# NDLOHGRP/pyReCoDe

Measured on AMD Instinct MI355X. Metric: frames/sec + GB/s in, 4096x4096 uint16 @1% sparsity, 1/2/4/8 GPU, higher is better.
Workload: dtype u16; 1 GPU; 4096x4096 uint16, 1.00% sparsity, L1 + LZ4 frame, source_bit_depth 16, batch 64 frames/GPU/step, 256-frame stack/GPU in HBM; parallelism=dp1 (contiguous frame blocks per rank; single process: no collective), gather_every=0, gathers_issued_in_all=0, launch=single process, collective_ranks=1

## Files before the change

### pyrecode_amd/csrc/rc_api.hip

```cpp
#include "rc_host.h"
#include "rc_deflate_model.h"

thread_local std::string g_last_error;
WorkerPool *g_pool = new WorkerPool;
Util g_utils[RC_MAX_DEV];
thread_local Util *t_util = nullptr;


struct rc_ctx {
    int device = 0;
    hipStream_t own_stream = nullptr, stream = nullptr;
    uint32_t nx = 0, ny = 0, depth = 0, level = 0, op_mode = 0, scheme = 0, clevel = 0, max_batch = 0;
    uint32_t emit = rc::EMIT_RAW;
    rc::Scratch sets[2];
    int cur = 0;
    int last = 0;
    const rc::Scratch &geo() const { return sets[0]; }
    const rc::Scratch &recent() const { return sets[last]; }
    DevMem dmem, model_mem[2];
    PinMem hmem;
    hipStream_t pstream = nullptr;
    hipStream_t pstream_b = nullptr;
    hipStream_t last_ps = nullptr;
    bool two_chains = false;
    hipEvent_t ev_red[2] = {}, ev_post[2] = {}, ev_in[2] = {};
    bool post_pending[2] = {false, false};
    bool pipelined = false;
    bool thr_set = false;
    bool keep_bitmap = true;
    uint32_t src_bytes = 2;
    uint32_t *thr32 = nullptr;
    uint32_t last_n = 0;
    DevBuf d_frames, d_out, d_dark;
    uint64_t *d_rec_off = nullptr;
    uint32_t *d_md = nullptr;
    void *d_ztab = nullptr;
    rc::ValueStage values = rc::VALUES_NONE;
    bool values_on = false;
    bool modelled = false, model_ready = false;
    rc::ZstdModel *d_model = nullptr, *h_model = nullptr;
    rc::ZstdSample *d_sample = nullptr, *h_sample = nullptr;
    rc::DeflateModel *d_dzm = nullptr, *h_dzm = nullptr;
    uint32_t *d_dzhist = nullptr, *h_dzhist = nullptr;
    uint32_t l2_sum = 0;
    rc::u32x2 *d_l2_node[2] = {};
    uint16_t *d_l2_base[2] = {};
    rc::BatchStatus *h_status = nullptr;
    rc::BatchStatus *d_first_err = nullptr;
    uint32_t batch_seq = 0;
    const uint8_t *prev_out = nullptr, *prev_rec = nullptr, *prev_md = nullptr;
    uint64_t prev_out_cap = 0;
    uint32_t prev_n = 0;
    hipEvent_t ev[5] = {};
    float stage_ms[5] = {};
    bool profiling = false;
    uint32_t prof_every = 1, prof_phase = 0;
    bool profile_all = getenv("RC_PROFILE_ALL_STAGES") != nullptr;
    struct PipeSlot {
        uint8_t *d_in = nullptr;
        uint8_t *d_out = nullptr;
        uint64_t *d_rec = nullptr, *h_rec = nullptr;
        uint32_t *d_md = nullptr, *h_md = nullptr;
        rc::BatchStatus *h_stat = nullptr;
        hipEvent_t ev_h2d = nullptr, ev_done = nullptr, ev_fetch = nullptr, ev_val = nullptr;
        uint32_t *d_val = nullptr, *h_val = nullptr;
        bool has_val = false;
        uint32_t n = 0;
        bool zero_copy = false;
        enum State { FREE, SUBMITTED, RESULT_TAKEN, FETCHING } state = FREE;
    } pipe[RC_PIPE_SLOTS];
    hipStream_t copy_stream = nullptr, d2h_stream = nullptr;
    uint32_t val_gap = 0, val_x0 = 0, val_y0 = 0, val_w = 0, val_h = 0;
    std::vector<hipEvent_t> prof_ev;
    size_t prof_used = 0;
    double prof_sum_ms[5] = {};
    uint64_t prof_batches = 0;
};

RC_EXPORT int rc_abi_version(void) { return RC_ABI_VERSION; }

RC_EXPORT const char *rc_strerror(int status)
{
    switch (status) {
    case RC_OK: return "ok";
    case RC_ERR_BAD_ARG: return "bad argument";
    case RC_ERR_OUT_TOO_SMALL: return "output buffer too small";
    case RC_ERR_DEVICE: return "GPU / HIP error";
    case RC_ERR_UNSUPPORTED: return "not implemented on device";
    case RC_ERR_RECORD_TOO_LARGE: return "Buffer size smaller than compressed data size";
    case RC_ERR_CORRUPT: return "corrupt input stream";
    case RC_ERR_WORKSPACE: return "out of device memory for the ctx's workspace";
    default: return "unknown status";
    }
}
RC_EXPORT const char *rc_last_error(void) { return g_last_error.c_str(); }

RC_EXPORT int rc_device_count(int *count)
{
    if (!count) return fail(RC_ERR_BAD_ARG, "count is NULL");
    int n = 0;
    if (hipGetDeviceCount(&n) != hipSuccess) {
        (void)hipGetLastError();
        n = 0;
    }
    *count = n;
    return RC_OK;
}
RC_EXPORT int rc_scheme_on_device(uint32_t scheme)
{
    return (scheme == RC_SCHEME_LZ4 || scheme == RC_SCHEME_ZSTD || scheme == RC_SCHEME_BLOSC_LZ4 || scheme == RC_SCHEME_ZLIB_DEVICE) ? 1 : 0;
}

static int alloc_set(rc_ctx *c, rc::Scratch &sc, DevMem &model_mem)
{
    using namespace rc;
    DevMem &m = c->dmem;
    const uint64_t B = c->max_batch, T = sc.ntiles;
    RC_ALLOC(m, sc.bitmap, B * sc.nb_stride + 64);
    RC_ALLOC(m, sc.tile_cnt, B * T * 4);
    RC_ALLOC(m, sc.tile_off, B * T * 4);
    RC_ALLOC(m, sc.tile_next, B * T * 4);
    RC_ALLOC(m, sc.frame_nnz, B * 4);
    RC_ALLOC(m, sc.frame_cbytes, B * 4);
    RC_ALLOC(m, sc.scan_part, B * ((T + 255) / 256) * 32);
    RC_ALLOC(m, sc.status, sizeof(BatchStatus));
    if (c->level != 3) RC_ALLOC(m, sc.pix_slots, B * T * TILE_PX * 2 + 64);
    if (c->emit != EMIT_RAW) {
        if (c->level == 1) {
            sc.comb = c->emit == EMIT_ZSTD ? COMB_AT_BLK_SLOT : COMB_BEHIND_BLOCK;
            sc.blk_stride = 1536;
        }
        RC_ALLOC(m, sc.blk_slots, B * T * (uint64_t)sc.blk_stride + 256);
        RC_ALLOC(m, sc.blk_size, B * T * 4);
        RC_ALLOC(m, sc.blk_off, B * T * 4);
        if (c->emit == EMIT_DEFLATE) {
            RC_ALLOC(m, sc.blk_aux, B * T * 4);
            RC_ALLOC(m, sc.zl_acc, B * 32);
            HIP_TRY(hipMemset(sc.zl_acc, 0, B * 32));
        }
    }
    if (c->values != VALUES_NONE) {
        const ValueGeom g = value_geom(c->values);
        sc.pixraw_stride = ((sc.N * 2 + 15) & ~15ull) + 32;
        sc.nchunk_max = (uint32_t)((sc.N * 2 + g.chunk - 1) / g.chunk) + 1;
        RC_ALLOC(model_mem, sc.pixraw, B * sc.pixraw_stride + 64);
        RC_ALLOC(model_mem, sc.pix_chunks, B * (uint64_t)sc.nchunk_max * g.slot + 64);
        if (c->values == VALUES_DEFLATE_HUFF) RC_ALLOC(model_mem, sc.chunk_aux, B * (uint64_t)(sc.nchunk_max + 1) * 8);
        RC_ALLOC(model_mem, sc.chunk_size, B * (uint64_t)sc.nchunk_max * 4);
        RC_ALLOC(model_mem, sc.chunk_off, B * (uint64_t)sc.nchunk_max * 4);
        RC_ALLOC(model_mem, sc.frame_pbytes, B * 4);
        HIP_TRY(hipMemset(sc.frame_pbytes, 0, B * 4));
    }
    HIP_TRY(hipMemset(sc.frame_nnz, 0, B * 4));
    HIP_TRY(hipMemset(sc.frame_cbytes, 0, B * 4));
    HIP_TRY(hipMemset(sc.status, 0, sizeof(BatchStatus)));
    return RC_OK;
}

static void free_value_stage(rc_ctx *c)
{
    c->values = rc::VALUES_NONE;
    c->values_on = false;
    for (int k = 0; k < 2; ++k) {
        rc::Scratch &set = c->sets[k];
        c->model_mem[k].release_all();
        set.pixraw = nullptr; set.pix_chunks = nullptr; set.chunk_aux = nullptr; set.chunk_size = nullptr; set.chunk_off = nullptr;
        set.frame_pbytes = nullptr; set.pixraw_stride = 0; set.nchunk_max = 0;
    }
}

static int ctx_alloc(rc_ctx *c)
{
    using namespace rc;
    const uint64_t B = c->max_batch;
    RC_ON_DEVICE(c->device);
    HIP_TRY(hipStreamCreateWithFlags(&c->own_stream, hipStreamNonBlocking));
    HIP_TRY(hipStreamCreateWithFlags(&c->pstream, hipStreamNonBlocking));
    {
        int lo = 0, hi = 0;
        HIP_TRY(hipDeviceGetStreamPriorityRange(&lo, &hi));
        HIP_TRY(hipStreamCreateWithPriority(&c->pstream_b, hipStreamNonBlocking, hi));
    }
    c->last_ps = c->pstream;
    c->stream = c->own_stream;
    DevMem &m = c->dmem;
    int r;
    RC_ALLOC(m, c->sets[0].thr, c->geo().N * 2);
    RC_ALLOC(m, c->d_first_err, sizeof(BatchStatus));
    HIP_TRY(hipMemset(c->d_first_err, 0, sizeof(BatchStatus)));
    c->sets[0].first_err = c->d_first_err;
    c->sets[1] = c->sets[0];
    for (int k = 0; k < 2; ++k)
        if ((r = alloc_set(c, c->sets[k], c->model_mem[k])) != RC_OK) return r;
    c->two_chains = false;
    if (c->level == 2) {
        const uint64_t ids = (uint64_t)c->geo().ntiles * rc::TILE_PX;
        RC_ALLOC(m, c->d_l2_node[0], B * ids * 8);
        HIP_TRY(hipMemset(c->d_l2_node[0], 0, B * ids * 8));
        RC_ALLOC(m, c->d_l2_base[0], B * (uint64_t)c->geo().ntiles * 64 * 2);
        for (int i = 0; i < 2; ++i) {
            Scratch &set = c->sets[i];
            set.l2_node = c->d_l2_node[0]; set.l2_ids_per_frame = ids; set.l2_base = c->d_l2_base[0];
        }
    }
    if (c->emit == EMIT_ZSTD) {
        if ((r = zstd_encoder_tables(m, c->d_ztab)) != RC_OK) return r;
        c->modelled = c->clevel != 0;
        if (c->modelled) {
            RC_ALLOC(m, c->d_model, sizeof(ZstdModel));
            RC_ALLOC(m, c->d_sample, sizeof(ZstdSample));
            RC_ALLOC(c->hmem, c->h_model, sizeof(ZstdModel));
            RC_ALLOC(c->hmem, c->h_sample, sizeof(ZstdSample));
        }
    }
    if (c->values == VALUES_DEFLATE_HUFF) {
        RC_ALLOC(m, c->d_dzm, sizeof(DeflateModel));
        RC_ALLOC(m, c->d_dzhist, 256 * 4);
        RC_ALLOC(c->hmem, c->h_dzm, sizeof(DeflateModel));
        RC_ALLOC(c->hmem, c->h_dzhist, 256 * 4);
    }
    RC_ALLOC(m, c->d_rec_off, (B + 1) * 8);
    RC_ALLOC(m, c->d_md, B * 3 * 4);
    RC_ALLOC(c->hmem, c->h_status, 2 * sizeof(BatchStatus));
    for (auto &e : c->ev) HIP_TRY(hipEventCreate(&e));
    for (auto &e : c->ev_red) HIP_TRY(hipEventCreateWithFlags(&e, hipEventDisableTiming));
    for (auto &e : c->ev_post) HIP_TRY(hipEventCreateWithFlags(&e, hipEventDisableTiming));
    for (auto &e : c->ev_in) HIP_TRY(hipEventCreateWithFlags(&e, hipEventDisableTiming));
    return RC_OK;
}

RC_EXPORT rc_ctx *rc_ctx_create(uint32_t nx, uint32_t ny, uint32_t src_bit_depth, uint32_t reduction_level,
                                uint32_t op_mode, uint32_t scheme, uint32_t clevel, int device_id, uint32_t max_batch,
                                int *status)
{
    int dummy;
    if (!status) status = &dummy;
    *status = RC_OK;
    if (nx == 0 || ny == 0 || max_batch == 0 || max_batch > 65535u || op_mode > 1) {
        *status = fail(RC_ERR_BAD_ARG, "nx, ny, max_batch must be > 0, max_batch <= 65535 and op_mode 0 or 1");
        return nullptr;
    }
    if ((uint64_t)nx * ny >= (1ull << 32)) {
        *status = fail(RC_ERR_BAD_ARG, "nx*ny must be < 2^32");
        return nullptr;
    }
    if ((uint64_t)nx * ny * 2 >= (1ull << 32)) {
        *status = fail(RC_ERR_UNSUPPORTED, "a raw frame of 4 GiB or more (nx*ny*bytes_per_pixel >= 2^32) does not fit the format's u32 size fields");
        return nullptr;
    }
    if (reduction_level < 1 || reduction_level > 3) {
        *status = fail(RC_ERR_UNSUPPORTED, "reduction_level 4 (centroiding) is not implemented on device");
        return nullptr;
    }
    if (reduction_level == 2 && nx > 65535u) {
        *status = fail(RC_ERR_UNSUPPORTED, "reduction_level 2 needs nx <= 65535");
        return nullptr;
    }
    if (src_bit_depth < 1 || src_bit_depth > 32) {
        *status = fail(RC_ERR_UNSUPPORTED, "source_bit_depth must be 1..32 (uint8 / uint16 / uint32 source frames)");
        return nullptr;
    }
    int ndev = 0;
    if (hipGetDeviceCount(&ndev) != hipSuccess || device_id < 0 || device_id >= ndev) {
        (void)hipGetLastError();
        *status = fail(RC_ERR_DEVICE, "no such HIP device (this library has no CPU path)");
        return nullptr;
    }
    rc_ctx *c = new (std::nothrow) rc_ctx();
    if (!c) {
        *status = fail(RC_ERR_DEVICE, "out of host memory");
        return nullptr;
    }
    c->device = device_id;
    c->nx = nx; c->ny = ny; c->depth = src_bit_depth; c->level = reduction_level; c->op_mode = op_mode;
    c->scheme = scheme; c->clevel = clevel; c->max_batch = max_batch;
    c->emit = (op_mode == 1 && rc_scheme_on_device(scheme)) ? scheme : rc::EMIT_RAW;
    c->values = rc::value_stage_of(c->emit, clevel, reduction_level);
    rc::Scratch &sc = c->sets[0];
    sc.N = (uint64_t)nx * ny;
    sc.ntiles = (uint32_t)((sc.N + rc::TILE_PX - 1) / rc::TILE_PX);
    sc.nb = (sc.N + 7) / 8;
    sc.nb_stride = (uint64_t)sc.ntiles * rc::TILE_BM;
    sc.max_batch = max_batch;
    sc.guarded_loads = getenv("RC_REDUCE_GUARDED_LOADS") != nullptr;
    int rcode = ctx_alloc(c);
    if (rcode != RC_OK) {
        *status = rcode;
        std::string keep = g_last_error;
        rc_ctx_destroy(c);
        g_last_error = keep;
        return nullptr;
    }
    return c;
}

RC_EXPORT int rc_ctx_destroy(rc_ctx *c)
{
    if (!c) return RC_OK;
    DeviceGuard dev_guard_;
    (void)dev_guard_.enter(c->device);
    for (hipStream_t st : {c->stream, c->pstream, c->pstream_b, c->own_stream, c->copy_stream, c->d2h_stream})
        if (st) (void)hipStreamSynchronize(st);
    c->dmem.release_all();
    for (DevMem &m : c->model_mem) m.release_all();
    c->hmem.release_all();
    for (auto &p : c->pipe)
        for (hipEvent_t e : {p.ev_h2d, p.ev_done, p.ev_fetch, p.ev_val})
            if (e) (void)hipEventDestroy(e);
    for (hipEvent_t e : {c->ev_red[0], c->ev_red[1], c->ev_post[0], c->ev_post[1], c->ev_in[0], c->ev_in[1]})
        if (e) (void)hipEventDestroy(e);
    for (auto &e : c->ev)
        if (e) (void)hipEventDestroy(e);
    for (auto &e : c->prof_ev) (void)hipEventDestroy(e);
    for (hipStream_t st : {c->copy_stream, c->d2h_stream, c->pstream, c->pstream_b, c->own_stream})
        if (st) (void)hipStreamDestroy(st);
    delete c;
    return RC_OK;
}

RC_EXPORT int rc_ctx_set_stream(rc_ctx *c, void *hip_stream)
{
    if (!c) return fail(RC_ERR_BAD_ARG, "ctx is NULL");
    c->stream = hip_stream ? reinterpret_cast<hipStream_t>(hip_stream) : c->own_stream;
    return RC_OK;
}

RC_EXPORT int rc_set_threshold(rc_ctx *c, const void *thr)
{
    if (!c || !thr) return fail(RC_ERR_BAD_ARG, "ctx / thr is NULL");
    if (c->depth > 16 && c->src_bytes != 4) return fail(RC_ERR_BAD_ARG, "src_bit_depth > 16 means uint32 sources: rc_ctx_set_source_bytes(ctx, 4) first");
    RC_ON_DEVICE(c->device);
    HIP_TRY(hipMemcpyAsync(c->src_bytes == 4 ? (void *)c->thr32 : (void *)c->geo().thr, thr, c->geo().N * (c->src_bytes == 4 ? 4 : 2),
                           is_device_ptr(thr) ? hipMemcpyDeviceToDevice : hipMemcpyHostToDevice,
                           c->stream));
    HIP_TRY(hipStreamSynchronize(c->stream));
    c->thr_set = true;
    return RC_OK;
}

RC_EXPORT int rc_set_dark(rc_ctx *c, const void *dark, int64_t epsilon)
{
    if (!c || !dark) return fail(RC_ERR_BAD_ARG, "ctx / dark is NULL");
    RC_ON_DEVICE(c->device);
    const void *src = dark;
    const uint64_t bytes = c->geo().N * c->src_bytes;
    if (!is_device_ptr(dark)) {
        int r = c->d_dark.ensure(c->dmem, bytes);
        if (r != RC_OK) return r;
        HIP_TRY(hipMemcpyAsync(c->d_dark.p, dark, bytes, hipMemcpyHostToDevice, c->stream));
        src = c->d_dark.p;
    }
    if (c->depth > 16 && c->src_bytes != 4) return fail(RC_ERR_BAD_ARG, "src_bit_depth > 16 means uint32 sources: rc_ctx_set_source_bytes(ctx, 4) first");
    if (c->src_bytes == 4) rc::launch_threshold32(static_cast<const uint32_t *>(src), epsilon, c->geo().N, c->thr32, c->stream);
    else rc::launch_threshold(src, epsilon, c->geo().N, c->geo().thr, c->stream, c->src_bytes);
    HIP_TRY(hipGetLastError());
    HIP_TRY(hipStreamSynchronize(c->stream));
    c->thr_set = true;
    return RC_OK;
}

RC_EXPORT int rc_ctx_set_source_bytes(rc_ctx *c, uint32_t bytes_per_pixel)
{
    if (!c) return fail(RC_ERR_BAD_ARG, "ctx is NULL");
    if (bytes_per_pixel != 1 && bytes_per_pixel != 2 && bytes_per_pixel != 4) return fail(RC_ERR_BAD_ARG, "rc_ctx_set_source_bytes: 1 (uint8), 2 (uint16) or 4 (uint32)");
    if (bytes_per_pixel == 1 && c->depth > 8) return fail(RC_ERR_BAD_ARG, "rc_ctx_set_source_bytes: uint8 sources need src_bit_depth <= 8");
    if (bytes_per_pixel == 2 && c->depth > 16) return fail(RC_ERR_BAD_ARG, "rc_ctx_set_source_bytes: uint16 sources need src_bit_depth <= 16");
    if (c->batch_seq || c->thr_set) return fail(RC_ERR_BAD_ARG, "rc_ctx_set_source_bytes: call before rc_set_dark / rc_set_threshold and the first batch");
    if (c->geo().N * bytes_per_pixel >= (1ull << 32))
        return fail(RC_ERR_UNSUPPORTED, "rc_ctx_set_source_bytes: a raw frame of 4 GiB or more (nx*ny*bytes_per_pixel >= 2^32) does not fit the format's u32 size fields");
    if (bytes_per_pixel == 4) {
        if (c->depth <= 16) return fail(RC_ERR_BAD_ARG, "rc_ctx_set_source_bytes: uint32 sources are what source_bit_depth > 16 means (misc.py:41-49)");
        if (c->level == 2) return fail(RC_ERR_UNSUPPORTED, "rc_ctx_set_source_bytes: reduction level 2 is not implemented for uint32 sources");
        if (c->emit == rc::EMIT_DEFLATE) return fail(RC_ERR_UNSUPPORTED, "rc_ctx_set_source_bytes: the device DEFLATE encoder is not implemented for uint32 sources (use RC_SCHEME_ZLIB: the host's zlib)");
        RC_ON_DEVICE(c->device);
        uint32_t *thr32 = nullptr;
        uint16_t *slots[2] = {nullptr, nullptr};
        bool ok = c->dmem.try_alloc(thr32, c->geo().N * 4) == hipSuccess;
        for (int k = 0; ok && k < 2 && c->level != 3; ++k)
            ok = c->dmem.try_alloc(slots[k], (uint64_t)c->max_batch * c->geo().ntiles * rc::TILE_PX * 4 + 64) == hipSuccess;
        if (!ok) {
            (void)hipGetLastError();
            c->dmem.free_one(thr32);
            for (uint16_t *&p : slots) c->dmem.free_one(p);
            return fail(RC_ERR_DEVICE, "rc_ctx_set_source_bytes: out of device memory for the uint32 threshold / residual slots");
        }
        if (c->depth % 8 == 0) c->depth = 32;
        c->modelled = false;
        free_value_stage(c);
        c->thr32 = thr32;
        for (int k = 0; k < 2; ++k) {
            rc::Scratch *set = &c->sets[k];
            set->pix_slot_bytes = rc::TILE_PX * 4;
            set->comb = rc::COMB_OFF;
            if (c->level != 3) {
                c->dmem.free_one(set->pix_slots);
                set->pix_slots = slots[k];
            }
        }
    }
    c->src_bytes = bytes_per_pixel;
    return RC_OK;
}
RC_EXPORT uint32_t rc_ctx_source_bytes(const rc_ctx *c) { return c ? c->src_bytes : 0; }

RC_EXPORT uint64_t rc_out_capacity(const rc_ctx *c, uint32_t n) { return c ? (uint64_t)n * c->geo().N * c->src_bytes : 0; }

RC_EXPORT uint32_t rc_md_fields(const rc_ctx *c)
{
    if (!c) return 0;
    const bool comp = c->emit != rc::EMIT_RAW;
    if (c->level != 3) return comp ? 3 : 1;
    return comp ? 1 : 0;
}

static int fit_value_model(rc_ctx *c, const void *frames_dev, uint32_t n)
{
    using namespace rc;
    const bool dz = c->values == VALUES_DEFLATE_HUFF;
    hipStream_t s = c->stream;
    const Scratch &sc = c->sets[c->cur];
    const uint32_t ns = n < 2 ? n : 2;
    void *d_sample = dz ? (void *)c->d_dzhist : c->d_sample, *h_sample = dz ? (void *)c->h_dzhist : c->h_sample;
    void *d_model = dz ? (void *)c->d_dzm : c->d_model, *h_model = dz ? (void *)c->h_dzm : c->h_model;
    const size_t sample_bytes = dz ? 256 * 4 : sizeof(ZstdSample), model_bytes = dz ? sizeof(DeflateModel) : sizeof(ZstdModel);
    for (int k = 0; k < 2; ++k)
        if (c->post_pending[k]) HIP_TRY(hipStreamWaitEvent(s, c->ev_post[k], 0));
    HIP_TRY(hipMemsetAsync(d_sample, 0, sample_bytes, s));
    if (dz) {
        launch_reduce(sc, frames_dev, ns, 1u, CODEC_DEFLATE, true, c->depth, s, nullptr, c->src_bytes);
        launch_scans(sc, ns, true, true, s);
        RecordParams rp;
        rp.level = 1u; rp.emit = c->emit; rp.depth = c->depth; rp.first_frame_id = 0; rp.packed_slots = 1u;
        rp.frame_bytes = c->geo().N * c->src_bytes;
        rp.pix_mode = PIX_MODE_FLAT;
        launch_assemble(sc, rp, ns, nullptr, nullptr, c->batch_seq, s);
        launch_pd_hist(sc, ns, c->depth, c->d_dzhist, s);
    } else {
        launch_reduce(sc, frames_dev, ns, c->level == 3 ? 3u : 1u, CODEC_ZSTD_FAST, true, c->depth, s, nullptr, c->src_bytes);
        launch_zstd_sample(sc, ns, c->level == 1, c->depth, c->d_sample, s);
    }
    HIP_TRY(hipGetLastError());
    HIP_TRY(hipMemcpyAsync(h_sample, d_sample, sample_bytes, hipMemcpyDeviceToHost, s));
    HIP_TRY(hipStreamSynchronize(s));
    if (dz) {
        dm_build_model(c->h_dzhist, c->h_dzm);
        c->values_on = c->h_dzm->usable != 0;
    } else {
        zstd_model_from_sample(c->h_sample, c->h_model, c->clevel == 1 ? 50u : (c->clevel == 2 ? 20u : 0u));
        if (c->values == VALUES_NONE || !zm_code_pays(c->h_sample->pix, c->h_model->pix_code)) c->h_model->valid &= ~ZM_PIX_CODE;
        c->values_on = (c->h_model->valid & ZM_PIX_CODE) != 0;
    }
    HIP_TRY(hipMemcpyAsync(d_model, h_model, model_bytes, hipMemcpyHostToDevice, s));
    HIP_TRY(hipStreamSynchronize(s));
    for (Scratch &set : c->sets) {
        if (dz) { set.dz_model = c->d_dzm; continue; }
        const ZstdModel &M = *c->h_model;
        set.zm_model = c->d_model;
        set.zm_lit_code = c->d_model->lit_code;
        set.zm_valid = M.valid;
        set.zm_budget = zm_block_budget(M, BLK_SLOT);
        set.zm_seq_bits = (M.valid & ZM_SEQ_TABLES) ? M.seq.ll_log + M.seq.ml_log : 12u;
    }
    c->model_ready = true;
    return RC_OK;
}

static uint32_t fused_codec(uint32_t emit, uint32_t clevel, bool modelled, uint32_t src_bytes)
{
    using namespace rc;
    switch (emit) {
    case EMIT_ZSTD: return modelled && src_bytes != 4 ? CODEC_ZSTD_MODELLED : CODEC_ZSTD_FAST;
    case EMIT_LZ4: return clevel != 0 ? CODEC_LZ4_EVENTS : CODEC_LZ4_RUNS;
    case EMIT_BLOSC: return CODEC_BLOSC;
    case EMIT_DEFLATE: return CODEC_DEFLATE;
    default: return CODEC_NONE;
    }
}

static int enqueue_batch(rc_ctx *c, const void *frames_dev, uint32_t n, uint32_t first_frame_id, uint8_t *out_dev,
                         uint64_t out_cap, uint64_t *rec_off_dev, uint32_t *md_dev, bool timed)
{
    using namespace rc;
    hipStream_t s = c->stream;
    if ((c->modelled || c->values == VALUES_DEFLATE_HUFF) && !c->model_ready) {
        int r = fit_value_model(c, frames_dev, n);
        if (r != RC_OK) return r;
    }
    RecordParams rp;
    rp.level = c->level == 3 ? 3u : 1u;
    rp.emit = c->emit; rp.depth = c->depth; rp.first_frame_id = first_frame_id;
    rp.packed_slots = 1u;
    rp.frame_bytes = c->geo().N * c->src_bytes;
    hipEvent_t *ev = nullptr;
    if (timed) ev = c->ev;
    else if (c->profiling && (c->prof_phase++ % c->prof_every) == 0) {
        if (c->prof_used + 5 > c->prof_ev.size()) {
            for (int i = 0; i < 5; ++i) {
                hipEvent_t e;
                HIP_TRY(hipEventCreate(&e));
                c->prof_ev.push_back(e);
            }
        }
        ev = c->prof_ev.data() + c->prof_used;
        c->prof_used += 5;
    }
    const int k = c->cur;
    c->cur ^= 1;
    c->last = k;
    const rc::Scratch &sc = c->sets[k];
    const bool two = c->pipelined && c->two_chains;
    hipStream_t ps = two && k == 1 ? c->pstream_b : c->pstream;
    c->last_ps = ps;
    if (c->post_pending[k]) HIP_TRY(hipStreamWaitEvent(s, c->ev_post[k], 0));
    if (ev) HIP_TRY(hipEventRecord(ev[0], s));
    const bool fitted_seq = c->modelled && (c->h_model->valid & ZM_SEQ_TABLES);
    hipStream_t tail = nullptr;
    if (sc.N % TILE_PX) {
        HIP_TRY(hipEventRecord(c->ev_in[k], s));
        HIP_TRY(hipStreamWaitEvent(ps, c->ev_in[k], 0));
        tail = ps;
    }
    const uint32_t codec = fused_codec(c->emit, c->clevel, c->modelled, c->src_bytes);
    const bool keep_maps = c->keep_bitmap || c->emit == EMIT_RAW;
    if (c->src_bytes == 4)
        launch_reduce32(sc, static_cast<const uint32_t *>(frames_dev), c->thr32, n, c->level, c->depth, s, codec, keep_maps);
    else
        launch_reduce(sc, frames_dev, n, c->level, codec, keep_maps, c->depth, s, tail, c->src_bytes);
    const bool all_ev = ev && (timed || c->profile_all);
    hipEvent_t red = ev ? ev[1] : c->ev_red[k];
    HIP_TRY(hipEventRecord(red, s));
    HIP_TRY(hipStreamWaitEvent(ps, red, 0));
    if (c->level == 2) launch_l2(sc, n, c->nx, c->l2_sum, c->depth, ps);
    const bool lits_only = c->modelled && (c->h_model->valid & ZM_LITS_ONLY);
    if (c->emit == EMIT_ZSTD && !lits_only) launch_zstd_fse(sc, n, fitted_seq ? (const void *)&c->d_model->seq : c->d_ztab, fitted_seq, ps);
    if (all_ev) HIP_TRY(hipEventRecord(ev[2], ps));
    launch_scans(sc, n, c->level != 3, c->emit != EMIT_RAW, ps);
    if (all_ev) HIP_TRY(hipEventRecord(ev[3], ps));
    if (c->values_on) {
        rp.pix_mode = PIX_MODE_FLAT;
        launch_assemble(sc, rp, n, out_dev, rec_off_dev, c->batch_seq, ps);
        launch_values_encode(c->values, sc, n, c->depth, ps);
        launch_values_scan(c->values, sc, n, c->depth, ps);
        rp.pix_mode = PIX_MODE_SKIP;
    }
    if (two && c->post_pending[k ^ 1]) {
        auto overlap = [](const uint8_t *a, uint64_t an, const uint8_t *b, uint64_t bn) { return a && b && a < b + bn && b < a + an; };
        const uint8_t *rec8 = reinterpret_cast<const uint8_t *>(rec_off_dev), *md8 = reinterpret_cast<const uint8_t *>(md_dev);
        if (overlap(out_dev, out_cap, c->prev_out, c->prev_out_cap) || overlap(rec8, (uint64_t)(n + 1) * 8, c->prev_rec, (uint64_t)(c->prev_n + 1) * 8) ||
            overlap(md8, (uint64_t)n * 12, c->prev_md, (uint64_t)c->prev_n * 12))
            HIP_TRY(hipStreamWaitEvent(ps, c->ev_post[k ^ 1], 0));
    }
    c->prev_out = out_dev; c->prev_out_cap = out_cap; c->prev_n = n;
    c->prev_rec = reinterpret_cast<const uint8_t *>(rec_off_dev); c->prev_md = reinterpret_cast<const uint8_t *>(md_dev);
    launch_layout(sc, rp, n, out_cap, rec_off_dev, md_dev, ps);
    launch_assemble(sc, rp, n, out_dev, rec_off_dev, c->batch_seq, ps);
    ++c->batch_seq;
    if (c->values_on) launch_values_gather(c->values, sc, n, c->depth, 16, out_dev, rec_off_dev, ps);
    if (ev) HIP_TRY(hipEventRecord(ev[4], ps));
    if (two && c->post_pending[k ^ 1]) HIP_TRY(hipStreamWaitEvent(ps, c->ev_post[k ^ 1], 0));
    HIP_TRY(hipEventRecord(c->ev_post[k], ps));
    c->post_pending[k] = true;
    if (!c->pipelined) HIP_TRY(hipStreamWaitEvent(s, c->ev_post[k], 0));
    HIP_TRY(hipGetLastError());
    c->last_n = n;
    return RC_OK;
}

static int check_batch_args(rc_ctx *c, const void *frames, uint32_t n, const void *out, const void *rec, const void *md)
{
    if (!c || !frames || !out || !rec || !md) return fail(RC_ERR_BAD_ARG, "NULL argument");
    if (n == 0 || n > c->max_batch) return fail(RC_ERR_BAD_ARG, "n must be in 1..max_batch");
    if (!c->thr_set) return fail(RC_ERR_BAD_ARG, "threshold not set (rc_set_threshold / rc_set_dark)");
    return RC_OK;
}

RC_EXPORT int rc_reduce_compress_batch_async(rc_ctx *c, const void *frames_dev, uint32_t n, uint32_t first_frame_id,
                                             uint8_t *out_dev, uint64_t out_cap, uint64_t *rec_offsets_dev, uint32_t *md_dev)
{
    int r = check_batch_args(c, frames_dev, n, out_dev, rec_offsets_dev, md_dev);
    if (r != RC_OK) return r;
    RC_ON_DEVICE(c->device);
    return enqueue_batch(c, frames_dev, n, first_frame_id, out_dev, out_cap, rec_offsets_dev, md_dev, false);
}

static void l2_second_chain(rc_ctx *c)
{
    if (c->level != 2 || c->two_chains) return;
    const uint64_t B = c->max_batch, ids = (uint64_t)c->geo().ntiles * rc::TILE_PX;
    if (!c->d_l2_node[1]) {
        bool ok = c->dmem.try_alloc(c->d_l2_node[1], B * ids * 8) == hipSuccess && hipMemset(c->d_l2_node[1], 0, B * ids * 8) == hipSuccess &&
                  c->dmem.try_alloc(c->d_l2_base[1], B * (uint64_t)c->geo().ntiles * 64 * 2) == hipSuccess && hipDeviceSynchronize() == hipSuccess;
        if (!ok) {
            (void)hipGetLastError();
            c->dmem.free_one(c->d_l2_node[1]);
            c->dmem.free_one(c->d_l2_base[1]);
            return;
        }
    }
    c->sets[1].l2_node = c->d_l2_node[1];
    c->sets[1].l2_base = c->d_l2_base[1];
    c->two_chains = true;
}

RC_EXPORT int rc_ctx_set_pipelined(rc_ctx *c, int on)
{
    if (!c) return fail(RC_ERR_BAD_ARG, "ctx is NULL");
    RC_ON_DEVICE(c->device);
    HIP_TRY(hipStreamSynchronize(c->pstream));
    HIP_TRY(hipStreamSynchronize(c->pstream_b));
    if (on) l2_second_chain(c);
    c->pipelined = on != 0;
    return RC_OK;
}
RC_EXPORT int rc_ctx_wait_results(rc_ctx *c, void *hip_stream)
{
    if (!c) return fail(RC_ERR_BAD_ARG, "ctx is NULL");
    RC_ON_DEVICE(c->device);
    if (c->post_pending[c->last])
        HIP_TRY(hipStreamWaitEvent(hip_stream ? reinterpret_cast<hipStream_t>(hip_stream) : c->stream, c->ev_post[c->last], 0));
    return RC_OK;
}

RC_EXPORT int rc_ctx_sync(rc_ctx *c)
{
    if (!c) return fail(RC_ERR_BAD_ARG, "ctx is NULL");
    RC_ON_DEVICE(c->device);
    HIP_TRY(hipStreamSynchronize(c->pstream_b));
    HIP_TRY(hipMemcpyAsync(&c->h_status[0], c->recent().status, sizeof(rc::BatchStatus), hipMemcpyDeviceToHost, c->pstream));
    HIP_TRY(hipMemcpyAsync(&c->h_status[1], c->d_first_err, sizeof(rc::BatchStatus), hipMemcpyDeviceToHost, c->pstream));
    HIP_TRY(hipMemsetAsync(c->d_first_err, 0, sizeof(rc::BatchStatus), c->pstream));
    HIP_TRY(hipStreamSynchronize(c->pstream));
    HIP_TRY(hipStreamSynchronize(c->stream));
    const uint32_t n_batches = c->batch_seq;
    c->batch_seq = 0;
    for (size_t b = 0; b + 5 <= c->prof_used; b += 5) {
        float ms;
        if (!c->profile_all) {
            if (hipEventElapsedTime(&ms, c->prof_ev[b], c->prof_ev[b + 1]) == hipSuccess) c->prof_sum_ms[0] += ms;
        } else
        for (int i = 0; i < 4; ++i)
            if (hipEventElapsedTime(&ms, c->prof_ev[b + i], c->prof_ev[b + i + 1]) == hipSuccess) c->prof_sum_ms[i] += ms;
        if (hipEventElapsedTime(&ms, c->prof_ev[b], c->prof_ev[b + 4]) == hipSuccess) c->prof_sum_ms[4] += ms;
        ++c->prof_batches;
    }
    c->prof_used = 0;
    if (c->h_status[1].total != 0) c->h_status[1] = rc::first_err_decode(c->h_status[1].total);
    if (c->h_status[1].code != 0) {
        char msg[160];
        if (n_batches > 1)
            snprintf(msg, sizeof msg, "%s (frame %u of batch %llu of the %u enqueued since the last sync)", rc_strerror(c->h_status[1].code),
                     c->h_status[1].frame, (unsigned long long)c->h_status[1].total, n_batches);
        else
            snprintf(msg, sizeof msg, "%s (frame %u of the batch)", rc_strerror(c->h_status[1].code), c->h_status[1].frame);
        return fail(c->h_status[1].code, msg);
    }
    return RC_OK;
}

RC_EXPORT int rc_reduce_compress_batch(rc_ctx *c, const void *frames, uint32_t n, uint32_t first_frame_id, uint8_t *out,
                                       uint64_t out_cap, uint64_t *rec_offsets, uint32_t *md)
{
    int r = check_batch_args(c, frames, n, out, rec_offsets, md);
    if (r != RC_OK) return r;
    RC_ON_DEVICE(c->device);
    const uint64_t frame_bytes = c->geo().N * c->src_bytes;
    const void *fdev = frames;
    if (!is_device_ptr(frames)) {
        r = c->d_frames.ensure(c->dmem, (uint64_t)n * frame_bytes);
        if (r != RC_OK) return r;
        HIP_TRY(hipMemcpyAsync(c->d_frames.p, frames, (uint64_t)n * frame_bytes, hipMemcpyHostToDevice, c->stream));
        fdev = c->d_frames.p;
    }
    uint8_t *odev = out;
    uint64_t cap = out_cap;
    const bool out_host = !is_device_ptr(out);
    if (out_host) {
        const uint64_t worst = (uint64_t)n * frame_bytes;
        cap = out_cap < worst ? out_cap : worst;
        r = c->d_out.ensure(c->dmem, cap);
        if (r != RC_OK) return r;
        odev = c->d_out.p;
    }
    r = enqueue_batch(c, fdev, n, first_frame_id, odev, cap, c->d_rec_off, c->d_md, true);
    if (r != RC_OK) return r;
    r = rc_ctx_sync(c);
    for (int i = 0; i < 4; ++i) (void)hipEventElapsedTime(&c->stage_ms[i], c->ev[i], c->ev[i + 1]);
    (void)hipEventElapsedTime(&c->stage_ms[4], c->ev[0], c->ev[4]);
    if (r != RC_OK) return r;
    int r2 = copy_out(rec_offsets, c->d_rec_off, (uint64_t)(n + 1) * 8, c->stream);
    if (r2 == RC_OK) r2 = copy_out(md, c->d_md, (uint64_t)n * 12, c->stream);
    if (r2 == RC_OK && out_host) r2 = copy_out(out, c->d_out.p, c->h_status->total, c->stream);
    if (r2 != RC_OK) return r2;
    HIP_TRY(hipStreamSynchronize(c->stream));
    return RC_OK;
}

RC_EXPORT void *rc_host_alloc(uint64_t bytes)
{
    void *p = nullptr;
    if (hipHostMalloc(&p, bytes ? bytes : 16, hipHostMallocDefault) != hipSuccess) {
        (void)hipGetLastError();
        fail(RC_ERR_DEVICE, "hipHostMalloc failed");
        return nullptr;
    }
    return p;
}
RC_EXPORT int rc_host_free(void *p)
{
    if (p) HIP_TRY(hipHostFree(p));
    return RC_OK;
}
RC_EXPORT int rc_host_register(void *p, uint64_t bytes)
{
    if (!p || !bytes) return fail(RC_ERR_BAD_ARG, "NULL / zero argument");
    HIP_TRY(hipHostRegister(p, bytes, hipHostRegisterDefault));
    return RC_OK;
}
RC_EXPORT int rc_host_unregister(void *p)
{
    if (p) HIP_TRY(hipHostUnregister(p));
    return RC_OK;
}

static int pipe_slot_init(rc_ctx *c, rc_ctx::PipeSlot &p)
{
    const uint64_t B = c->max_batch;
    if (!c->copy_stream) HIP_TRY(hipStreamCreateWithFlags(&c->copy_stream, hipStreamNonBlocking));
    if (!c->d2h_stream) HIP_TRY(hipStreamCreateWithFlags(&c->d2h_stream, hipStreamNonBlocking));
    RC_ALLOC(c->dmem, p.d_in, B * c->geo().N * c->src_bytes + 64);
    RC_ALLOC(c->dmem, p.d_out, rc_out_capacity(c, (uint32_t)B) + 64);
    RC_ALLOC(c->dmem, p.d_rec, (B + 1) * 8);
    RC_ALLOC(c->dmem, p.d_md, B * 12);
    RC_ALLOC(c->hmem, p.h_rec, (B + 1) * 8);
    RC_ALLOC(c->hmem, p.h_md, B * 12);
    RC_ALLOC(c->hmem, p.h_stat, sizeof(rc::BatchStatus));
    HIP_TRY(hipEventCreateWithFlags(&p.ev_h2d, hipEventDisableTiming));
    HIP_TRY(hipEventCreateWithFlags(&p.ev_done, hipEventDisableTiming));
    HIP_TRY(hipEventCreateWithFlags(&p.ev_fetch, hipEventDisableTiming));
    HIP_TRY(hipEventCreateWithFlags(&p.ev_val, hipEventDisableTiming));
    RC_ALLOC(c->dmem, p.d_val, B * 4 + 64);
    RC_ALLOC(c->hmem, p.h_val, B * 4 + 64);
    return RC_OK;
}

RC_EXPORT int rc_ctx_set_validation(rc_ctx *c, uint32_t gap, uint32_t x0, uint32_t y0, uint32_t w, uint32_t h)
{
    if (!c) return fail(RC_ERR_BAD_ARG, "ctx is NULL");
    if (gap && (w == 0 || h == 0 || w > 128 || h > 128 || (uint64_t)x0 + w > c->nx || (uint64_t)y0 + h > c->ny))
        return fail(RC_ERR_BAD_ARG, "rc_ctx_set_validation: the region must lie inside the frame and hold at most 128 x 128 pixels");
    c->val_gap = gap; c->val_x0 = x0; c->val_y0 = y0; c->val_w = w; c->val_h = h;
    return RC_OK;
}

RC_EXPORT int rc_pipe_validation(rc_ctx *c, uint32_t slot, uint32_t *counts)
{
    if (!c || slot >= RC_PIPE_SLOTS || !counts) return fail(RC_ERR_BAD_ARG, "NULL argument / slot out of range");
    rc_ctx::PipeSlot &p = c->pipe[slot];
    if (p.state != p.SUBMITTED && p.state != p.RESULT_TAKEN) return fail(RC_ERR_BAD_ARG, "nothing submitted on this slot");
    if (!p.has_val) { for (uint32_t i = 0; i < p.n; ++i) counts[i] = 0xFFFFFFFFu; return RC_OK; }
    HIP_TRY(hipEventSynchronize(p.ev_val));
    memcpy(counts, p.h_val, (uint64_t)p.n * 4);
    return RC_OK;
}

RC_EXPORT int rc_pipe_submit(rc_ctx *c, uint32_t slot, const void *frames_host, uint32_t n, uint32_t first_frame_id)
{
    if (!c || !frames_host || slot >= RC_PIPE_SLOTS) return fail(RC_ERR_BAD_ARG, "NULL argument / slot out of range");
    if (n == 0 || n > c->max_batch) return fail(RC_ERR_BAD_ARG, "n must be in 1..max_batch");
    if (!c->thr_set) return fail(RC_ERR_BAD_ARG, "threshold not set (rc_set_threshold / rc_set_dark)");
    RC_ON_DEVICE(c->device);
    rc_ctx::PipeSlot &p = c->pipe[slot];
    if (p.state != p.FREE) return fail(RC_ERR_BAD_ARG, "slot is still in use (result / fetch_wait not called)");
    if (!p.d_in) {
        int r = pipe_slot_init(c, p);
        if (r != RC_OK) return r;
    }
    if (!c->pipelined) {
        HIP_TRY(hipStreamSynchronize(c->pstream));
        HIP_TRY(hipStreamSynchronize(c->pstream_b));
        l2_second_chain(c);
        c->pipelined = true;
    }
    const void *fdev = nullptr;
    hipPointerAttribute_t a;
    if (hipPointerGetAttributes(&a, frames_host) == hipSuccess) {
        if (a.type == hipMemoryTypeHost && a.devicePointer) fdev = a.devicePointer;
    } else (void)hipGetLastError();
    p.zero_copy = fdev != nullptr;
    if (!fdev) {
        HIP_TRY(hipMemcpyAsync(p.d_in, frames_host, (uint64_t)n * c->geo().N * c->src_bytes, hipMemcpyHostToDevice, c->copy_stream));
        HIP_TRY(hipEventRecord(p.ev_h2d, c->copy_stream));
        HIP_TRY(hipStreamWaitEvent(c->stream, p.ev_h2d, 0));
        fdev = p.d_in;
    }
    int r = enqueue_batch(c, fdev, n, first_frame_id, p.d_out, rc_out_capacity(c, c->max_batch), p.d_rec, p.d_md, false);
    if (r != RC_OK) return r;
    p.has_val = c->val_gap != 0;
    if (p.has_val) {
        rc::launch_roi_components(fdev, c->src_bytes == 4 ? (const void *)c->thr32 : (const void *)c->geo().thr, c->geo().N, c->nx, n, first_frame_id, c->val_gap, c->val_x0, c->val_y0, c->val_w, c->val_h, p.d_val, c->stream, c->src_bytes);
        HIP_TRY(hipGetLastError());
        HIP_TRY(hipMemcpyAsync(p.h_val, p.d_val, (uint64_t)n * 4, hipMemcpyDeviceToHost, c->stream));
        HIP_TRY(hipEventRecord(p.ev_val, c->stream));
    }
    if (p.zero_copy) HIP_TRY(hipEventRecord(p.ev_h2d, c->stream));
    hipStream_t ps = c->last_ps;
    HIP_TRY(hipMemcpyAsync(p.h_rec, p.d_rec, (uint64_t)(n + 1) * 8, hipMemcpyDeviceToHost, ps));
    HIP_TRY(hipMemcpyAsync(p.h_md, p.d_md, (uint64_t)n * 12, hipMemcpyDeviceToHost, ps));
    HIP_TRY(hipMemcpyAsync(p.h_stat, c->recent().status, sizeof(rc::BatchStatus), hipMemcpyDeviceToHost, ps));
    HIP_TRY(hipEventRecord(p.ev_done, ps));
    p.n = n;
    p.state = p.SUBMITTED;
    return RC_OK;
}

RC_EXPORT int rc_pipe_input_done(rc_ctx *c, uint32_t slot)
{
    if (!c || slot >= RC_PIPE_SLOTS) return fail(RC_ERR_BAD_ARG, "NULL argument / slot out of range");
    if (c->pipe[slot].state == rc_ctx::PipeSlot::FREE) return RC_OK;
    HIP_TRY(hipEventSynchronize(c->pipe[slot].ev_h2d));
    return RC_OK;
}

RC_EXPORT int rc_pipe_result(rc_ctx *c, uint32_t slot, uint64_t *rec_offsets, uint32_t *md, uint64_t *total)
{
    if (!c || slot >= RC_PIPE_SLOTS || !rec_offsets || !md || !total) return fail(RC_ERR_BAD_ARG, "NULL argument / slot out of range");
    rc_ctx::PipeSlot &p = c->pipe[slot];
    if (p.state != p.SUBMITTED) return fail(RC_ERR_BAD_ARG, "nothing submitted on this slot");
    HIP_TRY(hipEventSynchronize(p.ev_done));
    p.state = p.RESULT_TAKEN;
    if (p.h_stat->code != 0) {
        char msg[128];
        snprintf(msg, sizeof msg, "%s (frame %u of the batch)", rc_strerror(p.h_stat->code), p.h_stat->frame);
        p.state = p.FREE;
        return fail(p.h_stat->code, msg);
    }
    memcpy(rec_offsets, p.h_rec, (uint64_t)(p.n + 1) * 8);
    memcpy(md, p.h_md, (uint64_t)p.n * 12);
    *total = p.h_stat->total;
    return RC_OK;
}

RC_EXPORT int rc_pipe_fetch(rc_ctx *c, uint32_t slot, uint8_t *dst_host, uint64_t bytes)
{
    if (!c || slot >= RC_PIPE_SLOTS || (!dst_host && bytes)) return fail(RC_ERR_BAD_ARG, "NULL argument / slot out of range");
    rc_ctx::PipeSlot &p = c->pipe[slot];
    if (p.state != p.RESULT_TAKEN) return fail(RC_ERR_BAD_ARG, "rc_pipe_result has not been called for this slot");
    if (bytes > p.h_stat->total) return fail(RC_ERR_BAD_ARG, "more bytes than the batch's records hold");
    RC_ON_DEVICE(c->device);
    if (bytes) HIP_TRY(hipMemcpyAsync(dst_host, p.d_out, bytes, hipMemcpyDeviceToHost, c->d2h_stream));
    HIP_TRY(hipEventRecord(p.ev_fetch, c->d2h_stream));
    p.state = p.FETCHING;
    return RC_OK;
}

RC_EXPORT int rc_pipe_fetch_wait(rc_ctx *c, uint32_t slot)
{
    if (!c || slot >= RC_PIPE_SLOTS) return fail(RC_ERR_BAD_ARG, "NULL argument / slot out of range");
    rc_ctx::PipeSlot &p = c->pipe[slot];
    if (p.state == p.RESULT_TAKEN) { p.state = p.FREE; return RC_OK; }
    if (p.state != p.FETCHING) return fail(RC_ERR_BAD_ARG, "rc_pipe_fetch has not been called for this slot");
    HIP_TRY(hipEventSynchronize(p.ev_fetch));
    p.state = p.FREE;
    return RC_OK;
}

RC_EXPORT int rc_ctx_refit_model(rc_ctx *c)
{
    if (!c) return fail(RC_ERR_BAD_ARG, "ctx is NULL");
    c->model_ready = false;
    return RC_OK;
}

RC_EXPORT int rc_get_binary_map(rc_ctx *c, uint32_t i, uint8_t *bitmap_out)
{
    if (!c || !bitmap_out) return fail(RC_ERR_BAD_ARG, "NULL argument");
    if (i >= c->last_n) return fail(RC_ERR_BAD_ARG, "frame index outside the most recent batch");
    if (!c->keep_bitmap && c->emit != rc::EMIT_RAW && c->level != 2) return fail(RC_ERR_BAD_ARG, "binary maps are not kept (rc_ctx_keep_binary_maps(ctx, 0))");
    RC_ON_DEVICE(c->device);
    int r = copy_out(bitmap_out, c->recent().bitmap + (uint64_t)i * c->geo().nb_stride, c->geo().nb, c->stream);
    if (r != RC_OK) return r;
    HIP_TRY(hipStreamSynchronize(c->stream));
    return RC_OK;
}

RC_EXPORT int rc_ctx_set_profiling(rc_ctx *c, int on)
{
    if (!c) return fail(RC_ERR_BAD_ARG, "ctx is NULL");
    c->profiling = on != 0;
    c->prof_every = on > 1 ? (uint32_t)on : 1u;
    c->prof_phase = 0;
    for (double &v : c->prof_sum_ms) v = 0;
    c->prof_batches = 0;
    return RC_OK;
}
RC_EXPORT int rc_ctx_get_profile(rc_ctx *c, double sum_ms[5], uint64_t *batches)
{
    if (!c || !sum_ms || !batches) return fail(RC_ERR_BAD_ARG, "NULL argument");
    memcpy(sum_ms, c->prof_sum_ms, sizeof c->prof_sum_ms);
    *batches = c->prof_batches;
    return RC_OK;
}

RC_EXPORT int rc_ctx_set_l2_statistics(rc_ctx *c, uint32_t l2_statistics)
{
    if (!c || l2_statistics > 2) return fail(RC_ERR_BAD_ARG, "l2_statistics must be 0, 1 (max) or 2 (sum)");
    c->l2_sum = l2_statistics == 2 ? 1u : 0u;
    return RC_OK;
}

RC_EXPORT int rc_ctx_keep_binary_maps(rc_ctx *c, int on)
{
    if (!c) return fail(RC_ERR_BAD_ARG, "ctx is NULL");
    c->keep_bitmap = on != 0;
    return RC_OK;
}

RC_EXPORT int rc_get_stage_ms(rc_ctx *c, float ms[5])
{
    if (!c || !ms) return fail(RC_ERR_BAD_ARG, "NULL argument");
    memcpy(ms, c->stage_ms, sizeof c->stage_ms);
    return RC_OK;
}

RC_EXPORT int64_t rc_unpack_frame_sparse(uint32_t nx, uint32_t ny, uint32_t bit_depth, const uint8_t *bitmap,
                                         const uint8_t *pixvals, uint64_t pixvals_bytes, uint64_t *out,
                                         uint64_t out_cap_triplets, uint32_t reduction_level)
{
    if (!bitmap || nx == 0 || ny == 0 || (!out && out_cap_triplets)) return fail(RC_ERR_BAD_ARG, "NULL / zero argument");
    if (reduction_level == 1 && (bit_depth == 0 || bit_depth > 64)) return fail(RC_ERR_BAD_ARG, "bit_depth must be 1..64");
    if (reduction_level == 1 && !pixvals && pixvals_bytes) return fail(RC_ERR_BAD_ARG, "pixvals is NULL");
    UtilScope util_scope;
    int r = util_scope.enter();
    if (r != RC_OK) return r;
    Util &u = g_util;
    const uint64_t N = (uint64_t)nx * ny, nb = (N + 7) / 8, nb8 = (nb + 7) / 8;
    const uint32_t nblk = (uint32_t)((nb8 + rc::WG - 1) / rc::WG);
    const uint8_t *d_bm = nullptr, *d_px = nullptr;
    r = stage_in(bitmap, nb, u.a, d_bm, nb8 * 8 - nb + 8);
    if (r != RC_OK) return r;
    if (reduction_level == 1 && pixvals_bytes) {
        r = stage_in(pixvals, pixvals_bytes, u.b, d_px);
        if (r != RC_OK) return r;
    }
    r = u.w.ensure(u.dmem, (uint64_t)nblk * 8 + 16);
    if (r != RC_OK) return r;
    uint32_t *blk_cnt = u.w.as<uint32_t>(), *blk_off = blk_cnt + nblk;
    uint64_t *nnz_dev = reinterpret_cast<uint64_t *>(blk_cnt + 2 * (uint64_t)nblk);
    rc::launch_expand_count(d_bm, nb8, N, blk_cnt, blk_off, nnz_dev, u.stream);
    HIP_TRY(hipMemcpyAsync(u.h_scalar, nnz_dev, 8, hipMemcpyDeviceToHost, u.stream));
    HIP_TRY(hipStreamSynchronize(u.stream));
    const uint64_t nnz = *u.h_scalar;
    if (!out) return (int64_t)nnz;
    if (nnz > out_cap_triplets) return fail(RC_ERR_OUT_TOO_SMALL, "out holds fewer triplets than the bitmap has set bits");
    if (reduction_level == 1 && (nnz * bit_depth + 7) / 8 > pixvals_bytes)
        return fail(RC_ERR_CORRUPT, "pixvals shorter than popcount(bitmap) * bit_depth bits");
    if (nnz == 0) return 0;
    StagedOut so;
    if ((r = so.begin(out, nnz * 24)) != RC_OK) return r;
    rc::launch_expand_emit(d_bm, nb8, N, nx, blk_off, d_px, pixvals_bytes, bit_depth, reduction_level, nnz, so.as<uint64_t>(), u.stream);
    HIP_TRY(hipGetLastError());
    if ((r = so.finish(out, nnz * 24)) != RC_OK) return r;
    return (int64_t)nnz;
}

RC_EXPORT int rc_bit_pack(const uint16_t *pixvals, uint64_t n, uint32_t bit_depth, uint8_t *out, uint64_t out_n)
{
    if (!out || (!pixvals && n)) return fail(RC_ERR_BAD_ARG, "NULL argument");
    if (bit_depth == 0 || bit_depth > 32) return fail(RC_ERR_BAD_ARG, "bit_depth must be 1..32");
    if (out_n != (n * bit_depth + 7) / 8) return fail(RC_ERR_BAD_ARG, "out_n must be ceil(n*bit_depth/8)");
    if (out_n == 0) return RC_OK;
    UtilScope util_scope;
    int r = util_scope.enter();
    if (r != RC_OK) return r;
    Util &u = g_util;
    const uint16_t *d_in = nullptr;
    r = stage_in(pixvals, n * 2, u.a, d_in);
    if (r != RC_OK) return r;
    StagedOut so;
    if ((r = so.begin(out, out_n)) != RC_OK) return r;
    rc::launch_bit_pack(d_in, n, bit_depth, so.as<uint8_t>(), out_n, u.stream);
    HIP_TRY(hipGetLastError());
    return so.finish(out, out_n);
}

RC_EXPORT int rc_bit_unpack(const uint8_t *packed, uint64_t packed_bytes, uint64_t n, uint32_t bit_depth, uint64_t *out)
{
    if (!out || (!packed && packed_bytes)) return fail(RC_ERR_BAD_ARG, "NULL argument");
    if (bit_depth == 0 || bit_depth > 64) return fail(RC_ERR_BAD_ARG, "bit_depth must be 1..64");
    if ((n * bit_depth + 7) / 8 > packed_bytes) return fail(RC_ERR_CORRUPT, "packed shorter than n * bit_depth bits");
    if (n == 0) return RC_OK;
    UtilScope util_scope;
    int r = util_scope.enter();
    if (r != RC_OK) return r;
    Util &u = g_util;
    const uint8_t *d_in = nullptr;
    r = stage_in(packed, packed_bytes, u.a, d_in);
    if (r != RC_OK) return r;
    StagedOut so;
    if ((r = so.begin(out, n * 8)) != RC_OK) return r;
    rc::launch_bit_unpack(d_in, packed_bytes, n, bit_depth, so.as<uint64_t>(), u.stream);
    HIP_TRY(hipGetLastError());
    return so.finish(out, n * 8);
}

RC_EXPORT int rc_synth_dark(int device_id, uint32_t seed, uint64_t n_pixels, uint16_t *dark_dev)
{
    if (!dark_dev) return fail(RC_ERR_BAD_ARG, "NULL argument");
    RC_ON_DEVICE(device_id);
    rc::launch_synth_dark(seed, n_pixels, dark_dev, nullptr);
    HIP_TRY(hipGetLastError());
    HIP_TRY(hipDeviceSynchronize());
    return RC_OK;
}
RC_EXPORT int rc_synth_frames_clustered(int device_id, uint32_t seed, uint32_t first_frame, uint32_t n_frames, uint32_t nx, uint32_t ny,
                                        uint32_t seed_ppm, const uint16_t *dark_dev, uint16_t *frames_dev)
{
    if (!dark_dev || !frames_dev || n_frames == 0 || nx == 0 || ny == 0) return fail(RC_ERR_BAD_ARG, "NULL / zero argument");
    if ((uint64_t)nx * ny > 0xFFFFFFFFull) return fail(RC_ERR_BAD_ARG, "rc_synth_frames_clustered: nx * ny must fit 32 bits");
    RC_ON_DEVICE(device_id);
    rc::launch_synth_frames_clustered(seed, first_frame, n_frames, nx, ny, seed_ppm, dark_dev, frames_dev, nullptr);
    HIP_TRY(hipGetLastError());
    HIP_TRY(hipDeviceSynchronize());
    return RC_OK;
}
RC_EXPORT int rc_synth_frames(int device_id, uint32_t seed, uint32_t first_frame, uint32_t n_frames, uint64_t n_pixels,
                              uint32_t sparsity_ppm, const uint16_t *dark_dev, uint16_t *frames_dev)
{
    if (!dark_dev || !frames_dev || n_frames == 0) return fail(RC_ERR_BAD_ARG, "NULL / zero argument");
    RC_ON_DEVICE(device_id);
    rc::launch_synth_frames(seed, first_frame, n_frames, n_pixels, sparsity_ppm, dark_dev, frames_dev, nullptr);
    HIP_TRY(hipGetLastError());
    HIP_TRY(hipDeviceSynchronize());
    return RC_OK;
}
```

### pyrecode_amd/csrc/rc_codec_api.hip

```cpp
#include "rc_host.h"

template <class Encode, class Total, class Gather>
static int tiled_compress(const uint8_t *src, uint64_t n, uint8_t *dst, uint64_t dst_cap, uint64_t *out_n, const uint8_t *empty, uint64_t empty_n,
                          Encode encode, Total total_of, Gather gather)
{
    using namespace rc;
    Util &u = g_util;
    if (n == 0) {
        if (dst_cap < empty_n) return fail(RC_ERR_OUT_TOO_SMALL, "rc_compress: dst too small");
        HIP_TRY(hipMemcpy(dst, empty, empty_n, is_device_ptr(dst) ? hipMemcpyHostToDevice : hipMemcpyHostToHost));
        *out_n = empty_n;
        return RC_OK;
    }
    Scratch sc;
    sc.ntiles = (uint32_t)((n + TILE_BM - 1) / TILE_BM);
    sc.nb = n;
    sc.nb_stride = (uint64_t)sc.ntiles * TILE_BM;
    const uint8_t *d_src = nullptr;
    int r = stage_in(src, n, u.a, d_src, sc.nb_stride - n + 16);
    if (r != RC_OK) return r;
    sc.bitmap = const_cast<uint8_t *>(d_src);
    const uint64_t T = sc.ntiles;
    r = u.w.ensure(u.dmem, T * BLK_SLOT + T * 8 + 64);
    if (r != RC_OK) return r;
    sc.blk_slots = u.w.p;
    sc.blk_size = reinterpret_cast<uint32_t *>(u.w.p + T * BLK_SLOT);
    sc.blk_off = sc.blk_size + T;
    sc.frame_cbytes = sc.blk_off + T;
    if ((r = encode(sc)) != RC_OK) return r;
    launch_scans(sc, 1, false, true, u.stream);
    HIP_TRY(hipMemcpyAsync(u.h_scalar, sc.frame_cbytes, 4, hipMemcpyDeviceToHost, u.stream));
    HIP_TRY(hipStreamSynchronize(u.stream));
    const uint64_t total = total_of(T, *reinterpret_cast<uint32_t *>(u.h_scalar));
    if (total > dst_cap) return fail(RC_ERR_OUT_TOO_SMALL, "rc_compress: dst too small (see rc_compress_bound)");
    StagedOut so;
    if ((r = so.begin(dst, total)) != RC_OK) return r;
    gather(sc, so.as<uint8_t>());
    HIP_TRY(hipGetLastError());
    if ((r = so.finish(dst, total)) != RC_OK) return r;
    *out_n = total;
    return RC_OK;
}

RC_EXPORT int rc_compress(uint32_t scheme, uint32_t level, const uint8_t *src, uint64_t n, uint8_t *dst, uint64_t dst_cap,
                          uint64_t *out_n)
{
    using namespace rc;
    if (!dst || !out_n || (!src && n)) return fail(RC_ERR_BAD_ARG, "NULL argument");
    if (scheme != RC_SCHEME_LZ4 && scheme != RC_SCHEME_ZSTD && scheme != RC_SCHEME_BLOSC_LZ4)
        return fail(RC_ERR_UNSUPPORTED, "rc_compress: compression scheme not implemented on device");
    UtilScope util_scope;
    int r = util_scope.enter();
    if (r != RC_OK) return r;
    Util &u = g_util;
    if (scheme == RC_SCHEME_BLOSC_LZ4) {
        if (n >= (1ull << 31) - 16) return fail(RC_ERR_BAD_ARG, "rc_compress: a blosc1 chunk holds < 2 GiB");
        const uint8_t f[16] = {2, 1, 0x36, 8, 0, 0, 0, 0, 0, 0, 0, 0, 16, 0, 0, 0};
        return tiled_compress(src, n, dst, dst_cap, out_n, f, sizeof f,
                              [&](const Scratch &sc) { launch_blosc_encode_blocks(sc, 1, u.stream); return RC_OK; },
                              [](uint64_t T, uint32_t blocks) { return 16ull + 4ull * T + blocks; },
                              [&](const Scratch &sc, uint8_t *d_out) { launch_blosc_gather(sc, d_out, u.stream); });
    }
    if (n >= (1ull << 32)) return fail(RC_ERR_BAD_ARG, "rc_compress: input must be < 4 GiB");
    if (scheme == RC_SCHEME_LZ4) {
        const uint32_t h = lz4f_descriptor(0x40);
        const uint8_t f[11] = {0x04, 0x22, 0x4D, 0x18, (uint8_t)h, (uint8_t)(h >> 8), (uint8_t)(h >> 16), 0, 0, 0, 0};
        return tiled_compress(src, n, dst, dst_cap, out_n, f, sizeof f,
                              [&](const Scratch &sc) { launch_lz4_encode_buffer(sc, u.stream, level != 0); return RC_OK; },
                              [](uint64_t, uint32_t blocks) { return 7ull + blocks + 4; },
                              [&](const Scratch &sc, uint8_t *d_out) { launch_lz4f_gather(sc, h, d_out, u.stream); });
    }
    const uint8_t f[9] = {0x28, 0xB5, 0x2F, 0xFD, 0x00, 0x00, 0x01, 0x00, 0x00};
    return tiled_compress(src, n, dst, dst_cap, out_n, f, sizeof f,
                          [&](const Scratch &sc) {
                              int rt = zstd_encoder_tables(u.dmem, u.ztab);
                              if (rt == RC_OK) launch_zstd_encode_blocks(sc, 1, u.ztab, u.stream);
                              return rt;
                          },
                          [](uint64_t, uint32_t blocks) { return 6ull + blocks; },
                          [&](const Scratch &sc, uint8_t *d_out) { launch_zstd_gather(sc, d_out, u.stream); });
}

static int lz4_decompress(const uint8_t *src, uint64_t n, uint8_t *dst, uint64_t dst_cap, uint64_t *out_n)
{
    using namespace rc;
    Util &u = g_util;
    HostView h;
    int r = h.open(src, n);
    if (r != RC_OK) return r;
    if (n < 11 || h.rd32(0) != 0x184D2204u) return fail(RC_ERR_CORRUPT, "not an LZ4 frame");
    const uint32_t flg = h[4], bd = h[5];
    if ((flg >> 6) != 1 || (flg & 2) || (bd & 0x8F) || ((bd >> 4) & 7) < 4) return fail(RC_ERR_CORRUPT, "bad LZ4 frame descriptor");
    const int linked = !((flg >> 5) & 1), bsum = (flg >> 4) & 1, csize = (flg >> 3) & 1, csum = (flg >> 2) & 1, dict = flg & 1;
    const uint64_t bmax = 1ull << (8 + 2 * ((bd >> 4) & 7));
    uint64_t ip = 6 + (csize ? 8 : 0) + (dict ? 4 : 0) + 1;
    std::vector<Lz4Block> blks;
    for (;;) {
        if (ip + 4 > n) return fail(RC_ERR_CORRUPT, "truncated LZ4 frame");
        uint32_t bs = h.rd32(ip);
        ip += 4;
        if (bs == 0) break;
        const uint32_t raw = bs >> 31;
        bs &= 0x7FFFFFFFu;
        if (bs > bmax || ip + bs > n) return fail(RC_ERR_CORRUPT, "LZ4 block exceeds the frame");
        blks.push_back(Lz4Block{ip, bs, raw});
        ip += bs + (bsum ? 4 : 0);
    }
    if (csum) ip += 4;
    if (ip != n) return fail(RC_ERR_CORRUPT, "trailing bytes after the LZ4 frame");
    const uint32_t nblk = (uint32_t)blks.size();
    if (nblk == 0) { *out_n = 0; return RC_OK; }
    const uint8_t *d_src = nullptr;
    r = stage_in(src, n, u.a, d_src);
    if (r != RC_OK) return r;
    const uint64_t tab = (uint64_t)nblk * sizeof(Lz4Block), szs = ((uint64_t)nblk * 4 + 7) & ~7ull, offs = (uint64_t)nblk * 8;
    r = u.w.ensure(u.dmem, tab + szs + offs + 16);
    if (r != RC_OK) return r;
    Lz4Block *d_blks = u.w.as<Lz4Block>();
    uint32_t *d_sizes = reinterpret_cast<uint32_t *>(u.w.p + tab);
    uint64_t *d_offs = reinterpret_cast<uint64_t *>(u.w.p + tab + szs);
    int *d_err = reinterpret_cast<int *>(u.w.p + tab + szs + offs);
    HIP_TRY(hipMemcpyAsync(d_blks, blks.data(), tab, hipMemcpyHostToDevice, u.stream));
    HIP_TRY(hipMemsetAsync(d_err, 0, 4, u.stream));
    launch_lz4_decode(d_src, d_blks, nblk, d_sizes, nullptr, nullptr, ~0ull, linked, d_err, u.stream);
    std::vector<uint32_t> sizes(nblk);
    int err = 0;
    HIP_TRY(hipMemcpyAsync(sizes.data(), d_sizes, (uint64_t)(linked ? 1 : nblk) * 4, hipMemcpyDeviceToHost, u.stream));
    HIP_TRY(hipMemcpyAsync(&err, d_err, 4, hipMemcpyDeviceToHost, u.stream));
    HIP_TRY(hipStreamSynchronize(u.stream));
    if (err) return fail(RC_ERR_CORRUPT, "malformed LZ4 block");
    std::vector<uint64_t> off(nblk, 0);
    uint64_t total = 0;
    if (linked) total = sizes[0];
    else
        for (uint32_t b = 0; b < nblk; ++b) {
            if (sizes[b] > bmax) return fail(RC_ERR_CORRUPT, "LZ4 block decodes beyond its declared maximum");
            off[b] = total;
            total += sizes[b];
        }
    *out_n = total;
    if (total > dst_cap) return fail(RC_ERR_OUT_TOO_SMALL, "rc_decompress: dst too small");
    if (total == 0) return RC_OK;
    StagedOut so;
    if ((r = so.begin(dst, total)) != RC_OK) return r;
    HIP_TRY(hipMemcpyAsync(d_offs, off.data(), offs, hipMemcpyHostToDevice, u.stream));
    uint32_t max_stored = 0;
    for (const Lz4Block &q : blks) if (q.raw) max_stored = std::max(max_stored, q.size);
    launch_lz4_decode(d_src, d_blks, nblk, nullptr, d_offs, so.as<uint8_t>(), total, linked, d_err, u.stream, max_stored);
    HIP_TRY(hipGetLastError());
    HIP_TRY(hipMemcpyAsync(&err, d_err, 4, hipMemcpyDeviceToHost, u.stream));
    if ((r = so.finish(dst, total)) != RC_OK) return r;
    if (err) return fail(RC_ERR_CORRUPT, "malformed LZ4 block");
    return RC_OK;
}

static int blosc_decompress(const uint8_t *src, uint64_t n, uint8_t *dst, uint64_t dst_cap, uint64_t *out_n)
{
    using namespace rc;
    Util &u = g_util;
    HostView h;
    int r = h.open(src, n);
    if (r != RC_OK) return r;
    if (n < 16 || h[0] != 2) return fail(RC_ERR_CORRUPT, "not a blosc1 chunk");
    const uint32_t flags = h[2], typesize = h[3] ? h[3] : 1;
    const uint64_t nbytes = h.rd32(4), blocksize = h.rd32(8), cbytes = h.rd32(12);
    if (cbytes != n || nbytes >= (1ull << 31)) return fail(RC_ERR_CORRUPT, "blosc1 header disagrees with the chunk length");
    *out_n = nbytes;
    if (nbytes > dst_cap) return fail(RC_ERR_OUT_TOO_SMALL, "rc_decompress: dst too small");
    if (nbytes == 0) return RC_OK;
    if (flags & 0x02) {
        if (n != 16 + nbytes) return fail(RC_ERR_CORRUPT, "bad memcpyed blosc1 chunk");
        HIP_TRY(hipMemcpy(dst, src + 16, nbytes, hipMemcpyDefault));
        return RC_OK;
    }
    if ((flags >> 5) != 1) return fail(RC_ERR_UNSUPPORTED, "blosc1 chunk: only the LZ4 codec is decoded on device");
    if (blocksize == 0 || blocksize > nbytes) return fail(RC_ERR_CORRUPT, "bad blosc1 blocksize");
    const uint64_t nblocks = (nbytes + blocksize - 1) / blocksize;
    if (16 + 4 * nblocks > n) return fail(RC_ERR_CORRUPT, "truncated blosc1 chunk");
    std::vector<Lz4Block> blks;
    std::vector<uint64_t> offs;
    std::vector<uint32_t> want;
    for (uint64_t b = 0; b < nblocks; ++b) {
        const uint64_t bsize = std::min<uint64_t>(blocksize, nbytes - b * blocksize);
        const bool leftover = bsize != blocksize;
        const bool split = !(flags & 0x10) && typesize <= 16 && blocksize / typesize >= 128 && !leftover;
        const uint32_t nsplits = split ? typesize : 1;
        const uint64_t neblock = bsize / nsplits;
        uint64_t pos = h.rd32(16 + 4 * b);
        for (uint32_t j = 0; j < nsplits; ++j) {
            if (pos + 4 > n) return fail(RC_ERR_CORRUPT, "blosc1 block table points outside the chunk");
            const uint32_t cs = h.rd32(pos);
            pos += 4;
            if (pos + cs > n || cs > neblock + neblock / 255 + 16) return fail(RC_ERR_CORRUPT, "blosc1 block exceeds the chunk");
            blks.push_back(Lz4Block{pos, cs, cs == neblock ? 1u : 0u});
            offs.push_back(b * blocksize + j * neblock);
            want.push_back((uint32_t)neblock);
            pos += cs;
        }
    }
    const uint32_t nb = (uint32_t)blks.size();
    const uint8_t *d_src = nullptr;
    r = stage_in(src, n, u.a, d_src);
    if (r != RC_OK) return r;
    const uint64_t tab = (uint64_t)nb * sizeof(Lz4Block), szs = ((uint64_t)nb * 4 + 7) & ~7ull, ofs = (uint64_t)nb * 8;
    r = u.w.ensure(u.dmem, tab + szs + ofs + 16);
    if (r != RC_OK) return r;
    r = u.b.ensure(u.dmem, nbytes + 16);
    if (r != RC_OK) return r;
    Lz4Block *d_blks = u.w.as<Lz4Block>();
    uint32_t *d_sizes = reinterpret_cast<uint32_t *>(u.w.p + tab);
    uint64_t *d_offs = reinterpret_cast<uint64_t *>(u.w.p + tab + szs);
    int *d_err = reinterpret_cast<int *>(u.w.p + tab + szs + ofs);
    HIP_TRY(hipMemcpyAsync(d_blks, blks.data(), tab, hipMemcpyHostToDevice, u.stream));
    HIP_TRY(hipMemcpyAsync(d_offs, offs.data(), ofs, hipMemcpyHostToDevice, u.stream));
    HIP_TRY(hipMemsetAsync(d_err, 0, 4, u.stream));
    launch_lz4_decode(d_src, d_blks, nb, d_sizes, nullptr, nullptr, ~0ull, 0, d_err, u.stream);
    std::vector<uint32_t> sizes(nb);
    int err = 0;
    HIP_TRY(hipMemcpyAsync(sizes.data(), d_sizes, (uint64_t)nb * 4, hipMemcpyDeviceToHost, u.stream));
    HIP_TRY(hipMemcpyAsync(&err, d_err, 4, hipMemcpyDeviceToHost, u.stream));
    HIP_TRY(hipStreamSynchronize(u.stream));
    if (err) return fail(RC_ERR_CORRUPT, "malformed LZ4 block inside the blosc1 chunk");
    for (uint32_t i = 0; i < nb; ++i)
        if (sizes[i] != want[i]) return fail(RC_ERR_CORRUPT, "blosc1 block decodes to the wrong size");
    uint32_t max_stored = 0;
    for (const Lz4Block &q : blks) if (q.raw) max_stored = std::max(max_stored, q.size);
    launch_lz4_decode(d_src, d_blks, nb, nullptr, d_offs, u.b.p, nbytes, 0, d_err, u.stream, max_stored);
    StagedOut so;
    if ((r = so.begin(dst, nbytes)) != RC_OK) return r;
    launch_blosc_unshuffle(u.b.p, so.as<uint8_t>(), nbytes, (uint32_t)blocksize, typesize, (flags & 0x04) ? 4u : ((flags & 0x01) ? 1u : 0u), u.stream);
    HIP_TRY(hipGetLastError());
    HIP_TRY(hipMemcpyAsync(&err, d_err, 4, hipMemcpyDeviceToHost, u.stream));
    if ((r = so.finish(dst, nbytes)) != RC_OK) return r;
    if (err) return fail(RC_ERR_CORRUPT, "malformed LZ4 block inside the blosc1 chunk");
    return RC_OK;
}

static int zstd_decompress(const uint8_t *src, uint64_t n, uint8_t *dst, uint64_t dst_cap, uint64_t *out_n)
{
    using namespace rc;
    Util &u = g_util;
    HostView h;
    int r = h.open(src, n);
    if (r != RC_OK) return r;
    std::vector<ZdBlock> all, comp, raw;
    ZdTables T;
    uint64_t bound = 0;
    const int zr = zd_index_frame(h.h, 0, n, 0, TILE_BM, ~0ull, all, T, &bound);
    if (zr == ZD_FOREIGN) return fail(RC_ERR_UNSUPPORTED, "rc_decompress: zstd stream outside the device decoder's subset (use the stock decoder)");
    if (zr != ZD_OK) return fail(RC_ERR_CORRUPT, "malformed zstd frame");
    uint32_t raw_max = 0;
    for (const ZdBlock &b : all) {
        if (b.type == 2) { if (b.regen > 1024) return fail(RC_ERR_UNSUPPORTED, "rc_decompress: zstd block larger than the device decoder's rows"); comp.push_back(b); }
        else { raw.push_back(b); raw_max = std::max(raw_max, b.regen); }
    }
    if (bound > dst_cap + 1024) { *out_n = bound; return fail(RC_ERR_OUT_TOO_SMALL, "rc_decompress: dst too small (out_n = an upper bound of the decoded size)"); }
    uint32_t row = TILE_BM;
    for (const ZdBlock &b : comp) if (b.regen > (uint32_t)TILE_BM) row = 1024;
    const uint8_t *d_src = nullptr;
    r = stage_in(src, n, u.a, d_src);
    if (r != RC_OK) return r;
    const uint64_t sz_blk = (comp.size() + raw.size()) * sizeof(ZdBlock) + 64;
    if ((r = u.zd_blocks.ensure(u.dmem, sz_blk)) != RC_OK || (r = u.zd_tables.ensure(u.dmem, sizeof(ZdTables) + 64)) != RC_OK ||
        (r = u.zd_ctl.ensure(u.dmem, 256)) != RC_OK || (r = u.zd_out.ensure(u.dmem, bound + 64)) != RC_OK ||
        (r = zstd_predefined_tables(u)) != RC_OK)
        return r;
    hipStream_t s = u.stream;
    ZdBlock *d_comp = u.zd_blocks.as<ZdBlock>(), *d_raw = d_comp + comp.size();
    ZdFrameList *d_lists = u.zd_ctl.as<ZdFrameList>();
    uint64_t *d_base = reinterpret_cast<uint64_t *>(u.zd_ctl.p + 32);
    int *d_err = reinterpret_cast<int *>(u.zd_ctl.p + 48);
    uint32_t *d_prod = reinterpret_cast<uint32_t *>(u.zd_ctl.p + 56);
    const ZdFrameList lists[2] = {{d_comp, (uint32_t)comp.size(), 0}, {d_raw, (uint32_t)raw.size(), 0}};
    const uint64_t base0 = 0;
    const uint32_t none = 0xFFFFFFFFu;
    if (!comp.empty()) HIP_TRY(hipMemcpyAsync(d_comp, comp.data(), comp.size() * sizeof(ZdBlock), hipMemcpyHostToDevice, s));
    if (!raw.empty()) HIP_TRY(hipMemcpyAsync(d_raw, raw.data(), raw.size() * sizeof(ZdBlock), hipMemcpyHostToDevice, s));
    HIP_TRY(hipMemcpyAsync(u.zd_tables.p, &T, sizeof T, hipMemcpyHostToDevice, s));
    HIP_TRY(hipMemcpyAsync(d_lists, lists, sizeof lists, hipMemcpyHostToDevice, s));
    HIP_TRY(hipMemcpyAsync(d_base, &base0, 8, hipMemcpyHostToDevice, s));
    HIP_TRY(hipMemsetAsync(d_err, 0, 4, s));
    HIP_TRY(hipMemsetAsync(u.zd_out.p, 0, bound + 64, s));
    HIP_TRY(hipMemcpyAsync(d_prod, &none, 4, hipMemcpyHostToDevice, s));
    if (!comp.empty()) launch_block_decode(rc::EMIT_ZSTD, (int)row, d_src, d_lists, 1, (uint32_t)comp.size(), u.zd_tables.p, u.zd_predef, u.zd_out.p, d_base, d_err, s, d_prod);
    launch_block_copy(d_src, d_lists + 1, 1, (uint32_t)raw.size(), raw_max, u.zd_out.p, d_base, s);
    HIP_TRY(hipGetLastError());
    int err = 0;
    uint32_t prod = none;
    HIP_TRY(hipMemcpyAsync(&err, d_err, 4, hipMemcpyDeviceToHost, s));
    HIP_TRY(hipMemcpyAsync(&prod, d_prod, 4, hipMemcpyDeviceToHost, s));
    HIP_TRY(hipStreamSynchronize(s));
    if (err) return fail(RC_ERR_CORRUPT, "malformed zstd block");
    uint64_t total = bound;
    if (prod != none) {
        for (const ZdBlock &b : comp) if (b.flex) total = bound - (b.regen - prod);
    }
    *out_n = total;
    if (total > dst_cap) return fail(RC_ERR_OUT_TOO_SMALL, "rc_decompress: dst too small");
    if (total) HIP_TRY(hipMemcpy(dst, u.zd_out.p, total, is_device_ptr(dst) ? hipMemcpyDeviceToDevice : hipMemcpyDeviceToHost));
    return RC_OK;
}

RC_EXPORT int rc_decompress(uint32_t scheme, const uint8_t *src, uint64_t n, uint8_t *dst, uint64_t dst_cap, uint64_t *out_n)
{
    if (!src || !out_n || (!dst && dst_cap)) return fail(RC_ERR_BAD_ARG, "NULL argument");
    if (scheme != RC_SCHEME_LZ4 && scheme != RC_SCHEME_BLOSC_LZ4 && scheme != RC_SCHEME_ZSTD)
        return fail(RC_ERR_UNSUPPORTED, "rc_decompress: compression scheme not implemented on device");
    UtilScope util_scope;
    int r = util_scope.enter();
    if (r != RC_OK) return r;
    if (scheme == RC_SCHEME_ZSTD) return zstd_decompress(src, n, dst, dst_cap, out_n);
    return scheme == RC_SCHEME_LZ4 ? lz4_decompress(src, n, dst, dst_cap, out_n) : blosc_decompress(src, n, dst, dst_cap, out_n);
}
RC_EXPORT uint64_t rc_compress_bound(uint32_t scheme, uint64_t n)
{
    const uint64_t blocks = (n + rc::TILE_BM - 1) / rc::TILE_BM;
    if (scheme == RC_SCHEME_LZ4) return 7 + n + 4 * blocks + 4;
    if (scheme == RC_SCHEME_ZSTD) return 9 + n + 3 * blocks;
    if (scheme == RC_SCHEME_BLOSC_LZ4) return 16 + n + 8 * blocks;
    return 0;
}
```

### pyrecode_amd/csrc/rc_gather.hip

```cpp
#include <cstdlib>

#include "rc_launch.h"
#include "rc_record.h"
#include "rc_deflate_block.h"

namespace rc {

struct GatherArgs {
    const uint8_t *blk_slots, *bitmap;
    const uint16_t *pix_slots;
    const uint32_t *blk_size, *blk_off, *tile_cnt, *tile_off, *tile_next, *frame_nnz, *frame_cbytes, *frame_pbytes;
    const uint32_t *blk_aux;
    uint32_t *zl_acc;
    uint8_t *pixraw;
    BatchStatus *status, *first_err;
    uint64_t nb, nb_stride, pixraw_stride;
    uint32_t ntiles, blk_stride, pix_slot_bytes, comb;
};

typedef u32x4 u32x4_u __attribute__((aligned(1)));
typedef u32x2 u32x2_u __attribute__((aligned(1)));
typedef uint32_t u32_u __attribute__((aligned(1)));
typedef uint16_t u16_u __attribute__((aligned(1)));

__device__ __forceinline__ uint32_t lane_get(uint32_t v, uint32_t src_lane)
{
    return (uint32_t)__builtin_amdgcn_ds_bpermute((int)(4u * src_lane), (int)v);
}

template <bool BITS>
__device__ __forceinline__ u32x4 shift_piece(const u32x4 &x, uint32_t e, uint32_t sh)
{
    u32x4 y = x;
    if (BITS) {
        y[0] = __builtin_amdgcn_alignbit(x[1], x[0], sh); y[1] = __builtin_amdgcn_alignbit(x[2], x[1], sh);
        y[2] = __builtin_amdgcn_alignbit(x[3], x[2], sh); y[3] = __builtin_amdgcn_alignbit(e, x[3], sh);
    }
    return y;
}
__device__ __forceinline__ void put_piece(uint8_t *p, const u32x4 &y, uint32_t valid)
{
    if (valid >= 16) { *reinterpret_cast<u32x4_u *>(p) = y; return; }
    uint32_t a0 = y[0], a1 = y[1];
    if (valid & 8u) { *reinterpret_cast<u32x2_u *>(p) = u32x2{a0, a1}; p += 8; a0 = y[2]; a1 = y[3]; }
    if (valid & 4u) { *reinterpret_cast<u32_u *>(p) = a0; p += 4; a0 = a1; }
    if (valid & 2u) { *reinterpret_cast<u16_u *>(p) = (uint16_t)a0; p += 2; a0 >>= 16; }
    if (valid & 1u) *p = (uint8_t)a0;
}

struct AdlerAcc { uint32_t A, W; };
__device__ __forceinline__ void adler_piece(AdlerAcc &acc, const u32x4 &y, uint32_t valid, uint32_t sp)
{
    uint32_t a = 0, q = 0;
#pragma unroll
    for (int k = 0; k < 4; ++k) {
        const uint32_t nb = valid > 4u * k ? min(valid - 4u * k, 4u) : 0u;
        const uint32_t v = y[k] & (nb >= 4u ? 0xFFFFFFFFu : ((1u << (8u * nb)) - 1u));
        a = __builtin_amdgcn_sad_u8(v, 0u, a);
        q = __builtin_amdgcn_udot4(v, 0x03020100u + 0x04040404u * (uint32_t)k, q, false);
    }
    acc.A += a;
    acc.W = (acc.W + (sp % ADLER_P) * a + q) % ADLER_P;
}
__device__ __forceinline__ void adler_byte(AdlerAcc &acc, uint32_t byte, uint32_t sp)
{
    acc.A += byte;
    acc.W = (acc.W + (sp % ADLER_P) * byte) % ADLER_P;
}

struct ResidGeom { uint32_t b_lo, n, ps0, avail; };
__device__ __forceinline__ ResidGeom resid_geom(uint32_t coff, uint32_t cnt, uint32_t d)
{
    const uint64_t dbit = (uint64_t)coff * d;
    const uint32_t nbits = cnt * d;
    const uint64_t b_lo = (dbit + 7) >> 3, b_hi = (dbit + nbits + 7) >> 3;
    ResidGeom g{(uint32_t)b_lo, (uint32_t)(b_hi - b_lo), (uint32_t)(8 * b_lo - dbit), (uint32_t)((dbit + nbits) & 7u)};
    if (g.avail && g.n) --g.n;
    else g.avail = 0;
    return g;
}

constexpr int GATHER_U = 4, GATHER_UB = 3;
constexpr int GATHER_WPE = 8;
template <bool BITS, int U, bool ADLER>
__global__ __launch_bounds__(64) __attribute__((amdgpu_waves_per_eu(GATHER_WPE))) void k_gather(GatherArgs sc, RecordParams rp, uint8_t *__restrict__ out, const uint64_t *__restrict__ rec_off,
                                               uint32_t lz4f_hdr_bitmap, uint32_t lz4f_hdr_pix, uint32_t batch_seq, uint32_t gpf, uint32_t nitems, uint32_t tpi)
{
    if (sc.status->code != 0) {
        if (blockIdx.x == 0 && threadIdx.x == 0 && sc.first_err)
            atomicMax(reinterpret_cast<unsigned long long *>(&sc.first_err->total), first_err_key(batch_seq, sc.status->code, sc.status->frame));
        return;
    }
    const uint32_t lane = (uint32_t)lane_id();
    const bool flat = rp.pix_mode == PIX_MODE_FLAT, skip_pix = rp.pix_mode == PIX_MODE_SKIP;
    const bool pixp = rp.level == 1 && rp.packed_slots && !skip_pix;
    const bool plain_pos = rp.emit == EMIT_RAW || flat;
    const uint32_t d = rp.depth;
    const FrameFmt ff = frame_fmt(rp.emit);
    const uint32_t bhdr = bitmap_hdr(ff, rp.emit, sc.ntiles);
    const uint8_t *pix_base = reinterpret_cast<const uint8_t *>(sc.pix_slots);
    for (uint32_t item = blockIdx.x; item < nitems; item += gridDim.x) {
        const uint32_t f = item / gpf, g = item - f * gpf, t0 = tpi * g, t = t0 + lane;
        const bool have = lane < tpi && t < sc.ntiles;
        const uint64_t frow = (uint64_t)f * sc.ntiles;
        uint8_t *rec = flat ? sc.pixraw + (uint64_t)f * sc.pixraw_stride : out + rec_off[f];
        const uint32_t nnz = rp.level == 1 ? sc.frame_nnz[f] : 0;
        const uint32_t npk = rp.level == 1 ? packed_bytes(nnz, d) : 0;
        uint64_t bitmap_pos = 0, pix_pos = 0;
        uint32_t cb = 0;
        if (!flat) {
            if (rp.emit == EMIT_RAW) { bitmap_pos = rp.level == 1 ? 8 : 4; pix_pos = bitmap_pos + sc.nb; }
            else { cb = bhdr + sc.frame_cbytes[f] + ff.end; bitmap_pos = rp.level == 1 ? 16 : 8; pix_pos = bitmap_pos + cb; }
        }
        if (g == 0 && lane == 0 && !flat) record_fixed_fields(sc, rp, f, rec, bitmap_pos, pix_pos, cb, npk, ff, skip_pix, lz4f_hdr_bitmap, lz4f_hdr_pix);
        uint8_t *pdst = rec + pix_pos;

        uint32_t word = 0, bsz = 0, bdst = 0, cnt = 0, rn = 0, rdst = 0, rs = 0xFFFFFFFFu, ps0 = 0, flags = 0, blo = 0;
        AdlerAcc ad{0u, 0u};
        if (have && rp.emit != EMIT_RAW && (!flat || (sc.comb == COMB_BEHIND_BLOCK && pixp))) word = sc.blk_size[frow + t];
        if (have && !flat) {
            if (rp.emit == EMIT_RAW) {
                const uint64_t b0 = (uint64_t)t * TILE_BM;
                bsz = (uint32_t)min((uint64_t)TILE_BM, sc.nb - b0);
                bdst = (uint32_t)(bitmap_pos + b0);
            } else {
                bsz = word;
                const uint32_t boff = bhdr + sc.blk_off[frow + t];
                bdst = (uint32_t)bitmap_pos + boff;
                if (rp.emit == EMIT_BLOSC) store_u32_le(rec + bitmap_pos + 16 + 4 * (uint64_t)t, boff);
            }
        }
        if (have && pixp) {
            cnt = sc.tile_cnt[frow + t];
            if (cnt) {
                const ResidGeom q = resid_geom(sc.tile_off[frow + t], cnt, d);
                ps0 = q.ps0;
                if (ADLER) blo = q.b_lo;
                if (sc.comb) {
                    const uint32_t ro16 = sc.comb == COMB_AT_BLK_SLOT ? (uint32_t)BLK_SLOT / 16 : (word + 15) >> 4, r16 = (cnt * d + 127) >> 7;
                    if (16 * (ro16 + r16) <= sc.blk_stride) rs = 16 * ro16;
                }
                if (q.n && !plain_pos && ((uint64_t)q.b_lo >> ff.chunk_shift) != (((uint64_t)q.b_lo + q.n - 1) >> ff.chunk_shift)) flags = 1u << 31;
                else rn = q.n;
                rdst = (uint32_t)(pix_pos + (plain_pos ? (uint64_t)q.b_lo : stored_pos(ff, q.b_lo)));
            }
        }
        uint32_t ext_cnt = 0, ext_first = 0;
        if (BITS && pixp && t0 + tpi < sc.ntiles) {
            ext_cnt = sc.tile_cnt[frow + t0 + tpi];
            if (ext_cnt)
                ext_first = *reinterpret_cast<const uint32_t *>(residual_src(sc, frow + t0 + tpi, sc.comb == COMB_BEHIND_BLOCK ? sc.blk_size[frow + t0 + tpi] : 0u, ext_cnt, d));
        }
        const uint8_t *slot = rp.emit == EMIT_RAW ? sc.bitmap + (uint64_t)f * sc.nb_stride + (uint64_t)t0 * TILE_BM : sc.blk_slots + (frow + t0) * sc.blk_stride;
        const uint32_t slot_stride = rp.emit == EMIT_RAW ? (uint32_t)TILE_BM : sc.blk_stride;
        const uint8_t *rslot = pix_base + (frow + t0) * sc.pix_slot_bytes;

        const uint32_t nb16 = (bsz + 15) >> 4, tot = nb16 + ((rn + 15) >> 4);
        const uint32_t incl = wave_incl_scan(tot), cum = incl - tot, T = wave_last(incl);
        const uint32_t packed = bsz | (ps0 << 10) | (rn << 13) | flags;
        for (uint32_t i0 = 0; 64u * i0 < T; i0 += U) {
            u32x4 x[U];
            uint32_t e[U], dsto[U], meta[U];
            uint32_t spos[ADLER ? U : 1];
#pragma unroll
            for (int u = 0; u < U; ++u) {
                const uint32_t P = 64u * (i0 + u) + lane;
                uint32_t k = 0;
#pragma unroll
                for (uint32_t step = 32; step; step >>= 1) {
                    const uint32_t c = lane_get(cum, k + step);
                    if (c <= P) k += step;
                }
                const uint32_t ck = lane_get(cum, k), pk = lane_get(packed, k), bd = lane_get(bdst, k), rd = lane_get(rdst, k), rsk = lane_get(rs, k);
                const uint32_t blk = ADLER ? lane_get(blo, k) : 0u;
                const uint32_t bsz_k = pk & 1023u, ps0_k = (pk >> 10) & 7u, rn_k = (pk >> 13) & 0x7FFFu;
                const uint32_t idx = P - ck, nbk = (bsz_k + 15) >> 4;
                const bool isb = idx < nbk;
                const uint32_t j = isb ? idx : idx - nbk;
                const uint32_t left = (isb ? bsz_k : rn_k) - 16u * j;
                const bool act = P < T;
                const uint8_t *src = isb ? slot + (uint64_t)k * slot_stride + 16u * j
                                         : (rsk == 0xFFFFFFFFu ? rslot + (uint64_t)k * sc.pix_slot_bytes : slot + (uint64_t)k * slot_stride + rsk) + 16u * j;
                dsto[u] = (isb ? bd : rd) + 16u * j;
                meta[u] = act ? (min(left, 16u) | ((isb ? 0u : ps0_k) << 8)) : 0u;
                if (ADLER) spos[u] = isb ? 0xFFFFFFFFu : blk + 16u * j;
                x[u] = u32x4{0u, 0u, 0u, 0u};
                e[u] = 0;
                if (act) {
                    x[u] = *reinterpret_cast<const u32x4 *>(src);
                    if (BITS && !isb && ps0_k) e[u] = *reinterpret_cast<const uint32_t *>(src + 16);
                }
            }
#pragma unroll
            for (int u = 0; u < U; ++u)
                if (meta[u] & 0xFFu) {
                    const u32x4 y = shift_piece<BITS>(x[u], e[u], meta[u] >> 8);
                    put_piece(rec + dsto[u], y, meta[u] & 0xFFu);
                    if (ADLER && spos[u] != 0xFFFFFFFFu) adler_piece(ad, y, meta[u] & 0xFFu, spos[u]);
                }
        }
        if (pixp) {
        ResidGeom q{0u, 0u, 0u, 0u};
        if (cnt) q = resid_geom(sc.tile_off[frow + t], cnt, d);
        for (uint64_t m = __builtin_amdgcn_ballot_w64((packed >> 31) != 0); m; m &= m - 1) {
            const uint32_t k = (uint32_t)__builtin_ctzll(m);
            const uint32_t n = lane_get(q.n, k), p0 = lane_get(q.ps0, k), b0 = lane_get(q.b_lo, k), rsk = lane_get(rs, k);
            const uint32_t *s32 = reinterpret_cast<const uint32_t *>(rsk == 0xFFFFFFFFu ? rslot + (uint64_t)k * sc.pix_slot_bytes : slot + (uint64_t)k * slot_stride + rsk);
            for (uint32_t i = lane; i < n; i += 64) {
                const uint32_t qb = 8 * i + p0;
                const uint32_t v = __builtin_amdgcn_alignbit(s32[(qb >> 5) + 1], s32[qb >> 5], qb & 31u) & 0xFFu;
                pdst[stored_pos(ff, (uint64_t)b0 + i)] = (uint8_t)v;
                if (ADLER) adler_byte(ad, v, b0 + i);
            }
        }
        if (BITS) {

        const uint32_t fin_avail = q.avail, fin_q = 8 * q.n + q.ps0, fin_b = q.b_lo + q.n;
        const uint8_t *psrc = rs == 0xFFFFFFFFu ? rslot + (uint64_t)lane * sc.pix_slot_bytes : slot + (uint64_t)lane * slot_stride + rs;
        const uint32_t first = cnt ? *reinterpret_cast<const uint32_t *>(psrc) : 0u;
        uint32_t byte = 0, got = 8;
        if (fin_avail) {
            byte = (*reinterpret_cast<const u32_u *>(psrc + (fin_q >> 3)) >> (fin_q & 7u)) & ((1u << fin_avail) - 1u);
            got = fin_avail;
        }
        const uint64_t nonempty = __builtin_amdgcn_ballot_w64(cnt != 0);
        uint32_t cur = lane;
        while (__builtin_amdgcn_ballot_w64(got < 8 && cur < 64) != 0) {
            const uint64_t higher = cur >= 63 ? 0ull : nonempty & (~0ull << (cur + 1));
            const uint32_t nxt = higher ? (uint32_t)__builtin_ctzll(higher) : 64u;
            const uint32_t cc = lane_get(cnt, nxt & 63u), fd = lane_get(first, nxt & 63u);
            if (got < 8 && cur < 64) {
                const bool in = nxt < 64;
                const uint32_t c2 = in ? cc : ext_cnt, f2 = in ? fd : ext_first;
                if (in || c2) {
                    const uint32_t take = min(8u - got, c2 * d);
                    byte |= (f2 & ((1u << take) - 1u)) << got;
                    got += take;
                    cur = nxt;
                } else cur = 65;
            }
        }
        if (got < 8) {
            uint32_t tt = cur == 65 ? (t0 + tpi - 1 < sc.ntiles ? sc.tile_next[frow + t0 + tpi - 1] : sc.ntiles) : (t0 + tpi < sc.ntiles ? sc.tile_next[frow + t0 + tpi] : sc.ntiles);
            while (tt < sc.ntiles) {
                const uint32_t cc = sc.tile_cnt[frow + tt];
                const uint32_t fd = *reinterpret_cast<const uint32_t *>(residual_src(sc, frow + tt, sc.comb == COMB_BEHIND_BLOCK ? sc.blk_size[frow + tt] : 0u, cc, d));
                const uint32_t take = min(8u - got, cc * d);
                byte |= (fd & ((1u << take) - 1u)) << got;
                got += take;
                if (got >= 8) break;
                tt = sc.tile_next[frow + tt];
            }
        }
        if (fin_avail) {
            pdst[plain_pos ? (uint64_t)fin_b : stored_pos(ff, fin_b)] = (uint8_t)byte;
            if (ADLER) adler_byte(ad, byte & 0xFFu, fin_b);
        }
        }
        }
        if (ADLER && !flat) {
            const uint32_t aux = have ? sc.blk_aux[frow + t] : 0u;
            const uint32_t tA0 = wave_last(wave_incl_scan(aux & 0xFFFFu)), tW0 = wave_last(wave_incl_scan(aux >> 16));
            const uint32_t tA1 = wave_last(wave_incl_scan(ad.A % ADLER_P)), tW1 = wave_last(wave_incl_scan(ad.W));
            if (lane == 0) {
                uint32_t *acc = sc.zl_acc + 8 * (uint64_t)f;
                if (tA0 | tW0) {
                    __hip_atomic_fetch_add(&acc[0], tA0 % ADLER_P, __ATOMIC_RELAXED, __HIP_MEMORY_SCOPE_AGENT);
                    __hip_atomic_fetch_add(&acc[1], tW0 % ADLER_P, __ATOMIC_RELAXED, __HIP_MEMORY_SCOPE_AGENT);
                }
                if (tA1 | tW1) {
                    __hip_atomic_fetch_add(&acc[2], tA1 % ADLER_P, __ATOMIC_RELAXED, __HIP_MEMORY_SCOPE_AGENT);
                    __hip_atomic_fetch_add(&acc[3], tW1 % ADLER_P, __ATOMIC_RELAXED, __HIP_MEMORY_SCOPE_AGENT);
                }
            }
        }
    }
}

__global__ __launch_bounds__(64) void k_zlib_finish(GatherArgs sc, RecordParams rp, uint8_t *__restrict__ out, const uint64_t *__restrict__ rec_off, uint32_t B)
{
    const uint32_t f = blockIdx.x * 64 + threadIdx.x;
    if (f >= B || sc.status->code != 0) return;
    const FrameFmt ff = frame_fmt(rp.emit);
    const uint32_t *acc = sc.zl_acc + 8 * (uint64_t)f;
    uint8_t *rec = out + rec_off[f];
    const uint32_t cb = bitmap_hdr(ff, rp.emit, sc.ntiles) + sc.frame_cbytes[f] + ff.end, bitmap_pos = rp.level == 1 ? 16u : 8u;
    store_u32_be(rec + bitmap_pos + cb - 4, adler_from_sums(sc.nb, acc[0], acc[1]));
    if (rp.level == 1 && rp.pix_mode != PIX_MODE_SKIP) {
        const uint32_t npk = packed_bytes(sc.frame_nnz[f], rp.depth);
        store_u32_be(rec + bitmap_pos + cb + stored_size(ff, npk) - 4, adler_from_sums(npk, acc[2], acc[3]));
    }
}


void launch_gather(const Scratch &sc, const RecordParams &rp, uint32_t B, uint8_t *out, const uint64_t *rec_off, uint32_t hdr_bitmap, uint32_t hdr_pix,
                   uint32_t batch_seq, hipStream_t s)
{
    uint32_t tpi = 64;
    while (tpi > 8 && (uint64_t)B * ((sc.ntiles + tpi - 1) / tpi) < 1024) tpi >>= 1;
    const uint32_t gpf = (sc.ntiles + tpi - 1) / tpi, nitems = gpf * B, wgs = nitems;
    const GatherArgs ga{sc.blk_slots, sc.bitmap, sc.pix_slots, sc.blk_size, sc.blk_off, sc.tile_cnt, sc.tile_off, sc.tile_next, sc.frame_nnz, sc.frame_cbytes,
                        sc.frame_pbytes, sc.blk_aux, sc.zl_acc, sc.pixraw, sc.status, sc.first_err, sc.nb, sc.nb_stride, sc.pixraw_stride, sc.ntiles, sc.blk_stride, sc.pix_slot_bytes, sc.comb};
    const bool bits = rp.level == 1 && rp.depth % 8 != 0;
    if (rp.emit == EMIT_DEFLATE) {
        if (bits) hipLaunchKernelGGL((k_gather<true, GATHER_UB - 1, true>), dim3(wgs), dim3(64), 0, s, ga, rp, out, rec_off, hdr_bitmap, hdr_pix, batch_seq, gpf, nitems, tpi);
        else hipLaunchKernelGGL((k_gather<false, GATHER_U, true>), dim3(wgs), dim3(64), 0, s, ga, rp, out, rec_off, hdr_bitmap, hdr_pix, batch_seq, gpf, nitems, tpi);
        if (rp.pix_mode != PIX_MODE_FLAT) hipLaunchKernelGGL(k_zlib_finish, dim3((B + 63) / 64), dim3(64), 0, s, ga, rp, out, rec_off, B);
    } else if (bits)
        hipLaunchKernelGGL((k_gather<true, GATHER_UB, false>), dim3(wgs), dim3(64), 0, s, ga, rp, out, rec_off, hdr_bitmap, hdr_pix, batch_seq, gpf, nitems, tpi);
    else
        hipLaunchKernelGGL((k_gather<false, GATHER_U, false>), dim3(wgs), dim3(64), 0, s, ga, rp, out, rec_off, hdr_bitmap, hdr_pix, batch_seq, gpf, nitems, tpi);
}

}
```

### pyrecode_amd/csrc/rc_launch.h

```cpp
#pragma once
#include <hip/hip_runtime.h>
#include <stdint.h>

#include "../../include/recode_hip.h"
#include "rc_device.h"

namespace rc {

struct ZstdModel;
struct DeflateModel;
struct InfStream;

constexpr uint32_t COMB_OFF = 0u;
constexpr uint32_t COMB_BEHIND_BLOCK = 1u;
constexpr uint32_t COMB_AT_BLK_SLOT = 2u;

struct Scratch {
    uint64_t N = 0;
    uint32_t ntiles = 0;
    uint64_t nb = 0;
    uint64_t nb_stride = 0;
    uint32_t max_batch = 0;
    bool guarded_loads = false;
    uint16_t *thr = nullptr;
    uint8_t *bitmap = nullptr;
    uint16_t *pix_slots = nullptr;
    uint32_t pix_slot_bytes = SLOT_PX * 2;
    uint32_t *tile_cnt = nullptr;
    uint32_t *tile_off = nullptr;
    uint32_t *tile_next = nullptr;
    uint8_t *blk_slots = nullptr;
    uint32_t blk_stride = BLK_SLOT;
    uint32_t comb = COMB_OFF;
    uint32_t *blk_size = nullptr;
    uint32_t *blk_aux = nullptr;
    uint32_t *zl_acc = nullptr;
    uint32_t *blk_off = nullptr;
    uint32_t *frame_nnz = nullptr;
    uint32_t *frame_cbytes = nullptr;
    uint32_t *scan_part = nullptr;
    BatchStatus *status = nullptr;
    BatchStatus *first_err = nullptr;
    uint8_t *pixraw = nullptr;
    uint64_t pixraw_stride = 0;
    uint8_t *pix_chunks = nullptr;
    uint32_t *chunk_size = nullptr;
    uint32_t *chunk_off = nullptr;
    uint32_t *frame_pbytes = nullptr;
    uint32_t nchunk_max = 0;
    const ZstdModel *zm_model = nullptr;
    const void *zm_lit_code = nullptr;
    uint32_t zm_valid = 0, zm_budget = 0, zm_seq_bits = 12;
    u32x2 *l2_node = nullptr;
    uint64_t l2_ids_per_frame = 0;
    uint16_t *l2_base = nullptr;
    uint32_t *chunk_aux = nullptr;
    const DeflateModel *dz_model = nullptr;
};

constexpr uint32_t EMIT_RAW = 0u;
constexpr uint32_t EMIT_ZSTD = 1u;
constexpr uint32_t EMIT_LZ4 = 2u;
constexpr uint32_t EMIT_BLOSC = 8u;
constexpr uint32_t EMIT_DEFLATE = 0x100u;
static_assert(EMIT_ZSTD == RC_SCHEME_ZSTD && EMIT_LZ4 == RC_SCHEME_LZ4 && EMIT_BLOSC == RC_SCHEME_BLOSC_LZ4 && EMIT_DEFLATE == RC_SCHEME_ZLIB_DEVICE,
              "rc_ctx_create assigns emit = compression_scheme");

constexpr int CODEC_NONE = 0;
constexpr int CODEC_ZSTD_FAST = 1;
constexpr int CODEC_LZ4_RUNS = 2;
constexpr int CODEC_ZSTD_MODELLED = 3;
constexpr int CODEC_LZ4_EVENTS = 4;
constexpr int CODEC_DEFLATE = 5;
constexpr int CODEC_BLOSC = 8;

constexpr uint32_t PIX_MODE_STORED = 0u;
constexpr uint32_t PIX_MODE_FLAT = 1u;
constexpr uint32_t PIX_MODE_SKIP = 2u;

struct RecordParams {
    uint32_t level;
    uint32_t emit;
    uint32_t depth;
    uint32_t packed_slots;
    uint32_t first_frame_id;
    uint64_t frame_bytes;
    uint32_t pix_mode = PIX_MODE_STORED;
};

void launch_threshold(const void *dark, int64_t eps, uint64_t N, uint16_t *thr, hipStream_t s, uint32_t src_bytes = 2);
void launch_reduce(const Scratch &sc, const void *frames, uint32_t B, uint32_t level, uint32_t codec, bool keep_bitmap,
                   uint32_t depth, hipStream_t s, hipStream_t s_tail = nullptr, uint32_t src_bytes = 2);
void launch_threshold32(const uint32_t *dark, int64_t eps, uint64_t N, uint32_t *thr, hipStream_t s);
void launch_reduce32(const Scratch &sc, const uint32_t *frames, const uint32_t *thr32, uint32_t B, uint32_t level, uint32_t depth, hipStream_t s,
                     uint32_t codec = CODEC_NONE, bool keep_bitmap = true);
void launch_l2(const Scratch &sc, uint32_t B, uint32_t nx, uint32_t use_sum, uint32_t depth, hipStream_t s);
void launch_scans(const Scratch &sc, uint32_t B, bool with_counts, bool with_blocks, hipStream_t s);
void launch_layout(const Scratch &sc, const RecordParams &rp, uint32_t B, uint64_t out_cap, uint64_t *rec_off,
                   uint32_t *md, hipStream_t s);
void launch_assemble(const Scratch &sc, const RecordParams &rp, uint32_t B, uint8_t *out, const uint64_t *rec_off,
                     uint32_t batch_seq, hipStream_t s);
void launch_gather(const Scratch &sc, const RecordParams &rp, uint32_t B, uint8_t *out, const uint64_t *rec_off, uint32_t hdr_bitmap, uint32_t hdr_pix,
                   uint32_t batch_seq, hipStream_t s);
enum ValueStage : uint32_t {
    VALUES_NONE = 0,
    VALUES_ZSTD_HUFF,
    VALUES_DEFLATE_HUFF,
};
inline ValueStage value_stage_of(uint32_t emit, uint32_t clevel, uint32_t level)
{
    if (level == 1 && emit == EMIT_ZSTD && clevel != 0) return VALUES_ZSTD_HUFF;
    return level == 1 && emit == EMIT_DEFLATE && clevel >= 2 ? VALUES_DEFLATE_HUFF : VALUES_NONE;
}
constexpr uint32_t PIX_CHUNK = 1008, PIX_SLOT = 1024, PD_CHUNK = 1u << 15, PD_SLOT = PD_CHUNK + 32;
struct ValueGeom { uint32_t chunk, slot; };
inline ValueGeom value_geom(ValueStage kind) { return kind == VALUES_DEFLATE_HUFF ? ValueGeom{PD_CHUNK, PD_SLOT} : ValueGeom{PIX_CHUNK, PIX_SLOT}; }
void launch_values_encode(ValueStage kind, const Scratch &sc, uint32_t B, uint32_t depth, hipStream_t s);
void launch_values_scan(ValueStage kind, const Scratch &sc, uint32_t B, uint32_t depth, hipStream_t s);
void launch_values_gather(ValueStage kind, const Scratch &sc, uint32_t B, uint32_t depth, uint32_t level1_hdr, uint8_t *out, const uint64_t *rec_off,
                          hipStream_t s);
void launch_pd_hist(const Scratch &sc, uint32_t B, uint32_t depth, uint32_t *hist_dev, hipStream_t s);
struct Lz4Block { uint64_t src_off; uint32_t size; uint32_t raw; };
void launch_lz4_encode_buffer(const Scratch &sc, hipStream_t s, bool events = false);
void launch_lz4_encode_rows(const Scratch &sc, uint32_t B, hipStream_t s, bool events);
void launch_lz4f_gather(const Scratch &sc, uint32_t hdr3, uint8_t *out, hipStream_t s);
void launch_lz4_decode(const uint8_t *src, const Lz4Block *blks, uint32_t nblk, uint32_t *sizes, const uint64_t *dst_off,
                       uint8_t *dst, uint64_t cap, int linked, int *err, hipStream_t s, uint32_t max_stored = 0);
uint32_t lz4f_descriptor(uint8_t bd);
void launch_blosc_encode_blocks(const Scratch &sc, uint32_t B, hipStream_t s);
void launch_blosc_gather(const Scratch &sc, uint8_t *out, hipStream_t s);
void launch_blosc_unshuffle(const uint8_t *in, uint8_t *out, uint64_t nbytes, uint32_t blocksize, uint32_t typesize,
                            uint32_t shuffle, hipStream_t s);
void launch_zstd_encode_blocks(const Scratch &sc, uint32_t B, const void *tables_dev, hipStream_t s);
void launch_zstd_tokenize_rows(const Scratch &sc, uint32_t B, hipStream_t s);
void launch_zstd_fse(const Scratch &sc, uint32_t B, const void *tables_dev, bool fitted, hipStream_t s);
void launch_zstd_sample(const Scratch &sc, uint32_t B, bool with_pix, uint32_t depth, void *sample_dev, hipStream_t s);
size_t zstd_model_bytes();
size_t zstd_sample_bytes();
void zstd_model_from_sample(const void *sample_host, void *model_host, uint32_t speed_permille = 0);
void launch_zstd_gather(const Scratch &sc, uint8_t *out, hipStream_t s);
size_t zstd_tables_bytes();
void zstd_tables_host(void *dst);

template <class S>
__host__ __device__ inline const uint8_t *residual_src(const S &sc, uint64_t ft, uint32_t bn, uint32_t cnt, uint32_t d)
{
    if (sc.comb) {
        const uint32_t ro16 = sc.comb == COMB_AT_BLK_SLOT ? (uint32_t)BLK_SLOT / 16 : (bn + 15) >> 4, r16 = (cnt * d + 127) >> 7;
        if (16 * (ro16 + r16) <= sc.blk_stride) return sc.blk_slots + ft * sc.blk_stride + 16 * ro16;
    }
    return reinterpret_cast<const uint8_t *>(sc.pix_slots) + ft * sc.pix_slot_bytes;
}

void launch_inflate(const uint8_t *data, const InfStream *streams, uint32_t n_map, uint32_t n_val, uint32_t map_cap_max, uint32_t map_units_max,
                    uint32_t val_cap_max, uint32_t val_units_max, uint32_t *cand_pos, uint32_t *ncand, uint32_t *link, uint32_t *unit_cand,
                    uint8_t *out, int *err, hipStream_t s);

void launch_roi_components(const void *frames, const void *thr, uint64_t N, uint32_t nx, uint32_t n, uint32_t first_frame_id, uint32_t gap,
                           uint32_t x0, uint32_t y0, uint32_t w, uint32_t h, uint32_t *counts, hipStream_t s, uint32_t src_bytes = 2);

constexpr uint32_t CALIB_LDS_MAX_FRAMES = 512;
void launch_calib_stats(const uint16_t *stack, uint32_t n, uint64_t N, uint32_t n_stats, float *median, float *sdev, int32_t *range2, hipStream_t s);
void launch_calib_hist(const uint16_t *frames, uint32_t n_stats, uint64_t N, const float *median, const double *edges, uint32_t n_bins,
                       uint64_t *counts, hipStream_t s);
void launch_calib_top(const uint16_t *stack, uint32_t n, uint64_t N, const float *median, uint32_t k, float *acc, uint64_t *n_undefined, hipStream_t s);
}
```

### pyrecode_amd/csrc/rc_reduce.hip

```cpp
#include <cstddef>
#include <cstdlib>
#include <type_traits>

#include "rc_launch.h"
#include "rc_values.h"
#include "rc_pack.h"
#ifdef RC_PHASE_TIMING
__device__ unsigned long long g_phase[16];
#define RC_LZ4_PHASE 1
#endif
#include "rc_lz4_block.h"
#include "rc_zstd_wave.h"
#include "rc_deflate_block.h"

namespace rc {

#ifdef RC_PHASE_TIMING
#define RC_PHASE_BEGIN unsigned long long ph_t_ = __builtin_amdgcn_s_memtime(); unsigned long long ph_a_[8] = {};
#define RC_PHASE(i) do { const unsigned long long ph_n_ = __builtin_amdgcn_s_memtime(); ph_a_[i] = ph_n_ - ph_t_; ph_t_ = ph_n_; \
        if ((i) == 6 && lane_id() == 0 && (blockIdx.x & 63u) == 0) { for (int q_ = 0; q_ < 7; ++q_) atomicAdd(&g_phase[q_], ph_a_[q_]); atomicAdd(&g_phase[7], 1ull); } } while (0)
#else
#define RC_PHASE_BEGIN
#define RC_PHASE(i) do { } while (0)
#endif
constexpr int REDUCE_BZ = 4;

__device__ __forceinline__ uint32_t pk_sub_sat_u16(uint32_t a, uint32_t b)
{
    uint32_t r;
    asm("v_pk_sub_u16 %0, %1, %2 clamp" : "=v"(r) : "v"(a), "v"(b));
    return r;
}
__device__ __forceinline__ uint32_t pk_add_u16(uint32_t a, uint32_t b)
{
    uint32_t r;
    asm("v_pk_add_u16 %0, %1, %2" : "=v"(r) : "v"(a), "v"(b));
    return r;
}
__device__ __forceinline__ uint32_t pk_min_u16(uint32_t a, uint32_t b)
{
    uint32_t r;
    asm("v_pk_min_u16 %0, %1, %2" : "=v"(r) : "v"(a), "v"(b));
    return r;
}

__global__ void k_threshold(const uint16_t *__restrict__ dark, uint32_t eps16, uint64_t N, uint16_t *__restrict__ thr)
{
    uint64_t i = (uint64_t)blockIdx.x * blockDim.x + threadIdx.x;
    const uint64_t stride = (uint64_t)gridDim.x * blockDim.x;
    for (; i < N; i += stride) thr[i] = (uint16_t)(dark[i] + eps16);
}

__global__ void k_threshold8(const uint8_t *__restrict__ dark, uint32_t eps8, uint64_t N, uint16_t *__restrict__ thr)
{
    uint64_t i = (uint64_t)blockIdx.x * blockDim.x + threadIdx.x;
    const uint64_t stride = (uint64_t)gridDim.x * blockDim.x;
    for (; i < N; i += stride) thr[i] = (uint16_t)(uint8_t)(dark[i] + eps8);
}

void launch_threshold(const void *dark, int64_t eps, uint64_t N, uint16_t *thr, hipStream_t s, uint32_t src_bytes)
{
    uint32_t blocks = (uint32_t)((N + 255) / 256);
    if (blocks > 4096) blocks = 4096;
    if (src_bytes == 1)
        hipLaunchKernelGGL(k_threshold8, dim3(blocks), dim3(256), 0, s, static_cast<const uint8_t *>(dark), (uint32_t)((uint64_t)eps & 0xFF), N, thr);
    else
        hipLaunchKernelGGL(k_threshold, dim3(blocks), dim3(256), 0, s, static_cast<const uint16_t *>(dark), (uint32_t)((uint64_t)eps & 0xFFFF), N, thr);
}

template <int SB> struct Src;
template <> struct Src<2> { typedef uint16_t T; typedef u32x4 X; };
template <> struct Src<1> { typedef uint8_t T; typedef u32x2 X; };
__device__ __forceinline__ u32x4 widen8(const u32x2 &v)
{
    return u32x4{__builtin_amdgcn_perm(0u, v[0], 0x0C010C00u), __builtin_amdgcn_perm(0u, v[0], 0x0C030C02u),
                 __builtin_amdgcn_perm(0u, v[1], 0x0C010C00u), __builtin_amdgcn_perm(0u, v[1], 0x0C030C02u)};
}
__device__ __forceinline__ u32x4 widen8(const u32x4 &v) { return v; }

template <bool ALIGNED, bool STREAM, int SB = 2>
__device__ __forceinline__ typename Src<SB>::X load8(const typename Src<SB>::T *__restrict__ base, uint64_t px0, uint64_t N, uint32_t fill)
{
    typedef typename Src<SB>::X X;
    constexpr int PER = 4 / SB;
    if (ALIGNED || px0 + 8 <= N) {
        if (px0 < N) {
            typedef X XU __attribute__((aligned(SB)));
            const XU *p = reinterpret_cast<const XU *>(base + px0);
            return STREAM ? __builtin_nontemporal_load(p) : *p;
        }
    }
    X v;
#pragma unroll
    for (int j = 0; j < 8 / PER; ++j) {
        uint32_t w = 0;
#pragma unroll
        for (int e = 0; e < PER; ++e) {
            const uint64_t k = px0 + (uint64_t)(PER * j + e);
            const uint32_t val = (!ALIGNED && k < N) ? (uint32_t)base[k] : fill;
            w |= val << (8 * SB * e);
        }
        v[j] = w;
    }
    return v;
}

struct Pending {
    bool valid;
    uint64_t ft;
    uint32_t f;
    uint32_t cnt;
    uint32_t csize;
    uint32_t staged;
    u32x2 own;
    uint64_t cown;
    uint32_t aux;
    bool last;
    uint32_t depth;
    uint16_t *buf;
};

__device__ __forceinline__ void vm_issue_loads(u32x4 (&x)[R], const uint16_t *lane_ptr)
{
    const uint8_t *p0 = reinterpret_cast<const uint8_t *>(lane_ptr), *p1 = p0 + 4096;
    asm volatile("global_load_dwordx4 %0, %4, off nt\n\t"
                 "global_load_dwordx4 %1, %4, off offset:1024 nt\n\t"
                 "global_load_dwordx4 %2, %4, off offset:2048 nt\n\t"
                 "global_load_dwordx4 %3, %4, off offset:3072 nt"
                 : "=&v"(x[0]), "=&v"(x[1]), "=&v"(x[2]), "=&v"(x[3]) : "v"(p0) : "memory");
    asm volatile("global_load_dwordx4 %0, %4, off nt\n\t"
                 "global_load_dwordx4 %1, %4, off offset:1024 nt\n\t"
                 "global_load_dwordx4 %2, %4, off offset:2048 nt\n\t"
                 "global_load_dwordx4 %3, %4, off offset:3072 nt"
                 : "=&v"(x[4]), "=&v"(x[5]), "=&v"(x[6]), "=&v"(x[7]) : "v"(p1) : "memory");
}
__device__ __forceinline__ void vm_issue_loads(u32x2 (&x)[R], const uint8_t *lane_ptr)
{
    asm volatile("global_load_dwordx2 %0, %8, off nt\n\t"
                 "global_load_dwordx2 %1, %8, off offset:512 nt\n\t"
                 "global_load_dwordx2 %2, %8, off offset:1024 nt\n\t"
                 "global_load_dwordx2 %3, %8, off offset:1536 nt\n\t"
                 "global_load_dwordx2 %4, %8, off offset:2048 nt\n\t"
                 "global_load_dwordx2 %5, %8, off offset:2560 nt\n\t"
                 "global_load_dwordx2 %6, %8, off offset:3072 nt\n\t"
                 "global_load_dwordx2 %7, %8, off offset:3584 nt"
                 : "=&v"(x[0]), "=&v"(x[1]), "=&v"(x[2]), "=&v"(x[3]), "=&v"(x[4]), "=&v"(x[5]), "=&v"(x[6]), "=&v"(x[7]) : "v"(lane_ptr) : "memory");
}
__device__ __forceinline__ void vm_issue_load1(u32x4 &xr, const uint16_t *lane_ptr, int r)
{
    const uint8_t *p = reinterpret_cast<const uint8_t *>(lane_ptr) + (r >= 4 ? 4096 : 0);
    switch (r & 3) {
    case 0: asm volatile("global_load_dwordx4 %0, %1, off nt" : "=&v"(xr) : "v"(p) : "memory"); break;
    case 1: asm volatile("global_load_dwordx4 %0, %1, off offset:1024 nt" : "=&v"(xr) : "v"(p) : "memory"); break;
    case 2: asm volatile("global_load_dwordx4 %0, %1, off offset:2048 nt" : "=&v"(xr) : "v"(p) : "memory"); break;
    default: asm volatile("global_load_dwordx4 %0, %1, off offset:3072 nt" : "=&v"(xr) : "v"(p) : "memory"); break;
    }
}
__device__ __forceinline__ void vm_issue_load1(u32x2 &xr, const uint8_t *p, int r)
{
    switch (r) {
    case 0: asm volatile("global_load_dwordx2 %0, %1, off nt" : "=&v"(xr) : "v"(p) : "memory"); break;
    case 1: asm volatile("global_load_dwordx2 %0, %1, off offset:512 nt" : "=&v"(xr) : "v"(p) : "memory"); break;
    case 2: asm volatile("global_load_dwordx2 %0, %1, off offset:1024 nt" : "=&v"(xr) : "v"(p) : "memory"); break;
    case 3: asm volatile("global_load_dwordx2 %0, %1, off offset:1536 nt" : "=&v"(xr) : "v"(p) : "memory"); break;
    case 4: asm volatile("global_load_dwordx2 %0, %1, off offset:2048 nt" : "=&v"(xr) : "v"(p) : "memory"); break;
    case 5: asm volatile("global_load_dwordx2 %0, %1, off offset:2560 nt" : "=&v"(xr) : "v"(p) : "memory"); break;
    case 6: asm volatile("global_load_dwordx2 %0, %1, off offset:3072 nt" : "=&v"(xr) : "v"(p) : "memory"); break;
    default: asm volatile("global_load_dwordx2 %0, %1, off offset:3584 nt" : "=&v"(xr) : "v"(p) : "memory"); break;
    }
}
template <class X>
__device__ __forceinline__ void vm_wait_loads(uint32_t later, X (&x)[R])
{
    switch (later) {
    case 1: asm volatile("s_waitcnt vmcnt(1)" ::: "memory"); break;
    case 2: asm volatile("s_waitcnt vmcnt(2)" ::: "memory"); break;
    case 3: asm volatile("s_waitcnt vmcnt(3)" ::: "memory"); break;
    case 4: asm volatile("s_waitcnt vmcnt(4)" ::: "memory"); break;
    case 5: asm volatile("s_waitcnt vmcnt(5)" ::: "memory"); break;
    case 6: asm volatile("s_waitcnt vmcnt(6)" ::: "memory"); break;
    case 7: asm volatile("s_waitcnt vmcnt(7)" ::: "memory"); break;
    case 8: asm volatile("s_waitcnt vmcnt(8)" ::: "memory"); break;
    default: asm volatile("s_waitcnt vmcnt(0)" ::: "memory"); break;
    }
    asm volatile("" : "+v"(x[0]), "+v"(x[1]), "+v"(x[2]), "+v"(x[3]), "+v"(x[4]), "+v"(x[5]), "+v"(x[6]), "+v"(x[7]) :: "memory");
}

constexpr int STAGE_CAP = 256;
struct __attribute__((aligned(16))) WaveStage {
    uint16_t val[TILE_PX];
    uint16_t out[STAGE_CAP];
};
static_assert(offsetof(WaveStage, out) == sizeof(uint16_t) * TILE_PX && STAGE_CAP >= 64, "compact_dense_in_place: `out` lies right behind `val`, an entry per lane");

__device__ __forceinline__ uint32_t store_lines2(const uint8_t *s0, uint8_t *d0, uint32_t q0, const uint8_t *s1, uint8_t *d1, uint32_t q1)
{
    const uint32_t total = q0 + q1, lane = (uint32_t)lane_id();
    for (uint32_t base = 0; base < total; base += 64) {
        const uint32_t i = base + lane;
        if (i < total) {
            const bool second = i >= q0;
            const uint32_t j = second ? i - q0 : i;
            const u32x4 v = *reinterpret_cast<const u32x4 *>((second ? s1 : s0) + 16 * j);
            *reinterpret_cast<u32x4 *>((second ? d1 : d0) + 16 * j) = v;
        }
    }
    return (total + 63u) >> 6;
}

template <bool LEVEL1, int CODEC, bool KEEP_BITMAP>
__device__ __forceinline__ uint32_t flush_pending(const Pending &p, uint32_t tile, uint32_t n_blk, uint8_t *__restrict__ bitmap,
                                                  uint64_t nb_stride, uint16_t *__restrict__ pix_slots, uint32_t *__restrict__ tile_cnt,
                                                  uint8_t *__restrict__ blk_slots, uint32_t *__restrict__ blk_size, Lz4Lds *lz,
                                                  const WaveStage *st, uint32_t blk_stride, uint32_t comb, uint32_t *__restrict__ blk_aux)
{
    if (!p.valid) return 0;
    const int lane = lane_id();
    uint32_t nst = 0;
    const uint8_t *s0 = nullptr, *s1 = nullptr;
    uint8_t *d0 = nullptr, *d1 = nullptr;
    uint32_t q0 = 0, q1 = 0, bsz = 0;
    if (LEVEL1) {
        s0 = reinterpret_cast<const uint8_t *>(p.buf);
        d0 = reinterpret_cast<uint8_t *>(pix_slots + p.ft * SLOT_PX);
        q0 = ((((p.cnt * p.depth + 31) >> 5) + 31u) & ~31u) >> 2;
    }
    if (CODEC == CODEC_LZ4_RUNS || CODEC == CODEC_LZ4_EVENTS || CODEC == CODEC_BLOSC) {
        const uint64_t bytes = CODEC != CODEC_BLOSC ? ((uint64_t)p.own[0] | ((uint64_t)p.own[1] << 32)) : p.cown;
        bsz = lz4_stage_slot(bytes, n_blk, p.csize, *lz, CODEC == CODEC_BLOSC);
    }
    if (CODEC == CODEC_ZSTD_FAST || CODEC == CODEC_ZSTD_MODELLED) {
        (void)zstd_stage_slot(n_blk, p.last, p.staged, *lz);
        bsz = p.staged ? p.staged : 4u;
    }
    if (CODEC == CODEC_DEFLATE) bsz = p.csize;
    if (CODEC) {
        s1 = lz->out;
        d1 = blk_slots + p.ft * blk_stride;
        q1 = min((((bsz + 3) >> 2) + 31u) & ~31u, (uint32_t)BLK_SLOT / 4) >> 2;
    }
    if (LEVEL1 && CODEC && comb) {
        const uint32_t ro16 = comb == COMB_AT_BLK_SLOT ? (uint32_t)BLK_SLOT / 16 : (bsz + 15) >> 4, r16 = (p.cnt * p.depth + 127) >> 7;
        if (16 * (ro16 + r16) <= blk_stride) {
            d0 = d1 + 16 * ro16;
            if (comb == COMB_AT_BLK_SLOT) q0 = (r16 + 7u) & ~7u;
            else { q1 = ro16; q0 = ((ro16 + r16 + 7u) & ~7u) - ro16; }
        }
    }
    if (q0 + q1) nst += store_lines2(s0, d0, q0, s1, d1, q1);
    if (KEEP_BITMAP) {
        *reinterpret_cast<u32x2 *>(bitmap + (uint64_t)p.f * nb_stride + (uint64_t)tile * TILE_BM + lane * 8) = p.own;
        nst += 1;
    }
    if (LEVEL1 || CODEC) {
        const uint32_t word = CODEC == CODEC_ZSTD_FAST || CODEC == CODEC_ZSTD_MODELLED ? p.csize : bsz;
        if (LEVEL1 && CODEC == CODEC_DEFLATE) {
            if (lane < 3) *(lane == 0 ? &tile_cnt[p.ft] : (lane == 1 ? &blk_size[p.ft] : &blk_aux[p.ft])) = lane == 0 ? p.cnt : (lane == 1 ? word : p.aux);
        } else if (LEVEL1 && CODEC) {
            if (lane < 2) *(lane == 0 ? &tile_cnt[p.ft] : &blk_size[p.ft]) = lane == 0 ? p.cnt : word;
        } else if (LEVEL1) {
            if (lane == 0) tile_cnt[p.ft] = p.cnt;
        } else if (CODEC == CODEC_DEFLATE) {
            if (lane < 2) *(lane == 0 ? &blk_size[p.ft] : &blk_aux[p.ft]) = lane == 0 ? word : p.aux;
        } else {
            if (lane == 0) blk_size[p.ft] = word;
        }
        nst += 1;
    }
    return (uint32_t)__builtin_amdgcn_readfirstlane((int)nst);
}

__device__ __forceinline__ void compact_dense_in_place(WaveStage *st, const uint8_t *bm)
{
    const int lane = lane_id();
    uint32_t inc[3], tot[3];
#pragma unroll
    for (int g = 0; g < 3; ++g) {
        uint32_t pk = 0;
#pragma unroll
        for (int k = 0; k < 3; ++k)
            if (3 * g + k < R) pk |= (uint32_t)__builtin_popcount((uint32_t)bm[(3 * g + k) * 64 + lane]) << (10 * k);
        inc[g] = wave_incl_scan(pk);
        tot[g] = wave_last(inc[g]);
    }
    uint32_t base = 0;
#pragma unroll
    for (int r = 0; r < R; ++r) {
        const uint32_t m = bm[r * 64 + lane];
        const uint32_t dst = base + ((inc[r / 3] >> (10 * (r % 3))) & 0x3FFu) - (uint32_t)__builtin_popcount(m);
        const u32x4 v = (reinterpret_cast<const u32x4 *>(st->val) + lane)[r * 64];
        __builtin_amdgcn_wave_barrier();
        uint16_t *const vo = st->val;
#pragma unroll
        for (int j = 0; j < 8; ++j) {
            const uint32_t a = (m >> j) & 1u ? dst + (uint32_t)__builtin_popcount(m & ((1u << j) - 1u)) : (uint32_t)TILE_PX + (uint32_t)lane;
            vo[a] = (uint16_t)(v[j >> 1] >> (16 * (j & 1)));
        }
        __builtin_amdgcn_wave_barrier();
        base += (tot[r / 3] >> (10 * (r % 3))) & 0x3FFu;
    }
}

constexpr uint32_t FUSED12_CAP = (uint32_t)(STAGE_CAP * 16 / 12);
__device__ __forceinline__ void compact_pack12(WaveStage *st, const u32x2 &own, uint32_t exc, uint32_t cnt)
{
    const int lane = lane_id();
    uint32_t *out32 = reinterpret_cast<uint32_t *>(st->out);
    *reinterpret_cast<u32x2 *>(out32 + 2 * lane) = u32x2{0u, 0u};
    __builtin_amdgcn_wave_barrier();
    const uint16_t *mine = st->val + 64 * lane;
    uint64_t q = (uint64_t)own[0] | ((uint64_t)own[1] << 32);
    uint32_t left = cnt, P = 12u * exc;
    do {
        uint32_t x[4];
#pragma unroll
        for (int k = 0; k < 4; ++k) {
            const uint32_t i = q ? (uint32_t)__builtin_ctzll(q) : 0u;
            q &= q - 1;
            x[k] = mine[i];
        }
#pragma unroll
        for (int k = 0; k < 4; ++k) x[k] = (uint32_t)k < left ? (x[k] & 0xFFFu) : 0u;
        const uint32_t lo = x[0] | (x[1] << 12) | (x[2] << 24), hi = (x[2] >> 8) | (x[3] << 4);
        const uint32_t w = P >> 5, sh = P & 31u;
        const uint64_t a = (uint64_t)lo << sh, b = (uint64_t)hi << sh;
        const uint32_t d0 = (uint32_t)a, d1 = (uint32_t)(a >> 32) | (uint32_t)b, d2 = (uint32_t)(b >> 32);
        if (left) {
            __hip_atomic_fetch_or(&out32[w], d0, __ATOMIC_RELAXED, __HIP_MEMORY_SCOPE_WAVEFRONT);
            if (d1) __hip_atomic_fetch_or(&out32[w + 1], d1, __ATOMIC_RELAXED, __HIP_MEMORY_SCOPE_WAVEFRONT);
            if (d2) __hip_atomic_fetch_or(&out32[w + 2], d2, __ATOMIC_RELAXED, __HIP_MEMORY_SCOPE_WAVEFRONT);
        }
        left = left > 4u ? left - 4u : 0u;
        P += 48u;
    } while (__builtin_amdgcn_ballot_w64(left != 0) != 0);
    __builtin_amdgcn_wave_barrier();
}

template <bool ALIGNED, bool ASMLOAD, bool LEVEL1, int CODEC, bool KEEP_BITMAP, bool RAWVAL, int SB>
__device__ __forceinline__ void reduce_one_frame(typename Src<SB>::X (&x)[R], const typename Src<SB>::T *__restrict__ cur, const typename Src<SB>::T *__restrict__ next, bool have_next,
                                                 const u32x4 (&t)[R], uint64_t lane_px0, uint64_t N, bool full,
                                                 uint32_t f, uint32_t tile, uint64_t ft, uint32_t n_blk, uint8_t *__restrict__ bitmap,
                                                 uint64_t nb_stride, uint16_t *__restrict__ pix_slots,
                                                 uint32_t *__restrict__ tile_cnt, uint8_t *__restrict__ blk_slots,
                                                 uint32_t *__restrict__ blk_size, Lz4Lds *s_lz, uint8_t *s_bm, WaveStage *st,
                                                 Pending &pend, uint32_t &stores_behind, const ZmParams &zp, uint32_t blk_stride, uint32_t comb,
                                                 uint32_t *__restrict__ blk_aux)
{
    const int lane = lane_id();
    RC_PHASE_BEGIN
    if (ASMLOAD) vm_wait_loads(stores_behind, x);
    else if (ALIGNED && full) {
        typedef typename Src<SB>::X XU __attribute__((aligned(SB)));
        const XU *p = reinterpret_cast<const XU *>(cur + lane_px0);
#pragma unroll
        for (int r = 0; r < R; ++r) x[r] = __builtin_nontemporal_load(p + r * (GROUP_PX / 8));
    } else {
#pragma unroll
        for (int r = 0; r < R; ++r) x[r] = load8<ALIGNED, true, SB>(cur, lane_px0 + (uint64_t)r * GROUP_PX, N, 0);
    }
    RC_PHASE(0);
    uint32_t m8[R];
#pragma unroll
    for (int r = 0; r < R; ++r) {
        const u32x4 tt = t[r];
        u32x4 xv = widen8(x[r]);
#pragma unroll
        for (int k = 0; k < 4; ++k) xv[k] = pk_sub_sat_u16(xv[k], tt[k]);
        const uint32_t one = 0x00010001u;
        uint32_t M = 0;
#pragma unroll
        for (int k = 3; k >= 0; --k)
            M = __builtin_amdgcn_udot2(__builtin_bit_cast(u16x2, pk_min_u16(xv[k], one)),
                                       __builtin_bit_cast(u16x2, (uint32_t)((1u << (2 * k)) | (2u << (2 * k + 16)))), M, false);
        m8[r] = M;
        if (LEVEL1) {
            u32x4 v = xv;
            if (RAWVAL) {
#pragma unroll
                for (int k = 0; k < 4; ++k) v[k] = pk_add_u16(v[k], tt[k]);
            }
            (reinterpret_cast<u32x4 *>(st->val) + lane)[r * 64] = v;
        }
        if (ASMLOAD && have_next) vm_issue_load1(x[r], next + lane_px0, r);
    }
    RC_PHASE(1);
    RC_PHASE(2);
    pend.valid = true;
    pend.ft = ft;
    pend.f = f;
    pend.cnt = 0;
    pend.csize = 0;
    pend.buf = st->out;
    if (LEVEL1 || KEEP_BITMAP || CODEC) {
        uint8_t *bm = CODEC ? s_lz->raw : s_bm;
#pragma unroll
        for (int r = 0; r < R; ++r) bm[r * 64 + lane] = (uint8_t)m8[r];
        __builtin_amdgcn_wave_barrier();
        pend.own = *reinterpret_cast<const u32x2 *>(&bm[lane * 8]);
    }
    RC_PHASE(3);
    if (LEVEL1) {
        const uint32_t cnt = (uint32_t)__builtin_popcount(pend.own[0]) + (uint32_t)__builtin_popcount(pend.own[1]);
        const uint32_t inc = wave_incl_scan(cnt);
        const uint32_t wave_total = wave_last(inc);
        bool packed = false;
        if (pend.depth == 12 && wave_total <= FUSED12_CAP) {
            if (wave_total) compact_pack12(st, pend.own, inc - cnt, cnt);
            packed = true;
        } else if (wave_total <= (uint32_t)STAGE_CAP) {
#pragma unroll
            for (int h = 0; h < 2; ++h) {
                const uint16_t *mine = st->val + 64 * lane + 32 * h;
                uint32_t qh = pend.own[h];
                uint32_t o = inc - cnt + (h ? (uint32_t)__builtin_popcount(pend.own[0]) : 0u);
                while (qh) {
                    const uint32_t i0 = (uint32_t)__builtin_ctz(qh);
                    qh &= qh - 1;
                    const bool two = qh != 0;
                    const uint32_t i1 = two ? (uint32_t)__builtin_ctz(qh) : i0;
                    qh &= qh - 1;
                    const uint16_t v0 = mine[i0], v1 = mine[i1];
                    st->out[o] = v0;
                    if (two) st->out[o + 1] = v1;
                    o += 2;
                }
            }
        } else {
            pend.buf = st->val;
            __builtin_amdgcn_wave_barrier();
            compact_dense_in_place(st, CODEC ? s_lz->raw : s_bm);
        }
        __builtin_amdgcn_wave_barrier();
        pend.cnt = wave_total;
        if (!packed && pend.depth < 16 && wave_total) pack_stage(pend.buf, wave_total, pend.depth);
    }
    RC_PHASE(4);
    if (CODEC == CODEC_LZ4_RUNS) {
        const uint64_t bytes = (uint64_t)pend.own[0] | ((uint64_t)pend.own[1] << 32);
        pend.csize = lz4_encode_block<false>(bytes, n_blk, *s_lz);
    }
    if (CODEC == CODEC_LZ4_EVENTS) {
        const uint64_t bytes = (uint64_t)pend.own[0] | ((uint64_t)pend.own[1] << 32);
        pend.csize = lz4_encode_block<true>(bytes, n_blk, *s_lz);
    }
    if (CODEC == CODEC_ZSTD_FAST) {
        const uint64_t bytes = (uint64_t)pend.own[0] | ((uint64_t)pend.own[1] << 32);
        pend.csize = zstd_tokenize_block(bytes, n_blk, pend.last, *s_lz, pend.staged);
    }
    if (CODEC == CODEC_ZSTD_MODELLED) {
        const uint64_t bytes = (uint64_t)pend.own[0] | ((uint64_t)pend.own[1] << 32);
        pend.csize = zstd_tokenize_block_m(bytes, n_blk, pend.last, *s_lz, pend.staged, zp);
    }
    if (CODEC == CODEC_DEFLATE) {
        const uint64_t bytes = (uint64_t)pend.own[0] | ((uint64_t)pend.own[1] << 32);
        pend.aux = deflate_adler_word(bytes, tile);
        pend.csize = deflate_encode_block<true>(bytes, n_blk, pend.last, *s_lz);
    }
    if (CODEC == CODEC_BLOSC) {
        const uint64_t bytes = (uint64_t)pend.own[0] | ((uint64_t)pend.own[1] << 32);
        pend.cown = bitshuffle_block(bytes, n_blk, *s_lz);
        pend.csize = lz4_encode_block(pend.cown, n_blk, *s_lz);
    }
    RC_PHASE(5);
    stores_behind = flush_pending<LEVEL1, CODEC, KEEP_BITMAP>(pend, tile, n_blk, bitmap, nb_stride, pix_slots, tile_cnt, blk_slots, blk_size, s_lz, st, blk_stride, comb, blk_aux);
    pend.valid = false;
    RC_PHASE(6);
}

template <int RWAVES, int BZ, bool ALIGNED, bool ASMLOAD, bool LEVEL1, int CODEC, bool KEEP_BITMAP, bool RAWVAL, int SB>
__global__ __launch_bounds__(64 * RWAVES) __attribute__((amdgpu_waves_per_eu((ALIGNED && ASMLOAD) ? ((RWAVES == 4 && LEVEL1) ? 3 : 4) : 1))) void k_reduce_tiles(const typename Src<SB>::T *__restrict__ frames,
                                                       const uint16_t *__restrict__ thr, uint64_t N, uint32_t ntiles,
                                                       uint32_t tile0, uint32_t tile_end,
                                                       uint32_t B, uint32_t ngroups, uint64_t nb,
                                                       uint8_t *__restrict__ bitmap, uint64_t nb_stride,
                                                       uint16_t *__restrict__ pix_slots, uint32_t *__restrict__ tile_cnt,
                                                       uint8_t *__restrict__ blk_slots, uint32_t *__restrict__ blk_size, uint32_t depth,
                                                       BatchStatus *__restrict__ status, ZmParams zm, uint32_t blk_stride, uint32_t comb,
                                                       uint32_t *__restrict__ blk_aux)
{
    if (blockIdx.x == 0 && threadIdx.x == 0) { status->code = 0; status->frame = 0; status->total = 0; }
    __shared__ uint16_t s_code[CODEC == CODEC_ZSTD_MODELLED ? 256 : 2];
    if (CODEC == CODEC_ZSTD_MODELLED) {
        for (uint32_t i = threadIdx.x; i < 128; i += 64 * RWAVES) reinterpret_cast<uint32_t *>(s_code)[i] = reinterpret_cast<const uint32_t *>(zm.lit_code)[i];
        __syncthreads();
        zm.lit_code = s_code;
    }
    __shared__ Lz4Lds s_lz[CODEC ? RWAVES : 1];
    __shared__ __attribute__((aligned(16))) uint8_t s_bm[CODEC ? 1 : RWAVES][CODEC ? 16 : TILE_BM];
    __shared__ WaveStage s_stage[LEVEL1 ? RWAVES : 1];

    const uint32_t xcd = blockIdx.x & 7u, j = blockIdx.x >> 3;
    const uint32_t grp = j % ngroups;
    const uint32_t tblock = (j / ngroups) * 8u + xcd;
    const int lane = lane_id();
    const int w = __builtin_amdgcn_readfirstlane((int)(threadIdx.x >> 6));
    const uint32_t tile = tile0 + tblock * RWAVES + w;
    if (tile >= tile_end) return;
    const uint64_t lane_px0 = (uint64_t)tile * TILE_PX + (uint64_t)lane * 8;
    const uint32_t f0 = grp * BZ;
    if (f0 >= B) return;
    const bool full = (uint64_t)(tile + 1) * TILE_PX <= N;

    typename Src<SB>::X xa[R];
    if (ASMLOAD) vm_issue_loads(xa, frames + (uint64_t)f0 * N + lane_px0);
    u32x4 t[R];
#pragma unroll
    for (int r = 0; r < R; ++r) t[r] = load8<ALIGNED, false, 2>(thr, lane_px0 + (uint64_t)r * GROUP_PX, N, 0xFFFF);
    const uint32_t n_blk = (uint32_t)min((uint64_t)TILE_BM, nb - (uint64_t)tile * TILE_BM);
    Lz4Lds *lz = &s_lz[CODEC ? w : 0];
    uint8_t *bm = s_bm[CODEC ? 0 : w];
    WaveStage *st = &s_stage[LEVEL1 ? w : 0];
    Pending pend;
    pend.valid = false;
    pend.ft = 0; pend.f = 0; pend.cnt = 0; pend.csize = 0; pend.own = u32x2{0u, 0u};
    pend.staged = 0; pend.last = tile + 1 == ntiles; pend.cown = 0; pend.aux = 0;
    pend.depth = (LEVEL1 && !RAWVAL) ? depth : 16u;
    pend.buf = nullptr;

    uint32_t stores_behind = 0;
#pragma unroll 1
    for (int z = 0; z < BZ; ++z) {
        const uint32_t f = f0 + z;
        if (f >= B) break;
        const bool nxt = z + 1 < BZ && f + 1 < B;
        reduce_one_frame<ALIGNED, ASMLOAD, LEVEL1, CODEC, KEEP_BITMAP, RAWVAL, SB>(xa, frames + (uint64_t)f * N, frames + (uint64_t)(f + 1) * N, nxt, t,
                                                                             lane_px0, N, full, f, tile, (uint64_t)f * ntiles + tile, n_blk,
                                                                             bitmap, nb_stride, pix_slots, tile_cnt, blk_slots,
                                                                             blk_size, lz, bm, st, pend, stores_behind, zm, blk_stride, comb, blk_aux);
        if (!nxt) break;
    }
    flush_pending<LEVEL1, CODEC, KEEP_BITMAP>(pend, tile, n_blk, bitmap, nb_stride, pix_slots, tile_cnt, blk_slots, blk_size, lz, st, blk_stride, comb, blk_aux);
}

template <int BZ, bool AL, bool L1, int CODEC, bool KEEP, bool RAW, int SB>
static void launch_reduce_t(const Scratch &sc, const typename Src<SB>::T *frames, uint32_t B, uint32_t depth, hipStream_t s, hipStream_t s_tail)
{
    const uint32_t ngroups = (B + BZ - 1) / BZ;
    const uint32_t nfull = AL ? (uint32_t)(sc.N / TILE_PX) : 0u;
    const ZmParams zm{reinterpret_cast<const uint16_t *>(sc.zm_lit_code), sc.zm_valid, sc.zm_budget, sc.zm_seq_bits};
    const uint32_t comb = (L1 && !RAW && CODEC) ? sc.comb : COMB_OFF;
    const bool three = L1 && !RAW && CODEC != CODEC_DEFLATE &&
                       (CODEC == CODEC_LZ4_RUNS || CODEC == CODEC_LZ4_EVENTS || sc.ntiles > 8192 || (CODEC == CODEC_ZSTD_MODELLED && (sc.zm_valid & ZM_LITS_ONLY)));
    auto go = [&](auto rw) {
        constexpr int RW = decltype(rw)::value;
        auto grid_for = [&](uint32_t nt) { return (((nt + RW - 1) / RW + 7) / 8) * 8 * ngroups; };
        if (nfull)
            hipLaunchKernelGGL((k_reduce_tiles<RW, BZ, AL, AL, L1, CODEC, KEEP, RAW, SB>), dim3(grid_for(nfull)), dim3(64 * RW), 0, s, frames, sc.thr, sc.N,
                               sc.ntiles, 0u, nfull, B, ngroups, sc.nb, sc.bitmap, sc.nb_stride, sc.pix_slots, sc.tile_cnt, sc.blk_slots,
                               sc.blk_size, depth, sc.status, zm, sc.blk_stride, comb, sc.blk_aux);
        if (nfull < sc.ntiles) {
            if (AL && sc.N % 8 != 0)
                hipLaunchKernelGGL((k_reduce_tiles<RW, BZ, false, false, L1, CODEC, KEEP, RAW, SB>), dim3(grid_for(sc.ntiles - nfull)), dim3(64 * RW), 0, nfull ? s_tail : s, frames,
                                   sc.thr, sc.N, sc.ntiles, nfull, sc.ntiles, B, ngroups, sc.nb, sc.bitmap, sc.nb_stride, sc.pix_slots, sc.tile_cnt,
                                   sc.blk_slots, sc.blk_size, depth, sc.status, zm, sc.blk_stride, comb, sc.blk_aux);
            else
                hipLaunchKernelGGL((k_reduce_tiles<RW, BZ, AL, false, L1, CODEC, KEEP, RAW, SB>), dim3(grid_for(sc.ntiles - nfull)), dim3(64 * RW), 0, nfull ? s_tail : s, frames,
                                   sc.thr, sc.N, sc.ntiles, nfull, sc.ntiles, B, ngroups, sc.nb, sc.bitmap, sc.nb_stride, sc.pix_slots, sc.tile_cnt,
                                   sc.blk_slots, sc.blk_size, depth, sc.status, zm, sc.blk_stride, comb, sc.blk_aux);
        }
    };
    if constexpr (SB == 2) {
        if (three) { go(int_c<3>{}); return; }
    }
    go(int_c<4>{});
}
template <int BZ, bool AL, bool L1, bool RAW, int SB>
static void launch_reduce_c(const Scratch &sc, const typename Src<SB>::T *frames, uint32_t B, uint32_t codec, bool keep, uint32_t depth, hipStream_t s, hipStream_t s_tail)
{
    if (RAW) keep = true;
#define RC_CODEC(C)                                                                                      \
    if (codec == C) {                                                                                    \
        if (keep) launch_reduce_t<BZ, AL, L1, C, true, RAW, SB>(sc, frames, B, depth, s, s_tail);        \
        else if (!RAW) launch_reduce_t<BZ, AL, L1, C, false, false, SB>(sc, frames, B, depth, s, s_tail); \
        return;                                                                                          \
    }
    RC_CODEC(CODEC_LZ4_RUNS) RC_CODEC(CODEC_LZ4_EVENTS) RC_CODEC(CODEC_ZSTD_FAST) RC_CODEC(CODEC_ZSTD_MODELLED) RC_CODEC(CODEC_BLOSC) RC_CODEC(CODEC_DEFLATE)
#undef RC_CODEC
    launch_reduce_t<BZ, AL, L1, CODEC_NONE, true, RAW, SB>(sc, frames, B, depth, s, s_tail);
}
template <int BZ, bool AL, int SB>
static void launch_reduce_a(const Scratch &sc, const typename Src<SB>::T *frames, uint32_t B, uint32_t level, uint32_t codec, bool keep,
                            uint32_t depth, hipStream_t s, hipStream_t s_tail)
{
    if (level == 2) launch_reduce_c<BZ, AL, true, true, SB>(sc, frames, B, codec, keep, depth, s, s_tail);
    else if (level == 1) launch_reduce_c<BZ, AL, true, false, SB>(sc, frames, B, codec, keep, depth, s, s_tail);
    else launch_reduce_c<BZ, AL, false, false, SB>(sc, frames, B, codec, keep, depth, s, s_tail);
}
#ifdef RC_PHASE_TIMING
extern "C" __attribute__((visibility("default"))) int rc_debug_phases(unsigned long long *out16)
{
    unsigned long long z[16] = {};
    if (hipDeviceSynchronize() != hipSuccess) return -1;
    if (hipMemcpyFromSymbol(out16, HIP_SYMBOL(g_phase), sizeof z) != hipSuccess) return -1;
    if (hipMemcpyToSymbol(HIP_SYMBOL(g_phase), z, sizeof z) != hipSuccess) return -1;
    return 0;
}
#endif
void launch_reduce(const Scratch &sc, const void *frames, uint32_t B, uint32_t level, uint32_t codec, bool keep_bitmap,
                   uint32_t depth, hipStream_t s, hipStream_t s_tail, uint32_t src_bytes)
{
    if (depth == 0 || depth > 16) depth = 16;
    if (!s_tail) s_tail = s;
    const bool aligned = !sc.guarded_loads;
    if (src_bytes == 1) {
        const uint8_t *f8 = static_cast<const uint8_t *>(frames);
        if (aligned) launch_reduce_a<REDUCE_BZ, true, 1>(sc, f8, B, level, codec, keep_bitmap, depth, s, s_tail);
        else launch_reduce_a<REDUCE_BZ, false, 1>(sc, f8, B, level, codec, keep_bitmap, depth, s, s_tail);
        return;
    }
    const uint16_t *f16 = static_cast<const uint16_t *>(frames);
    if (aligned) launch_reduce_a<REDUCE_BZ, true, 2>(sc, f16, B, level, codec, keep_bitmap, depth, s, s_tail);
    else launch_reduce_a<REDUCE_BZ, false, 2>(sc, f16, B, level, codec, keep_bitmap, depth, s, s_tail);
}

constexpr int SCAN_T = 256, SCAN_W = SCAN_T / 64;

__device__ __forceinline__ uint32_t scan_block_excl(uint32_t v, uint32_t *sm, uint32_t *total)
{
    const int w = threadIdx.x >> 6;
    const uint32_t inc = wave_incl_scan(v);
    if (lane_id() == 63) sm[w] = inc;
    __syncthreads();
    uint32_t base = 0, tot = 0;
#pragma unroll
    for (int i = 0; i < SCAN_W; ++i) {
        const uint32_t x = sm[i];
        if (i < w) base += x;
        tot += x;
    }
    __syncthreads();
    *total = tot;
    return base + inc - v;
}

template <int SCAN_I>
__device__ __forceinline__ void scan_row(uint32_t *__restrict__ row, uint32_t *__restrict__ orow, uint32_t n,
                                         uint32_t *__restrict__ total, uint32_t *sm, const uint32_t *adj = nullptr)
{
    uint32_t carry = 0;
    for (uint32_t t0 = 0; t0 < n; t0 += SCAN_T * SCAN_I) {
        const uint32_t t = t0 + threadIdx.x * SCAN_I;
        uint32_t v[SCAN_I], s = 0;
#pragma unroll
        for (int k = 0; k < SCAN_I; ++k) {
            v[k] = t + k < n ? row[t + k] : 0;
            if (adj) {
                v[k] &= 0xFFFFu;
                if (t + k == adj[0]) v[k] += adj[1];
                if (t + k == adj[2]) v[k] += adj[3];
                if (t + k < n) row[t + k] = v[k];
            }
            s += v[k];
        }
        uint32_t tot;
        uint32_t ex = carry + scan_block_excl(s, sm, &tot);
#pragma unroll
        for (int k = 0; k < SCAN_I; ++k) {
            if (t + k < n) orow[t + k] = ex;
            ex += v[k];
        }
        carry += tot;
    }
    if (threadIdx.x == 0) *total = carry;
}

__device__ __forceinline__ void zstd_rewrite_defs(const uint32_t *__restrict__ row, uint8_t *__restrict__ slots, uint32_t stride,
                                                  const uint8_t *__restrict__ tree, uint32_t tl, const uint8_t *__restrict__ sdesc, uint32_t sl,
                                                  uint32_t t_tree, uint32_t t_seq, uint32_t which, uint8_t *s_img, uint32_t *s_pos)
{
    for (int pass = 0; pass < 2; ++pass) {
        const uint32_t t = pass == 0 ? t_tree : t_seq;
        if (t == 0xFFFFFFFFu || (pass == 1 && t == t_tree) || !((which >> pass) & 1u)) continue;
        const uint32_t a_tl = pass == 0 ? tl : 0u, a_sl = (pass == 1 || t_seq == t_tree) ? sl : 0u;
        uint8_t *slot = slots + (uint64_t)t * stride;
        const uint32_t size = row[t] & 0xFFFFu;
        __syncthreads();
        for (uint32_t i = threadIdx.x; i < (size + 3) / 4; i += blockDim.x)
            reinterpret_cast<uint32_t *>(s_img)[i] = reinterpret_cast<const uint32_t *>(slot)[i];
        __syncthreads();
        if (threadIdx.x == 0) { uint32_t q; (void)zm_block_needs(s_img, &q); *s_pos = q; }
        __syncthreads();
        const uint32_t pos = *s_pos;
        for (uint32_t i = threadIdx.x; i < size + a_tl + a_sl; i += blockDim.x)
            slot[i] = zm_defs_byte(s_img, pos, tree, a_tl, sdesc, a_sl, i);
    }
    __syncthreads();
}

__device__ __forceinline__ void zstd_place_defs(const uint32_t *__restrict__ row, uint32_t n, uint8_t *__restrict__ slots, uint32_t stride,
                                                const uint8_t *__restrict__ tree, uint32_t tree_len, const uint8_t *__restrict__ sdesc,
                                                uint32_t sdesc_len, uint32_t *adj)
{
    __shared__ uint32_t s_first[2];
    __shared__ uint32_t s_pos;
    __shared__ __attribute__((aligned(16))) uint8_t s_img[PIX_SLOT + 16];
    if (threadIdx.x < 2) s_first[threadIdx.x] = 0xFFFFFFFFu;
    __syncthreads();
    const uint32_t w0 = row[0];
    const bool both0 = (w0 & ZW_TREE) && ((w0 & ZW_SEQ) || !sdesc_len);
    if (both0) {
        if (threadIdx.x == 0) { s_first[0] = 0; if (sdesc_len) s_first[1] = 0; }
    } else {
        uint32_t mt = 0xFFFFFFFFu, mq = 0xFFFFFFFFu;
        for (uint32_t t = threadIdx.x; t < n; t += SCAN_T) {
            const uint32_t w = row[t];
            if ((w & ZW_TREE) && t < mt) mt = t;
            if ((w & ZW_SEQ) && t < mq) mq = t;
        }
        if (mt != 0xFFFFFFFFu) atomicMin(&s_first[0], mt);
        if (mq != 0xFFFFFFFFu) atomicMin(&s_first[1], mq);
    }
    __syncthreads();
    const uint32_t t_tree = s_first[0], t_seq = s_first[1];
    const uint32_t tl = t_tree != 0xFFFFFFFFu ? tree_len : 0u, sl = t_seq != 0xFFFFFFFFu ? sdesc_len : 0u;
    if (threadIdx.x == 0) { adj[0] = t_tree; adj[1] = tl; adj[2] = t_seq; adj[3] = sl; }
    zstd_rewrite_defs(row, slots, stride, tree, tl, sdesc, sl, t_tree, t_seq, 3u, s_img, &s_pos);
}

__global__ __launch_bounds__(SCAN_T) void k_pix_scan(Scratch sc, uint32_t depth)
{
    __shared__ uint32_t sm[SCAN_W];
    __shared__ uint32_t s_adj[4];
    const uint32_t f = blockIdx.x;
    const ZstdModel *M = sc.zm_model;
    const uint32_t npk = packed_bytes(sc.frame_nnz[f], depth);
    const uint32_t nch = value_chunks(npk, PIX_CHUNK);
    uint32_t *row = sc.chunk_size + (uint64_t)f * sc.nchunk_max;
    zstd_place_defs(row, nch, sc.pix_chunks + (uint64_t)f * sc.nchunk_max * PIX_SLOT, PIX_SLOT, M->pix_desc, M->pix_desc_len, nullptr, 0, s_adj);
    scan_row<16>(row, sc.chunk_off + (uint64_t)f * sc.nchunk_max, nch, sc.frame_pbytes + f, sm, s_adj);
}
void launch_pix_scan(const Scratch &sc, uint32_t B, uint32_t depth, hipStream_t s)
{
    hipLaunchKernelGGL(k_pix_scan, dim3(B), dim3(SCAN_T), 0, s, sc, depth);
}

template <int SCAN_I>
__global__ __launch_bounds__(SCAN_T) void k_scan_frames(Scratch sc, int with_counts, int with_blocks)
{
    __shared__ uint32_t sm[SCAN_W];
    __shared__ uint32_t s_carry;
    __shared__ uint32_t s_adj[4];
    const uint32_t f = blockIdx.x, n = sc.ntiles;
    const uint64_t fr = (uint64_t)f * n;
    if (with_blocks) {
        if (sc.zm_model) {
            const ZstdModel *M = sc.zm_model;
            zstd_place_defs(sc.blk_size + fr, n, sc.blk_slots + fr * sc.blk_stride, sc.blk_stride, M->lit_desc, M->lit_desc_len, M->seq_desc,
                            M->seq_desc_len, s_adj);
        }
        scan_row<SCAN_I>(sc.blk_size + fr, sc.blk_off + fr, n, sc.frame_cbytes + f, sm, sc.zm_model ? s_adj : nullptr);
    }
    if (!with_counts) return;
    uint32_t *row = sc.tile_cnt + fr;
    scan_row<SCAN_I>(row, sc.tile_off + fr, n, sc.frame_nnz + f, sm);
    uint32_t *nrow = sc.tile_next + fr;
    if (threadIdx.x == 0) s_carry = n;
    __syncthreads();
    const uint32_t per_round = SCAN_T * SCAN_I;
    const uint32_t nrounds = (n + per_round - 1) / per_round;
    for (uint32_t c = nrounds; c-- > 0;) {
        const uint32_t t = c * per_round + threadIdx.x * SCAN_I;
        uint32_t v[SCAN_I];
        uint32_t first = 0xFFFFFFFFu;
#pragma unroll
        for (int k = SCAN_I - 1; k >= 0; --k) {
            v[k] = t + k < n ? row[t + k] : 0;
            if (v[k]) first = t + k;
        }
        uint32_t m = first;
#pragma unroll
        for (int d = 1; d < 64; d <<= 1) {
            const uint32_t y = __shfl_down(m, d);
            if (lane_id() + d < 64) m = min(m, y);
        }
        const int w = threadIdx.x >> 6;
        if (lane_id() == 0) sm[w] = m;
        __syncthreads();
        uint32_t right = s_carry;
#pragma unroll
        for (int i = SCAN_W - 1; i >= 0; --i)
            if (i > w) right = min(right, sm[i]);
        uint32_t excl = __shfl_down(m, 1);
        if (lane_id() == 63) excl = 0xFFFFFFFFu;
        uint32_t nxt = min(excl, right);
#pragma unroll
        for (int k = SCAN_I - 1; k >= 0; --k) {
            if (t + k < n) nrow[t + k] = nxt;
            if (v[k]) nxt = t + k;
        }
        __syncthreads();
        if (threadIdx.x == 0) {
            uint32_t all = s_carry;
#pragma unroll
            for (int i = 0; i < SCAN_W; ++i) all = min(all, sm[i]);
            s_carry = all;
        }
        __syncthreads();
    }
}

constexpr int SEG_I = 16, SEG = SCAN_T * SEG_I;
struct ScanPart { uint32_t blk_sum, cnt_sum, first_nonempty, first_tree, first_seq, pad[3]; };

__global__ __launch_bounds__(SCAN_T) void k_scan_seg(Scratch sc, int with_counts, int with_blocks)
{
    __shared__ uint32_t sm[SCAN_W];
    __shared__ uint32_t s_min[3];
    const uint32_t seg = blockIdx.x, f = blockIdx.y, n = sc.ntiles, nseg = gridDim.x;
    const uint64_t fr = (uint64_t)f * n;
    const uint32_t t = seg * SEG + threadIdx.x * SEG_I;
    ScanPart *part = reinterpret_cast<ScanPart *>(sc.scan_part) + (uint64_t)f * nseg + seg;
    if (threadIdx.x < 3) s_min[threadIdx.x] = 0xFFFFFFFFu;
    __syncthreads();
    uint32_t blk_sum = 0, cnt_sum = 0;
    if (with_blocks) {
        uint32_t *row = sc.blk_size + fr, *orow = sc.blk_off + fr;
        const bool zm = sc.zm_model != nullptr;
        uint32_t v[SEG_I], sum = 0, mt = 0xFFFFFFFFu, mq = 0xFFFFFFFFu;
#pragma unroll
        for (int k = 0; k < SEG_I; ++k) {
            const uint32_t w = t + k < n ? row[t + k] : 0;
            if (zm) {
                if ((w & ZW_TREE) && mt == 0xFFFFFFFFu) mt = t + k;
                if ((w & ZW_SEQ) && mq == 0xFFFFFFFFu) mq = t + k;
                v[k] = w & 0xFFFFu;
                if (t + k < n) row[t + k] = v[k];
            } else v[k] = w;
            sum += v[k];
        }
        if (mt != 0xFFFFFFFFu) atomicMin(&s_min[1], mt);
        if (mq != 0xFFFFFFFFu) atomicMin(&s_min[2], mq);
        uint32_t ex = scan_block_excl(sum, sm, &blk_sum);
#pragma unroll
        for (int k = 0; k < SEG_I; ++k) {
            if (t + k < n) orow[t + k] = ex;
            ex += v[k];
        }
    }
    if (with_counts) {
        const uint32_t *row = sc.tile_cnt + fr;
        uint32_t *orow = sc.tile_off + fr, *nrow = sc.tile_next + fr;
        uint32_t v[SEG_I], sum = 0, first = 0xFFFFFFFFu;
#pragma unroll
        for (int k = SEG_I - 1; k >= 0; --k) {
            v[k] = t + k < n ? row[t + k] : 0;
            if (v[k]) first = t + k;
            sum += v[k];
        }
        uint32_t ex = scan_block_excl(sum, sm, &cnt_sum);
#pragma unroll
        for (int k = 0; k < SEG_I; ++k) {
            if (t + k < n) orow[t + k] = ex;
            ex += v[k];
        }
        uint32_t m = first;
#pragma unroll
        for (int d = 1; d < 64; d <<= 1) {
            const uint32_t y = __shfl_down(m, d);
            if (lane_id() + d < 64) m = min(m, y);
        }
        const int w = threadIdx.x >> 6;
        __syncthreads();
        if (lane_id() == 0) sm[w] = m;
        __syncthreads();
        uint32_t right = 0xFFFFFFFFu;
#pragma unroll
        for (int i = SCAN_W - 1; i >= 0; --i)
            if (i > w) right = min(right, sm[i]);
        uint32_t excl = __shfl_down(m, 1);
        if (lane_id() == 63) excl = 0xFFFFFFFFu;
        uint32_t nxt = min(excl, right);
#pragma unroll
        for (int k = SEG_I - 1; k >= 0; --k) {
            if (t + k < n) nrow[t + k] = nxt;
            if (v[k]) nxt = t + k;
        }
        if (first != 0xFFFFFFFFu) atomicMin(&s_min[0], first);
    }
    __syncthreads();
    if (threadIdx.x == 0) {
        if (with_blocks) { part->blk_sum = blk_sum; part->first_tree = s_min[1]; part->first_seq = s_min[2]; }
        if (with_counts) { part->cnt_sum = cnt_sum; part->first_nonempty = s_min[0]; }
    }
}

__global__ __launch_bounds__(SCAN_T) void k_scan_fix(Scratch sc, int with_counts, int with_blocks)
{
    __shared__ uint32_t s_v[8];
    __shared__ uint32_t s_pos;
    __shared__ __attribute__((aligned(16))) uint8_t s_img[PIX_SLOT + 16];
    const uint32_t seg = blockIdx.x, f = blockIdx.y, n = sc.ntiles, nseg = gridDim.x;
    const uint64_t fr = (uint64_t)f * n;
    const ScanPart *parts = reinterpret_cast<const ScanPart *>(sc.scan_part) + (uint64_t)f * nseg;
    if (threadIdx.x == 0) {
        uint32_t bb = 0, cb = 0, bt = 0, ct = 0, nx = n, tt = 0xFFFFFFFFu, tq = 0xFFFFFFFFu;
        for (uint32_t i = 0; i < nseg; ++i) {
            const ScanPart p = parts[i];
            if (i < seg) { bb += p.blk_sum; cb += p.cnt_sum; }
            bt += p.blk_sum; ct += p.cnt_sum;
            if (i > seg && p.first_nonempty < nx) nx = p.first_nonempty;
            tt = min(tt, p.first_tree); tq = min(tq, p.first_seq);
        }
        s_v[0] = bb; s_v[1] = cb; s_v[2] = nx; s_v[3] = tt; s_v[4] = tq; s_v[5] = bt; s_v[6] = ct;
    }
    __syncthreads();
    const uint32_t lo = seg * SEG, hi = min(lo + (uint32_t)SEG, n);
    if (with_blocks) {
        uint32_t tl = 0, sl = 0;
        const uint32_t t_tree = s_v[3], t_seq = s_v[4];
        if (sc.zm_model) {
            const ZstdModel *M = sc.zm_model;
            tl = t_tree != 0xFFFFFFFFu ? M->lit_desc_len : 0u;
            sl = t_seq != 0xFFFFFFFFu ? M->seq_desc_len : 0u;
            const uint32_t mine = (t_tree >= lo && t_tree < hi ? 1u : 0u) | (t_seq >= lo && t_seq < hi ? 2u : 0u);
            if (mine) {
                zstd_rewrite_defs(sc.blk_size + fr, sc.blk_slots + fr * sc.blk_stride, sc.blk_stride, M->lit_desc, tl, M->seq_desc, sl, t_tree, t_seq, mine, s_img, &s_pos);
                if (threadIdx.x == 0) {
                    if (mine & 1u) sc.blk_size[fr + t_tree] += tl;
                    if (mine & 2u) sc.blk_size[fr + t_seq] += sl;
                }
            }
        }
        uint32_t *orow = sc.blk_off + fr;
        const uint32_t base = s_v[0];
        for (uint32_t t = lo + threadIdx.x; t < hi; t += SCAN_T)
            orow[t] += base + (t > t_tree ? tl : 0u) + (t > t_seq ? sl : 0u);
        if (seg == 0 && threadIdx.x == 0) sc.frame_cbytes[f] = s_v[5] + tl + sl;
    }
    if (with_counts) {
        uint32_t *orow = sc.tile_off + fr, *nrow = sc.tile_next + fr;
        const uint32_t base = s_v[1], nx = s_v[2];
        for (uint32_t t = lo + threadIdx.x; t < hi; t += SCAN_T) {
            orow[t] += base;
            if (nrow[t] == 0xFFFFFFFFu) nrow[t] = nx;
        }
        if (seg == 0 && threadIdx.x == 0) sc.frame_nnz[f] = s_v[6];
    }
}

void launch_scans(const Scratch &sc, uint32_t B, bool with_counts, bool with_blocks, hipStream_t s)
{
    if (!with_counts && !with_blocks) return;
    if (sc.ntiles > (uint32_t)SEG && sc.scan_part) {
        const dim3 grid((sc.ntiles + SEG - 1) / SEG, B);
        hipLaunchKernelGGL(k_scan_seg, grid, dim3(SCAN_T), 0, s, sc, with_counts ? 1 : 0, with_blocks ? 1 : 0);
        hipLaunchKernelGGL(k_scan_fix, grid, dim3(SCAN_T), 0, s, sc, with_counts ? 1 : 0, with_blocks ? 1 : 0);
        return;
    }
    if (sc.ntiles > 8192) hipLaunchKernelGGL(k_scan_frames<32>, dim3(B), dim3(SCAN_T), 0, s, sc, with_counts ? 1 : 0, with_blocks ? 1 : 0);
    else hipLaunchKernelGGL(k_scan_frames<16>, dim3(B), dim3(SCAN_T), 0, s, sc, with_counts ? 1 : 0, with_blocks ? 1 : 0);
}

constexpr int LWG = WG;
__global__ __launch_bounds__(LWG) void k_layout(const uint32_t *__restrict__ frame_nnz,
                                                 const uint32_t *__restrict__ frame_cbytes, const uint32_t *__restrict__ frame_pbytes,
                                                 RecordParams rp, uint64_t nb,
                                                 uint32_t ntiles, uint32_t B, uint64_t out_cap, uint64_t *__restrict__ rec_off,
                                                 uint32_t *__restrict__ md, BatchStatus *__restrict__ st, u32x4 *__restrict__ zl_acc)
{
    __shared__ uint64_t s_part[LWG];
    __shared__ uint32_t s_bad;
    if (threadIdx.x == 0) s_bad = 0xFFFFFFFFu;
    __syncthreads();
    const uint32_t per = (B + LWG - 1) / LWG;
    const uint32_t lo = threadIdx.x * per;
    const uint32_t hi = min(lo + per, B);
    uint64_t sum = 0;
    for (uint32_t f = lo; f < hi; ++f) {
        const uint32_t nnz = rp.level == 1 ? frame_nnz[f] : 0;
        const uint32_t npk = rp.level == 1 ? packed_bytes(nnz, rp.depth) : 0;
        uint64_t sz;
        uint32_t m0 = 0, m1 = 0, m2 = 0;
        if (rp.emit == EMIT_RAW) {
            if (rp.level == 1) { sz = 8 + nb + npk; m0 = npk; }
            else sz = 4 + nb;
        } else {
            const FrameFmt ff = frame_fmt(rp.emit);
            const uint32_t cb = bitmap_hdr(ff, rp.emit, ntiles) + frame_cbytes[f] + ff.end;
            if (rp.level == 1) {
                const uint32_t cp = rp.pix_mode == PIX_MODE_SKIP ? ff.hdr + frame_pbytes[f] : stored_size(ff, npk);
                sz = 16 + (uint64_t)cb + cp; m0 = cb; m1 = cp; m2 = npk;
            } else { sz = 8 + (uint64_t)cb; m0 = cb; }
        }
        md[3 * f] = m0; md[3 * f + 1] = m1; md[3 * f + 2] = m2;
        if (zl_acc) { zl_acc[2 * f] = u32x4{0u, 0u, 0u, 0u}; zl_acc[2 * f + 1] = u32x4{0u, 0u, 0u, 0u}; }
        if (sz > rp.frame_bytes) atomicMin(&s_bad, f);
        rec_off[f + 1] = sz;
        sum += sz;
    }
    s_part[threadIdx.x] = sum;
    __syncthreads();
    uint64_t base = 0;
    for (uint32_t i = 0; i < threadIdx.x; ++i) base += s_part[i];
    for (uint32_t f = lo; f < hi; ++f) {
        const uint64_t sz = rec_off[f + 1];
        base += sz;
        rec_off[f + 1] = base;
    }
    if (threadIdx.x == 0) rec_off[0] = 0;
    __syncthreads();
    if (threadIdx.x == LWG - 1) {
        uint64_t total = 0;
        for (uint32_t i = 0; i < LWG; ++i) total += s_part[i];
        st->total = total;
        if (s_bad != 0xFFFFFFFFu) { st->code = -5; st->frame = s_bad; }
        else if (total > out_cap) { st->code = -2; st->frame = 0; }
    }
}

void launch_layout(const Scratch &sc, const RecordParams &rp, uint32_t B, uint64_t out_cap, uint64_t *rec_off,
                   uint32_t *md, hipStream_t s)
{
    hipLaunchKernelGGL(k_layout, dim3(1), dim3(LWG), 0, s, sc.frame_nnz, sc.frame_cbytes, sc.frame_pbytes, rp, sc.nb, sc.ntiles, B, out_cap,
                       rec_off, md, sc.status, reinterpret_cast<u32x4 *>(sc.zl_acc));
}

static uint32_t xxh32_small(const uint8_t *p, size_t n)
{
    const uint32_t P1 = 2654435761u, P2 = 2246822519u, P3 = 3266489917u, P4 = 668265263u, P5 = 374761393u;
    (void)P1; (void)P4;
    uint32_t h = 0  + P5 + (uint32_t)n;
    for (size_t i = 0; i < n; ++i) {
        h += p[i] * P5;
        h = ((h << 11) | (h >> 21)) * P1;
    }
    h ^= h >> 15; h *= P2; h ^= h >> 13; h *= P3; h ^= h >> 16;
    return h;
}
uint32_t lz4f_descriptor(uint8_t bd)
{
    const uint8_t desc[2] = {0x60 , bd};
    const uint8_t hc = (uint8_t)((xxh32_small(desc, 2) >> 8) & 0xFF);
    return desc[0] | ((uint32_t)desc[1] << 8) | ((uint32_t)hc << 16);
}

void launch_assemble(const Scratch &sc, const RecordParams &rp, uint32_t B, uint8_t *out, const uint64_t *rec_off,
                     uint32_t batch_seq, hipStream_t s)
{
    static const uint32_t hdr_bitmap = lz4f_descriptor(0x40);
    static const uint32_t hdr_pix = lz4f_descriptor(0x70);
    launch_gather(sc, rp, B, out, rec_off, hdr_bitmap, hdr_pix, batch_seq, s);
}

}
```

Baseline: 145,000 frames/s.

## Replace separate per-tile scan kernels with per-item sums accumulated during reduce

For LZ4, blosc L1 and raw L1 paths with no value stage, the reduce kernel now writes a packed per-tile word (count and block size) and accumulates per-gather-item sums. The layout kernel scans these item sums to produce item bases and frame totals, and gather recomputes per-tile offsets with in-wave scans. This removes the dedicated tile scan kernels and the tile_off, blk_off and tile_next arrays. The tile_next scan is also skipped when gather does not need it. The cost is extra atomics or item-sum traffic in reduce, more serial work in the single-workgroup layout kernel, and a lane-parallel forward search in gather that replaces the tile_next lookup.

```diff
diff --git a/pyrecode_amd/csrc/rc_api.hip b/pyrecode_amd/csrc/rc_api.hip
--- a/pyrecode_amd/csrc/rc_api.hip
+++ b/pyrecode_amd/csrc/rc_api.hip
@@ -117,12 +117,21 @@
     DevMem &m = c->dmem;
     const uint64_t B = c->max_batch, T = sc.ntiles;
     RC_ALLOC(m, sc.bitmap, B * sc.nb_stride + 64);
-    RC_ALLOC(m, sc.tile_cnt, B * T * 4);
-    RC_ALLOC(m, sc.tile_off, B * T * 4);
-    RC_ALLOC(m, sc.tile_next, B * T * 4);
+    const bool items = sc.item_sums;
+    if (items) {
+        const uint64_t ni = ((B + 7) & ~7ull) * ((T + ITEM_TILES_MIN - 1) / ITEM_TILES_MIN);
+        RC_ALLOC(m, sc.tile_word, B * T * 4);
+        RC_ALLOC(m, sc.item_sum, ni * 8);
+        RC_ALLOC(m, sc.item_base, ni * 8);
+        HIP_TRY(hipMemset(sc.item_sum, 0, ni * 8));
+    } else {
+        RC_ALLOC(m, sc.tile_cnt, B * T * 4);
+        RC_ALLOC(m, sc.tile_off, B * T * 4);
+        RC_ALLOC(m, sc.tile_next, B * T * 4);
+        RC_ALLOC(m, sc.scan_part, B * ((T + 255) / 256) * 32);
+    }
     RC_ALLOC(m, sc.frame_nnz, B * 4);
     RC_ALLOC(m, sc.frame_cbytes, B * 4);
-    RC_ALLOC(m, sc.scan_part, B * ((T + 255) / 256) * 32);
     RC_ALLOC(m, sc.status, sizeof(BatchStatus));
     if (c->level != 3) RC_ALLOC(m, sc.pix_slots, B * T * TILE_PX * 2 + 64);
     if (c->emit != EMIT_RAW) {
@@ -131,8 +140,10 @@
             sc.blk_stride = 1536;
         }
         RC_ALLOC(m, sc.blk_slots, B * T * (uint64_t)sc.blk_stride + 256);
-        RC_ALLOC(m, sc.blk_size, B * T * 4);
-        RC_ALLOC(m, sc.blk_off, B * T * 4);
+        if (!items) {
+            RC_ALLOC(m, sc.blk_size, B * T * 4);
+            RC_ALLOC(m, sc.blk_off, B * T * 4);
+        }
         if (c->emit == EMIT_DEFLATE) {
             RC_ALLOC(m, sc.blk_aux, B * T * 4);
             RC_ALLOC(m, sc.zl_acc, B * 32);
@@ -283,6 +294,7 @@
     sc.nb_stride = (uint64_t)sc.ntiles * rc::TILE_BM;
     sc.max_batch = max_batch;
     sc.guarded_loads = getenv("RC_REDUCE_GUARDED_LOADS") != nullptr;
+    sc.item_sums = rc::item_sums_for(c->emit, reduction_level, src_bit_depth, c->values) && getenv("RC_SECOND_STAGE_SCANS") == nullptr;
     int rcode = ctx_alloc(c);
     if (rcode != RC_OK) {
         *status = rcode;
@@ -428,7 +440,7 @@
     HIP_TRY(hipMemsetAsync(d_sample, 0, sample_bytes, s));
     if (dz) {
         launch_reduce(sc, frames_dev, ns, 1u, CODEC_DEFLATE, true, c->depth, s, nullptr, c->src_bytes);
-        launch_scans(sc, ns, true, true, s);
+        launch_scans(sc, ns, true, true, gather_reads_tile_next(1u, c->depth), s);
         RecordParams rp;
         rp.level = 1u; rp.emit = c->emit; rp.depth = c->depth; rp.first_frame_id = 0; rp.packed_slots = 1u;
         rp.frame_bytes = c->geo().N * c->src_bytes;
@@ -534,7 +546,7 @@
     const bool lits_only = c->modelled && (c->h_model->valid & ZM_LITS_ONLY);
     if (c->emit == EMIT_ZSTD && !lits_only) launch_zstd_fse(sc, n, fitted_seq ? (const void *)&c->d_model->seq : c->d_ztab, fitted_seq, ps);
     if (all_ev) HIP_TRY(hipEventRecord(ev[2], ps));
-    launch_scans(sc, n, c->level != 3, c->emit != EMIT_RAW, ps);
+    if (!sc.item_sums) launch_scans(sc, n, c->level != 3, c->emit != EMIT_RAW, gather_reads_tile_next(c->level, c->depth), ps);
     if (all_ev) HIP_TRY(hipEventRecord(ev[3], ps));
     if (c->values_on) {
         rp.pix_mode = PIX_MODE_FLAT;
diff --git a/pyrecode_amd/csrc/rc_codec_api.hip b/pyrecode_amd/csrc/rc_codec_api.hip
--- a/pyrecode_amd/csrc/rc_codec_api.hip
+++ b/pyrecode_amd/csrc/rc_codec_api.hip
@@ -28,7 +28,7 @@
     sc.blk_off = sc.blk_size + T;
     sc.frame_cbytes = sc.blk_off + T;
     if ((r = encode(sc)) != RC_OK) return r;
-    launch_scans(sc, 1, false, true, u.stream);
+    launch_scans(sc, 1, false, true, false, u.stream);
     HIP_TRY(hipMemcpyAsync(u.h_scalar, sc.frame_cbytes, 4, hipMemcpyDeviceToHost, u.stream));
     HIP_TRY(hipStreamSynchronize(u.stream));
     const uint64_t total = total_of(T, *reinterpret_cast<uint32_t *>(u.h_scalar));
diff --git a/pyrecode_amd/csrc/rc_gather.hip b/pyrecode_amd/csrc/rc_gather.hip
--- a/pyrecode_amd/csrc/rc_gather.hip
+++ b/pyrecode_amd/csrc/rc_gather.hip
@@ -10,6 +10,8 @@
     const uint8_t *blk_slots, *bitmap;
     const uint16_t *pix_slots;
     const uint32_t *blk_size, *blk_off, *tile_cnt, *tile_off, *tile_next, *frame_nnz, *frame_cbytes, *frame_pbytes;
+    const uint32_t *tile_word;
+    const uint64_t *item_base;
     const uint32_t *blk_aux;
     uint32_t *zl_acc;
     uint8_t *pixraw;
@@ -82,7 +84,7 @@
 
 constexpr int GATHER_U = 4, GATHER_UB = 3;
 constexpr int GATHER_WPE = 8;
-template <bool BITS, int U, bool ADLER>
+template <bool BITS, int U, bool ADLER, bool ITEMS>
 __global__ __launch_bounds__(64) __attribute__((amdgpu_waves_per_eu(GATHER_WPE))) void k_gather(GatherArgs sc, RecordParams rp, uint8_t *__restrict__ out, const uint64_t *__restrict__ rec_off,
                                                uint32_t lz4f_hdr_bitmap, uint32_t lz4f_hdr_pix, uint32_t batch_seq, uint32_t gpf, uint32_t nitems, uint32_t tpi)
 {
@@ -117,7 +119,15 @@
 
         uint32_t word = 0, bsz = 0, bdst = 0, cnt = 0, rn = 0, rdst = 0, rs = 0xFFFFFFFFu, ps0 = 0, flags = 0, blo = 0;
         AdlerAcc ad{0u, 0u};
-        if (have && rp.emit != EMIT_RAW && (!flat || (sc.comb == COMB_BEHIND_BLOCK && pixp))) word = sc.blk_size[frow + t];
+        uint32_t cnt_w = 0, boff_w = 0, coff_w = 0;
+        uint64_t ibase = 0;
+        if (ITEMS) {
+            const uint32_t tw = have && (rp.emit != EMIT_RAW || pixp) ? sc.tile_word[frow + t] : 0u;
+            ibase = sc.item_base[item];
+            word = tw >> 16; cnt_w = tw & 0xFFFFu;
+            boff_w = (uint32_t)(ibase >> 32) + wave_incl_scan(word) - word;
+            coff_w = (uint32_t)ibase + wave_incl_scan(cnt_w) - cnt_w;
+        } else if (have && rp.emit != EMIT_RAW && (!flat || (sc.comb == COMB_BEHIND_BLOCK && pixp))) word = sc.blk_size[frow + t];
         if (have && !flat) {
             if (rp.emit == EMIT_RAW) {
                 const uint64_t b0 = (uint64_t)t * TILE_BM;
@@ -125,15 +135,15 @@
                 bdst = (uint32_t)(bitmap_pos + b0);
             } else {
                 bsz = word;
-                const uint32_t boff = bhdr + sc.blk_off[frow + t];
+                const uint32_t boff = bhdr + (ITEMS ? boff_w : sc.blk_off[frow + t]);
                 bdst = (uint32_t)bitmap_pos + boff;
                 if (rp.emit == EMIT_BLOSC) store_u32_le(rec + bitmap_pos + 16 + 4 * (uint64_t)t, boff);
             }
         }
         if (have && pixp) {
-            cnt = sc.tile_cnt[frow + t];
+            cnt = ITEMS ? cnt_w : sc.tile_cnt[frow + t];
             if (cnt) {
-                const ResidGeom q = resid_geom(sc.tile_off[frow + t], cnt, d);
+                const ResidGeom q = resid_geom(ITEMS ? coff_w : sc.tile_off[frow + t], cnt, d);
                 ps0 = q.ps0;
                 if (ADLER) blo = q.b_lo;
                 if (sc.comb) {
@@ -147,9 +157,10 @@
         }
         uint32_t ext_cnt = 0, ext_first = 0;
         if (BITS && pixp && t0 + tpi < sc.ntiles) {
-            ext_cnt = sc.tile_cnt[frow + t0 + tpi];
+            const uint32_t ew = ITEMS ? sc.tile_word[frow + t0 + tpi] : 0u;
+            ext_cnt = ITEMS ? ew & 0xFFFFu : sc.tile_cnt[frow + t0 + tpi];
             if (ext_cnt)
-                ext_first = *reinterpret_cast<const uint32_t *>(residual_src(sc, frow + t0 + tpi, sc.comb == COMB_BEHIND_BLOCK ? sc.blk_size[frow + t0 + tpi] : 0u, ext_cnt, d));
+                ext_first = *reinterpret_cast<const uint32_t *>(residual_src(sc, frow + t0 + tpi, ITEMS ? ew >> 16 : (sc.comb == COMB_BEHIND_BLOCK ? sc.blk_size[frow + t0 + tpi] : 0u), ext_cnt, d));
         }
         const uint8_t *slot = rp.emit == EMIT_RAW ? sc.bitmap + (uint64_t)f * sc.nb_stride + (uint64_t)t0 * TILE_BM : sc.blk_slots + (frow + t0) * sc.blk_stride;
         const uint32_t slot_stride = rp.emit == EMIT_RAW ? (uint32_t)TILE_BM : sc.blk_stride;
@@ -201,7 +212,8 @@
         }
         if (pixp) {
         ResidGeom q{0u, 0u, 0u, 0u};
-        if (cnt) q = resid_geom(sc.tile_off[frow + t], cnt, d);
+        const uint32_t coff2 = ITEMS ? (uint32_t)sc.item_base[item] + wave_incl_scan(cnt) - cnt : 0u;
+        if (cnt) q = resid_geom(ITEMS ? coff2 : sc.tile_off[frow + t], cnt, d);
         for (uint64_t m = __builtin_amdgcn_ballot_w64((packed >> 31) != 0); m; m &= m - 1) {
             const uint32_t k = (uint32_t)__builtin_ctzll(m);
             const uint32_t n = lane_get(q.n, k), p0 = lane_get(q.ps0, k), b0 = lane_get(q.b_lo, k), rsk = lane_get(rs, k);
@@ -240,7 +252,24 @@
                 } else cur = 65;
             }
         }
-        if (got < 8) {
+        if (ITEMS) {
+            for (uint32_t b0 = t0 + tpi + 1; b0 < sc.ntiles && __builtin_amdgcn_ballot_w64(got < 8) != 0; b0 += 64) {
+                const uint32_t tt = b0 + lane;
+                uint32_t offer = tt < sc.ntiles ? sc.tile_word[frow + tt] : 0u;
+                if (offer & 0xFFFFu) {
+                    const uint32_t c2 = offer & 0xFFFFu;
+                    offer = (*reinterpret_cast<const uint32_t *>(residual_src(sc, frow + tt, offer >> 16, c2, d)) & 0xFFu) | (min(c2 * d, 8u) << 8);
+                } else offer = 0u;
+                for (uint64_t m = __builtin_amdgcn_ballot_w64(offer != 0); m && __builtin_amdgcn_ballot_w64(got < 8) != 0; m &= m - 1) {
+                    const uint32_t o2 = lane_get(offer, (uint32_t)__builtin_ctzll(m));
+                    if (got < 8) {
+                        const uint32_t take = min(8u - got, o2 >> 8);
+                        byte |= (o2 & ((1u << take) - 1u)) << got;
+                        got += take;
+                    }
+                }
+            }
+        } else if (got < 8) {
             uint32_t tt = cur == 65 ? (t0 + tpi - 1 < sc.ntiles ? sc.tile_next[frow + t0 + tpi - 1] : sc.ntiles) : (t0 + tpi < sc.ntiles ? sc.tile_next[frow + t0 + tpi] : sc.ntiles);
             while (tt < sc.ntiles) {
                 const uint32_t cc = sc.tile_cnt[frow + tt];
@@ -296,20 +325,25 @@
 void launch_gather(const Scratch &sc, const RecordParams &rp, uint32_t B, uint8_t *out, const uint64_t *rec_off, uint32_t hdr_bitmap, uint32_t hdr_pix,
                    uint32_t batch_seq, hipStream_t s)
 {
-    uint32_t tpi = 64;
-    while (tpi > 8 && (uint64_t)B * ((sc.ntiles + tpi - 1) / tpi) < 1024) tpi >>= 1;
+    const uint32_t tpi = item_tiles(B, sc.ntiles);
     const uint32_t gpf = (sc.ntiles + tpi - 1) / tpi, nitems = gpf * B, wgs = nitems;
     const GatherArgs ga{sc.blk_slots, sc.bitmap, sc.pix_slots, sc.blk_size, sc.blk_off, sc.tile_cnt, sc.tile_off, sc.tile_next, sc.frame_nnz, sc.frame_cbytes,
-                        sc.frame_pbytes, sc.blk_aux, sc.zl_acc, sc.pixraw, sc.status, sc.first_err, sc.nb, sc.nb_stride, sc.pixraw_stride, sc.ntiles, sc.blk_stride, sc.pix_slot_bytes, sc.comb};
+                        sc.frame_pbytes, sc.tile_word, sc.item_base, sc.blk_aux, sc.zl_acc, sc.pixraw, sc.status, sc.first_err, sc.nb, sc.nb_stride, sc.pixraw_stride, sc.ntiles, sc.blk_stride, sc.pix_slot_bytes, sc.comb};
     const bool bits = rp.level == 1 && rp.depth % 8 != 0;
-    if (rp.emit == EMIT_DEFLATE) {
-        if (bits) hipLaunchKernelGGL((k_gather<true, GATHER_UB - 1, true>), dim3(wgs), dim3(64), 0, s, ga, rp, out, rec_off, hdr_bitmap, hdr_pix, batch_seq, gpf, nitems, tpi);
-        else hipLaunchKernelGGL((k_gather<false, GATHER_U, true>), dim3(wgs), dim3(64), 0, s, ga, rp, out, rec_off, hdr_bitmap, hdr_pix, batch_seq, gpf, nitems, tpi);
-        if (rp.pix_mode != PIX_MODE_FLAT) hipLaunchKernelGGL(k_zlib_finish, dim3((B + 63) / 64), dim3(64), 0, s, ga, rp, out, rec_off, B);
-    } else if (bits)
-        hipLaunchKernelGGL((k_gather<true, GATHER_UB, false>), dim3(wgs), dim3(64), 0, s, ga, rp, out, rec_off, hdr_bitmap, hdr_pix, batch_seq, gpf, nitems, tpi);
-    else
-        hipLaunchKernelGGL((k_gather<false, GATHER_U, false>), dim3(wgs), dim3(64), 0, s, ga, rp, out, rec_off, hdr_bitmap, hdr_pix, batch_seq, gpf, nitems, tpi);
-}
-
-}
+    auto go = [&](auto k, bool finish) {
+        hipLaunchKernelGGL(k, dim3(wgs), dim3(64), 0, s, ga, rp, out, rec_off, hdr_bitmap, hdr_pix, batch_seq, gpf, nitems, tpi);
+        if (finish && rp.pix_mode != PIX_MODE_FLAT) hipLaunchKernelGGL(k_zlib_finish, dim3((B + 63) / 64), dim3(64), 0, s, ga, rp, out, rec_off, B);
+    };
+    auto pick = [&](auto items) {
+        constexpr bool IT = decltype(items)::value != 0;
+        if (rp.emit == EMIT_DEFLATE) {
+            if (bits) go(k_gather<true, GATHER_UB - 1, true, IT>, true);
+            else go(k_gather<false, GATHER_U, true, IT>, true);
+        } else if (bits) go(k_gather<true, GATHER_UB, false, IT>, false);
+        else go(k_gather<false, GATHER_U, false, IT>, false);
+    };
+    if (sc.item_sums) pick(int_c<1>{});
+    else pick(int_c<0>{});
+}
+
+}
diff --git a/pyrecode_amd/csrc/rc_launch.h b/pyrecode_amd/csrc/rc_launch.h
--- a/pyrecode_amd/csrc/rc_launch.h
+++ b/pyrecode_amd/csrc/rc_launch.h
@@ -56,7 +56,20 @@
     uint16_t *l2_base = nullptr;
     uint32_t *chunk_aux = nullptr;
     const DeflateModel *dz_model = nullptr;
+    bool item_sums = false;
+    uint32_t *tile_word = nullptr;
+    uint64_t *item_sum = nullptr;
+    uint64_t *item_base = nullptr;
 };
+
+inline uint32_t item_tiles(uint32_t B, uint32_t ntiles)
+{
+    uint32_t tpi = 64;
+    while (tpi > 8 && (uint64_t)B * ((ntiles + tpi - 1) / tpi) < 1024) tpi >>= 1;
+    return tpi;
+}
+constexpr uint32_t ITEM_TILES_MIN = 8;
+__host__ __device__ inline uint32_t tile_word_of(uint32_t cnt, uint32_t bsz) { return cnt | (bsz << 16); }
 
 constexpr uint32_t EMIT_RAW = 0u;
 constexpr uint32_t EMIT_ZSTD = 1u;
@@ -95,7 +108,8 @@
 void launch_reduce32(const Scratch &sc, const uint32_t *frames, const uint32_t *thr32, uint32_t B, uint32_t level, uint32_t depth, hipStream_t s,
                      uint32_t codec = CODEC_NONE, bool keep_bitmap = true);
 void launch_l2(const Scratch &sc, uint32_t B, uint32_t nx, uint32_t use_sum, uint32_t depth, hipStream_t s);
-void launch_scans(const Scratch &sc, uint32_t B, bool with_counts, bool with_blocks, hipStream_t s);
+void launch_scans(const Scratch &sc, uint32_t B, bool with_counts, bool with_blocks, bool with_next, hipStream_t s);
+inline bool gather_reads_tile_next(uint32_t level, uint32_t depth) { return level != 3 && depth % 8 != 0; }
 void launch_layout(const Scratch &sc, const RecordParams &rp, uint32_t B, uint64_t out_cap, uint64_t *rec_off,
                    uint32_t *md, hipStream_t s);
 void launch_assemble(const Scratch &sc, const RecordParams &rp, uint32_t B, uint8_t *out, const uint64_t *rec_off,
@@ -111,6 +125,12 @@
 {
     if (level == 1 && emit == EMIT_ZSTD && clevel != 0) return VALUES_ZSTD_HUFF;
     return level == 1 && emit == EMIT_DEFLATE && clevel >= 2 ? VALUES_DEFLATE_HUFF : VALUES_NONE;
+}
+inline bool item_sums_for(uint32_t emit, uint32_t level, uint32_t src_bit_depth, ValueStage values)
+{
+    if (src_bit_depth > 16 || values != VALUES_NONE || (level != 1 && level != 3)) return false;
+    if (emit == EMIT_RAW) return level == 1;
+    return emit == EMIT_LZ4 || (emit == EMIT_BLOSC && level == 1);
 }
 constexpr uint32_t PIX_CHUNK = 1008, PIX_SLOT = 1024, PD_CHUNK = 1u << 15, PD_SLOT = PD_CHUNK + 32;
 struct ValueGeom { uint32_t chunk, slot; };
diff --git a/pyrecode_amd/csrc/rc_reduce.hip b/pyrecode_amd/csrc/rc_reduce.hip
--- a/pyrecode_amd/csrc/rc_reduce.hip
+++ b/pyrecode_amd/csrc/rc_reduce.hip
@@ -208,11 +208,19 @@
     return (total + 63u) >> 6;
 }
 
+struct ItemSums { uint64_t *sum; uint32_t shift, gpf; };
+constexpr bool codec_item_sums(int codec) { return codec != CODEC_ZSTD_FAST && codec != CODEC_ZSTD_MODELLED && codec != CODEC_DEFLATE; }
+__device__ __forceinline__ uint64_t item_sum_index(uint32_t f, uint32_t g, uint32_t gpf)
+{
+    return ((uint64_t)(f / REDUCE_BZ) * gpf + g) * REDUCE_BZ + f % REDUCE_BZ;
+}
+
 template <bool LEVEL1, int CODEC, bool KEEP_BITMAP>
 __device__ __forceinline__ uint32_t flush_pending(const Pending &p, uint32_t tile, uint32_t n_blk, uint8_t *__restrict__ bitmap,
                                                   uint64_t nb_stride, uint16_t *__restrict__ pix_slots, uint32_t *__restrict__ tile_cnt,
                                                   uint8_t *__restrict__ blk_slots, uint32_t *__restrict__ blk_size, Lz4Lds *lz,
-                                                  const WaveStage *st, uint32_t blk_stride, uint32_t comb, uint32_t *__restrict__ blk_aux)
+                                                  const WaveStage *st, uint32_t blk_stride, uint32_t comb, uint32_t *__restrict__ blk_aux,
+                                                  const ItemSums &is, uint32_t &tword)
 {
     if (!p.valid) return 0;
     const int lane = lane_id();
@@ -254,7 +262,10 @@
     }
     if (LEVEL1 || CODEC) {
         const uint32_t word = CODEC == CODEC_ZSTD_FAST || CODEC == CODEC_ZSTD_MODELLED ? p.csize : bsz;
-        if (LEVEL1 && CODEC == CODEC_DEFLATE) {
+        if (codec_item_sums(CODEC) && is.sum) {
+            tword = tile_word_of(LEVEL1 ? p.cnt : 0u, CODEC ? word : 0u);
+            if (lane == 0) tile_cnt[p.ft] = tword;
+        } else if (LEVEL1 && CODEC == CODEC_DEFLATE) {
             if (lane < 3) *(lane == 0 ? &tile_cnt[p.ft] : (lane == 1 ? &blk_size[p.ft] : &blk_aux[p.ft])) = lane == 0 ? p.cnt : (lane == 1 ? word : p.aux);
         } else if (LEVEL1 && CODEC) {
             if (lane < 2) *(lane == 0 ? &tile_cnt[p.ft] : &blk_size[p.ft]) = lane == 0 ? p.cnt : word;
@@ -344,7 +355,7 @@
                                                  uint32_t *__restrict__ tile_cnt, uint8_t *__restrict__ blk_slots,
                                                  uint32_t *__restrict__ blk_size, Lz4Lds *s_lz, uint8_t *s_bm, WaveStage *st,
                                                  Pending &pend, uint32_t &stores_behind, const ZmParams &zp, uint32_t blk_stride, uint32_t comb,
-                                                 uint32_t *__restrict__ blk_aux)
+                                                 uint32_t *__restrict__ blk_aux, const ItemSums &is, uint32_t &tword)
 {
     const int lane = lane_id();
     RC_PHASE_BEGIN
@@ -462,7 +473,7 @@
         pend.csize = lz4_encode_block(pend.cown, n_blk, *s_lz);
     }
     RC_PHASE(5);
-    stores_behind = flush_pending<LEVEL1, CODEC, KEEP_BITMAP>(pend, tile, n_blk, bitmap, nb_stride, pix_slots, tile_cnt, blk_slots, blk_size, s_lz, st, blk_stride, comb, blk_aux);
+    stores_behind = flush_pending<LEVEL1, CODEC, KEEP_BITMAP>(pend, tile, n_blk, bitmap, nb_stride, pix_slots, tile_cnt, blk_slots, blk_size, s_lz, st, blk_stride, comb, blk_aux, is, tword);
     pend.valid = false;
     RC_PHASE(6);
 }
@@ -476,7 +487,7 @@
                                                        uint16_t *__restrict__ pix_slots, uint32_t *__restrict__ tile_cnt,
                                                        uint8_t *__restrict__ blk_slots, uint32_t *__restrict__ blk_size, uint32_t depth,
                                                        BatchStatus *__restrict__ status, ZmParams zm, uint32_t blk_stride, uint32_t comb,
-                                                       uint32_t *__restrict__ blk_aux)
+                                                       uint32_t *__restrict__ blk_aux, ItemSums is)
 {
     if (blockIdx.x == 0 && threadIdx.x == 0) { status->code = 0; status->frame = 0; status->total = 0; }
     __shared__ uint16_t s_code[CODEC == CODEC_ZSTD_MODELLED ? 256 : 2];
@@ -518,6 +529,7 @@
     pend.buf = nullptr;
 
     uint32_t stores_behind = 0;
+    uint32_t tword = 0, tw[BZ] = {};
 #pragma unroll 1
     for (int z = 0; z < BZ; ++z) {
         const uint32_t f = f0 + z;
@@ -526,10 +538,21 @@
         reduce_one_frame<ALIGNED, ASMLOAD, LEVEL1, CODEC, KEEP_BITMAP, RAWVAL, SB>(xa, frames + (uint64_t)f * N, frames + (uint64_t)(f + 1) * N, nxt, t,
                                                                              lane_px0, N, full, f, tile, (uint64_t)f * ntiles + tile, n_blk,
                                                                              bitmap, nb_stride, pix_slots, tile_cnt, blk_slots,
-                                                                             blk_size, lz, bm, st, pend, stores_behind, zm, blk_stride, comb, blk_aux);
+                                                                             blk_size, lz, bm, st, pend, stores_behind, zm, blk_stride, comb, blk_aux, is, tword);
+        tword = (uint32_t)__builtin_amdgcn_readfirstlane((int)tword);
+#pragma unroll
+        for (int k = 0; k < BZ; ++k) tw[k] = z == k ? tword : tw[k];
         if (!nxt) break;
     }
-    flush_pending<LEVEL1, CODEC, KEEP_BITMAP>(pend, tile, n_blk, bitmap, nb_stride, pix_slots, tile_cnt, blk_slots, blk_size, lz, st, blk_stride, comb, blk_aux);
+    flush_pending<LEVEL1, CODEC, KEEP_BITMAP>(pend, tile, n_blk, bitmap, nb_stride, pix_slots, tile_cnt, blk_slots, blk_size, lz, st, blk_stride, comb, blk_aux, is, tword);
+    if (codec_item_sums(CODEC) && is.sum) {
+        uint32_t mine = 0;
+#pragma unroll
+        for (int k = 0; k < BZ; ++k) mine = lane == k ? tw[k] : mine;
+        if (lane < BZ && f0 + lane < B)
+            __hip_atomic_fetch_add(is.sum + item_sum_index(f0 + lane, tile >> is.shift, is.gpf), (uint64_t)(mine & 0xFFFFu) | ((uint64_t)(mine >> 16) << 32),
+                                   __ATOMIC_RELAXED, __HIP_MEMORY_SCOPE_AGENT);
+    }
 }
 
 template <int BZ, bool AL, bool L1, int CODEC, bool KEEP, bool RAW, int SB>
@@ -541,22 +564,26 @@
     const uint32_t comb = (L1 && !RAW && CODEC) ? sc.comb : COMB_OFF;
     const bool three = L1 && !RAW && CODEC != CODEC_DEFLATE &&
                        (CODEC == CODEC_LZ4_RUNS || CODEC == CODEC_LZ4_EVENTS || sc.ntiles > 8192 || (CODEC == CODEC_ZSTD_MODELLED && (sc.zm_valid & ZM_LITS_ONLY)));
+    const bool items = sc.item_sums && !RAW;
+    const uint32_t tpi = item_tiles(B, sc.ntiles);
+    const ItemSums is{items ? sc.item_sum : nullptr, (uint32_t)__builtin_ctz(tpi), (sc.ntiles + tpi - 1) / tpi};
+    uint32_t *const words = items ? sc.tile_word : sc.tile_cnt;
     auto go = [&](auto rw) {
         constexpr int RW = decltype(rw)::value;
         auto grid_for = [&](uint32_t nt) { return (((nt + RW - 1) / RW + 7) / 8) * 8 * ngroups; };
         if (nfull)
             hipLaunchKernelGGL((k_reduce_tiles<RW, BZ, AL, AL, L1, CODEC, KEEP, RAW, SB>), dim3(grid_for(nfull)), dim3(64 * RW), 0, s, frames, sc.thr, sc.N,
-                               sc.ntiles, 0u, nfull, B, ngroups, sc.nb, sc.bitmap, sc.nb_stride, sc.pix_slots, sc.tile_cnt, sc.blk_slots,
-                               sc.blk_size, depth, sc.status, zm, sc.blk_stride, comb, sc.blk_aux);
+                               sc.ntiles, 0u, nfull, B, ngroups, sc.nb, sc.bitmap, sc.nb_stride, sc.pix_slots, words, sc.blk_slots,
+                               sc.blk_size, depth, sc.status, zm, sc.blk_stride, comb, sc.blk_aux, is);
         if (nfull < sc.ntiles) {
             if (AL && sc.N % 8 != 0)
                 hipLaunchKernelGGL((k_reduce_tiles<RW, BZ, false, false, L1, CODEC, KEEP, RAW, SB>), dim3(grid_for(sc.ntiles - nfull)), dim3(64 * RW), 0, nfull ? s_tail : s, frames,
-                                   sc.thr, sc.N, sc.ntiles, nfull, sc.ntiles, B, ngroups, sc.nb, sc.bitmap, sc.nb_stride, sc.pix_slots, sc.tile_cnt,
-                                   sc.blk_slots, sc.blk_size, depth, sc.status, zm, sc.blk_stride, comb, sc.blk_aux);
+                                   sc.thr, sc.N, sc.ntiles, nfull, sc.ntiles, B, ngroups, sc.nb, sc.bitmap, sc.nb_stride, sc.pix_slots, words,
+                                   sc.blk_slots, sc.blk_size, depth, sc.status, zm, sc.blk_stride, comb, sc.blk_aux, is);
             else
                 hipLaunchKernelGGL((k_reduce_tiles<RW, BZ, AL, false, L1, CODEC, KEEP, RAW, SB>), dim3(grid_for(sc.ntiles - nfull)), dim3(64 * RW), 0, nfull ? s_tail : s, frames,
-                                   sc.thr, sc.N, sc.ntiles, nfull, sc.ntiles, B, ngroups, sc.nb, sc.bitmap, sc.nb_stride, sc.pix_slots, sc.tile_cnt,
-                                   sc.blk_slots, sc.blk_size, depth, sc.status, zm, sc.blk_stride, comb, sc.blk_aux);
+                                   sc.thr, sc.N, sc.ntiles, nfull, sc.ntiles, B, ngroups, sc.nb, sc.bitmap, sc.nb_stride, sc.pix_slots, words,
+                                   sc.blk_slots, sc.blk_size, depth, sc.status, zm, sc.blk_stride, comb, sc.blk_aux, is);
         }
     };
     if constexpr (SB == 2) {
@@ -614,6 +641,7 @@
 }
 
 constexpr int SCAN_T = 256, SCAN_W = SCAN_T / 64;
+constexpr int SCAN_CNT = 1, SCAN_NEXT = 2;
 
 __device__ __forceinline__ uint32_t scan_block_excl(uint32_t v, uint32_t *sm, uint32_t *total)
 {
@@ -753,6 +781,7 @@
     if (!with_counts) return;
     uint32_t *row = sc.tile_cnt + fr;
     scan_row<SCAN_I>(row, sc.tile_off + fr, n, sc.frame_nnz + f, sm);
+    if (!(with_counts & SCAN_NEXT)) return;
     uint32_t *nrow = sc.tile_next + fr;
     if (threadIdx.x == 0) s_carry = n;
     __syncthreads();
@@ -853,6 +882,7 @@
             if (t + k < n) orow[t + k] = ex;
             ex += v[k];
         }
+        if (with_counts & SCAN_NEXT) {
         uint32_t m = first;
 #pragma unroll
         for (int d = 1; d < 64; d <<= 1) {
@@ -876,6 +906,7 @@
             if (v[k]) nxt = t + k;
         }
         if (first != 0xFFFFFFFFu) atomicMin(&s_min[0], first);
+        }
     }
     __syncthreads();
     if (threadIdx.x == 0) {
@@ -932,35 +963,63 @@
         const uint32_t base = s_v[1], nx = s_v[2];
         for (uint32_t t = lo + threadIdx.x; t < hi; t += SCAN_T) {
             orow[t] += base;
-            if (nrow[t] == 0xFFFFFFFFu) nrow[t] = nx;
+            if ((with_counts & SCAN_NEXT) && nrow[t] == 0xFFFFFFFFu) nrow[t] = nx;
         }
         if (seg == 0 && threadIdx.x == 0) sc.frame_nnz[f] = s_v[6];
     }
 }
 
-void launch_scans(const Scratch &sc, uint32_t B, bool with_counts, bool with_blocks, hipStream_t s)
+void launch_scans(const Scratch &sc, uint32_t B, bool with_counts, bool with_blocks, bool with_next, hipStream_t s)
 {
     if (!with_counts && !with_blocks) return;
+    const int cnt = with_counts ? (with_next ? SCAN_CNT | SCAN_NEXT : SCAN_CNT) : 0;
     if (sc.ntiles > (uint32_t)SEG && sc.scan_part) {
         const dim3 grid((sc.ntiles + SEG - 1) / SEG, B);
-        hipLaunchKernelGGL(k_scan_seg, grid, dim3(SCAN_T), 0, s, sc, with_counts ? 1 : 0, with_blocks ? 1 : 0);
-        hipLaunchKernelGGL(k_scan_fix, grid, dim3(SCAN_T), 0, s, sc, with_counts ? 1 : 0, with_blocks ? 1 : 0);
+        hipLaunchKernelGGL(k_scan_seg, grid, dim3(SCAN_T), 0, s, sc, cnt, with_blocks ? 1 : 0);
+        hipLaunchKernelGGL(k_scan_fix, grid, dim3(SCAN_T), 0, s, sc, cnt, with_blocks ? 1 : 0);
         return;
     }
-    if (sc.ntiles > 8192) hipLaunchKernelGGL(k_scan_frames<32>, dim3(B), dim3(SCAN_T), 0, s, sc, with_counts ? 1 : 0, with_blocks ? 1 : 0);
-    else hipLaunchKernelGGL(k_scan_frames<16>, dim3(B), dim3(SCAN_T), 0, s, sc, with_counts ? 1 : 0, with_blocks ? 1 : 0);
-}
-
-constexpr int LWG = WG;
-__global__ __launch_bounds__(LWG) void k_layout(const uint32_t *__restrict__ frame_nnz,
-                                                 const uint32_t *__restrict__ frame_cbytes, const uint32_t *__restrict__ frame_pbytes,
+    if (sc.ntiles > 8192) hipLaunchKernelGGL(k_scan_frames<32>, dim3(B), dim3(SCAN_T), 0, s, sc, cnt, with_blocks ? 1 : 0);
+    else hipLaunchKernelGGL(k_scan_frames<16>, dim3(B), dim3(SCAN_T), 0, s, sc, cnt, with_blocks ? 1 : 0);
+}
+
+constexpr int LWG = WG, LAYOUT_U = 4;
+__global__ __launch_bounds__(LWG) void k_layout(uint32_t *frame_nnz, uint32_t *frame_cbytes, const uint32_t *__restrict__ frame_pbytes,
                                                  RecordParams rp, uint64_t nb,
                                                  uint32_t ntiles, uint32_t B, uint64_t out_cap, uint64_t *__restrict__ rec_off,
-                                                 uint32_t *__restrict__ md, BatchStatus *__restrict__ st, u32x4 *__restrict__ zl_acc)
+                                                 uint32_t *__restrict__ md, BatchStatus *__restrict__ st, u32x4 *__restrict__ zl_acc,
+                                                 uint64_t *__restrict__ item_sum, uint64_t *__restrict__ item_base, uint32_t gpf)
 {
     __shared__ uint64_t s_part[LWG];
     __shared__ uint32_t s_bad;
     if (threadIdx.x == 0) s_bad = 0xFFFFFFFFu;
+    if (item_sum) {
+        const uint32_t w = threadIdx.x >> 6, lane = (uint32_t)lane_id(), nch = (gpf + 63) / 64;
+        const uint32_t rows = w < B ? ((B - w + WAVES - 1) / WAVES) * nch : 0u;
+        auto at = [&](uint32_t i) { return (uint64_t)(w + WAVES * (i / nch)) * gpf + 64u * (i % nch) + lane; };
+        auto sum_at = [&](uint32_t i) { return item_sum_index(w + WAVES * (i / nch), 64u * (i % nch) + lane, gpf); };
+        auto have = [&](uint32_t i) { return 64u * (i % nch) + lane < gpf; };
+        uint64_t carry = 0;
+        for (uint32_t i0 = 0; i0 < rows; i0 += LAYOUT_U) {
+            uint64_t v[LAYOUT_U];
+#pragma unroll
+            for (int u = 0; u < LAYOUT_U; ++u) v[u] = i0 + u < rows && have(i0 + u) ? item_sum[sum_at(i0 + u)] : 0ull;
+#pragma unroll
+            for (int u = 0; u < LAYOUT_U; ++u) {
+                const uint32_t i = i0 + u;
+                if (i >= rows) break;
+                if (i % nch == 0) carry = 0;
+                const uint64_t inc = wave_incl_scan64(v[u]);
+                if (have(i)) { item_base[at(i)] = carry + inc - v[u]; item_sum[sum_at(i)] = 0; }
+                carry += ((uint64_t)wave_last((uint32_t)(inc >> 32)) << 32) | wave_last((uint32_t)inc);
+                if (i % nch == nch - 1 && lane == 0) {
+                    const uint32_t f = w + WAVES * (i / nch);
+                    frame_nnz[f] = (uint32_t)carry;
+                    frame_cbytes[f] = (uint32_t)(carry >> 32);
+                }
+            }
+        }
+    }
     __syncthreads();
     const uint32_t per = (B + LWG - 1) / LWG;
     const uint32_t lo = threadIdx.x * per;
@@ -1011,8 +1070,10 @@
 void launch_layout(const Scratch &sc, const RecordParams &rp, uint32_t B, uint64_t out_cap, uint64_t *rec_off,
                    uint32_t *md, hipStream_t s)
 {
+    const uint32_t tpi = item_tiles(B, sc.ntiles);
     hipLaunchKernelGGL(k_layout, dim3(1), dim3(LWG), 0, s, sc.frame_nnz, sc.frame_cbytes, sc.frame_pbytes, rp, sc.nb, sc.ntiles, B, out_cap,
-                       rec_off, md, sc.status, reinterpret_cast<u32x4 *>(sc.zl_acc));
+                       rec_off, md, sc.status, reinterpret_cast<u32x4 *>(sc.zl_acc), sc.item_sums ? sc.item_sum : nullptr, sc.item_base,
+                       (sc.ntiles + tpi - 1) / tpi);
 }
 
 static uint32_t xxh32_small(const uint8_t *p, size_t n)
```

After: 145,800 frames/s, median of 6. Within noise of the previous version (+0.5%).
